# apple/ml-unigen

Hardware: AMD Instinct MI355X
Metric: train-step samples/s (1.5B, 256^2 img) (higher is better)
Workload: dtype bf16

## Files before the change

include/unigen_hip.h:

```cpp
#ifndef UNIGEN_HIP_H
#define UNIGEN_HIP_H

#include <stdint.h>
#include <hip/hip_runtime_api.h>

#ifdef __cplusplus
extern "C" {
#endif

#define UG_ABI_VERSION 7

const char* ug_last_error(void);
int ug_abi_version(void);

typedef struct ug_handle ug_handle;
int ug_create(ug_handle** out);
int ug_destroy(ug_handle* h);

#define UG_EPI_BF16 0
#define UG_EPI_F32 1
#define UG_EPI_RESID 2
int ug_gemm_bf16(const ug_handle* h, const void* A, int64_t lda, int a_kmajor, const void* B, int64_t ldb, int b_kmajor,
                 void* C, int64_t ldc, int64_t M, int64_t N, int64_t K, int epilogue, const void* bias,
                 const float* resid, int64_t ldr, int beta, const float* alpha_dev, int policy, hipStream_t stream);
#define UG_GEMM_NARROW_EPILOGUE 0x100
#define UG_GEMM_ONE_BARRIER 0x200
#define UG_GEMM_TWO_BARRIERS 0x400
#define UG_GEMM_POLICY_AUTO_BITS 0xff

int ug_cast_f32_bf16(const float* in, void* out, int64_t n, hipStream_t stream);

int ug_gemm_bf16_swiglu_bwd(const ug_handle* h, const void* dy, int64_t ld_dy, const void* w_down, int64_t ldw, const void* gu,
                            int64_t ld_gu, void* dgu, int64_t ld_dgu, int64_t M, int64_t I, int64_t K, hipStream_t stream);
int ug_gemm_set_fused_tile_height(int rows);
int ug_gemm_bf16_qkv_rope(const ug_handle* h, const void* x, int64_t ldx, const void* w, int64_t ldw, const void* bias, void* qkv,
                          int64_t ldq, int64_t M, int64_t N, int64_t K, const float* cos_tab, const float* sin_tab, int64_t L,
                          int64_t rope_cols, int head_dim, hipStream_t stream);
int ug_gemm_bf16_swiglu(const ug_handle* h, const void* x, int64_t ldx, const void* w_gate_up, int64_t ldw, void* gu,
                        int64_t ld_gu, void* act, int64_t ld_act, int64_t M, int64_t I, int64_t K, hipStream_t stream);

int ug_gemm_bf16_wgrad_group(int n, const void* const* dy, const int64_t* ld_dy, const void* const* x, const int64_t* ld_x,
                             float* const* dw, const int64_t* ld_dw, const int64_t* rows, const int64_t* cols,
                             const int* beta, const int64_t* K, hipStream_t stream);

int ug_rmsnorm_fwd(const float* x, const float* w, void* y, float* rstd, int64_t rows, int64_t cols,
                   float eps, int out_f32, hipStream_t stream);
int ug_rmsnorm_bwd(const void* dy, const float* x, const float* rstd, const float* w, float* dres,
                   float* dw, void* dres_bf16, int64_t rows, int64_t cols, hipStream_t stream);
int ug_rope(void* qkv, const float* cos_tab, const float* sin_tab, int64_t tokens, int64_t L, int64_t ldq,
            int nheads, int head_dim, int backward, hipStream_t stream);
int ug_swiglu_fwd(const void* gate_up, void* act, int64_t tokens, int64_t I, hipStream_t stream);
int ug_swiglu_bwd(const void* gate_up, const void* dact, void* dgate_up, int64_t tokens, int64_t I,
                  hipStream_t stream);
int ug_gelu(const void* x, const void* dy_or_null, void* out, int64_t n, hipStream_t stream);
int ug_embed_fwd(const int64_t* ids, const float* W, float* out, int64_t tokens, int64_t H, int64_t V,
                 int* err_flag, hipStream_t stream);
int ug_embed_bwd(const int64_t* ids, const float* dout, float* dW, int64_t tokens, int64_t H, int64_t V,
                 hipStream_t stream);
int ug_embed_bwd_sorted(const int64_t* ids_sorted, const int64_t* order, const float* rows, float* dW, int64_t n,
                        int64_t H, int64_t V, float scale, hipStream_t stream);
int ug_gather_rows_bf16(const void* in, int64_t ld_in, const int64_t* idx, void* out, int64_t ld_out,
                        int64_t n, int64_t C, int scatter, hipStream_t stream);
int ug_colsum_bf16(const void* in, int64_t ld, float* out, int64_t R, int64_t C, hipStream_t stream);

#define UG_MASK_F32 0
#define UG_MASK_BF16 1
#define UG_MASK_I64 2
#define UG_MASK_BOOL 3
int ug_attn_mask_compress(const void* mask, int mask_dtype, int64_t stride_b, int64_t stride_row,
                          uint64_t* bits, uint8_t* tileany, int64_t B, int64_t L, int* err_flag,
                          hipStream_t stream);
int ug_attn_mask_causal(const uint8_t* key_valid , uint64_t* bits, uint8_t* tileany,
                        int64_t B, int64_t L, hipStream_t stream);
int ug_attn_fwd(const void* q, const void* k, const void* v, int64_t ldq, void* o,
                int64_t ldo, float* lse, const uint64_t* bits, const uint8_t* tileany, int64_t B, int64_t L,
                int64_t Lp, int H, int HKV, int head_dim, float scale, hipStream_t stream);
int ug_attn_bwd(const void* q, const void* k, const void* v, int64_t ldq,
                const void* o, const void* dout, int64_t ldo, const float* lse,
                float* delta, void* dq, void* dk, void* dv, int64_t ldg, const uint64_t* bits,
                const uint8_t* tileany, int64_t B, int64_t L, int64_t Lp, int H, int HKV, int head_dim,
                float scale, float* dkv_ws, const float* rope_cos, const float* rope_sin, float* dbias_qkv, hipStream_t stream);

int ug_kv_store(const void* qkv, int64_t ldq, int64_t k_col, int64_t v_col, void* cache_k, void* cache_v,
                int64_t rows, int64_t L, int HKV, int head_dim, int64_t Tmax, const int* pos_dev, int pos_host,
                hipStream_t stream);
int ug_rope_at(void* qkv, const float* cos_tab, const float* sin_tab, int64_t rows, int64_t ldq, int nheads,
               int head_dim, const int* pos_dev, int64_t max_pos, hipStream_t stream);
int ug_attn_decode(const void* q, int64_t ldq, const void* cache_k, const void* cache_v, const uint8_t* key_valid,
                   void* o, int64_t ldo, int64_t rows, int H, int HKV, int head_dim, int64_t Tmax,
                   const int* len_dev, float scale, hipStream_t stream);
int ug_gemv_bf16(const void* x, int64_t ldx, int64_t R, const void* W, int64_t ldw, float* acc, int64_t acc_stride_r,
                 int64_t acc_stride_n, int64_t N, int64_t K, hipStream_t stream);
int ug_decode_finish_resid_norm(float* acc, int64_t ldacc, float* x, const float* w, void* xn, int64_t rows, int64_t cols,
                                float eps, int* pos_inc, int* len_inc, hipStream_t stream);
int ug_decode_gemv(const void* x, int64_t ldx, int64_t R, const void* W, int64_t ldw, float* acc, int64_t ldacc, int64_t N,
                   int64_t K, float* zero0, int64_t n0, float* zero1, int64_t n1, float* ss_zero, hipStream_t stream);
int ug_decode_gemv_resid_norm(const float* x_in, const float* pending, int64_t ld_pending, const float* norm_w, float* x_out,
                              float* ss_out, int64_t R, const void* W, int64_t ldw, float* acc, int64_t ldacc, int64_t N,
                              int64_t K, float* zero0, int64_t n0, float* zero1, int64_t n1, float* ss_zero,
                              hipStream_t stream);
int ug_decode_gemv_swiglu(const float* gate_up_acc, int64_t ld_gu, const float* ss_in, float eps, int64_t norm_cols, int64_t R,
                          const void* W, int64_t ldw, float* acc, int64_t ldacc, int64_t N, int64_t K, float* zero0, int64_t n0,
                          float* zero1, int64_t n1, float* ss_zero, hipStream_t stream);
int ug_attn_decode_fused(const float* acc_qkv, int64_t ldacc, const float* ss_in, float eps, int64_t norm_cols, const void* bias,
                         const float* cos_tab, const float* sin_tab, const int* pos_dev, void* cache_k, void* cache_v,
                         const uint8_t* key_valid, void* o, int64_t ldo, int64_t rows, int H, int HKV, int head_dim,
                         int64_t Tmax, int64_t max_pos, float scale, hipStream_t stream);
int ug_decode_sw_supported(int64_t hidden, int64_t inter, int64_t q_dim, int head_dim);
int ug_decode_sw_kblock(const void* x, int64_t ldx, int64_t R, const void* W, int64_t ldw, float* acc, int64_t ldacc, int64_t N, int64_t K,
                        float* zero0, int64_t n0, float* zero1, int64_t n1, float* ss_zero, hipStream_t stream);
int ug_decode_sw_resid(const void* x, int64_t ldx, int64_t R, const void* W, int64_t ldw, int64_t N, int64_t K, float* h,
                       hipStream_t stream);
int ug_decode_sw_gate_up(const float* h, const float* pend, int64_t ld_pend, float* x_out, const float* norm_w, float eps, int64_t R,
                         int64_t H, const void* W, int64_t ldw, int64_t I, void* act, int64_t ld_act, hipStream_t stream);
int ug_decode_sw_head(const float* h, const float* pend, int64_t ld_pend, float* x_out, const float* norm_w, float eps, int64_t R,
                      int64_t H, const void* W, int64_t ldw, int64_t N, float* logits, int64_t ld_logits, int* pos_inc, int* len_inc,
                      hipStream_t stream);
int ug_skinny_finish(const float* acc, const void* bias, void* out_bf16, float* resid, int64_t M, int64_t N,
                     int mode, hipStream_t stream);
int ug_gemv_bf16_ord(const void* x, int64_t ldx, int64_t R, const void* W, int64_t ldw, float* part, int64_t ldpart, int64_t part_stride,
                     int64_t N, int64_t K, hipStream_t stream);
int ug_skinny_finish_ord(const float* parts, int64_t nparts, int64_t part_stride, const void* bias, void* out_bf16, float* out_f32,
                         float* resid, int64_t M, int64_t N, hipStream_t stream);
int ug_decode_gemv_resid_norm_ord(const float* x_in, const float* pend_parts, int64_t ld_pending, int64_t npend, const float* norm_w,
                                  float* x_out, float* ss_part, int64_t R, const void* W, int64_t ldw, float* part, int64_t ldpart,
                                  int64_t N, int64_t K, hipStream_t stream);
int ug_attn_decode_fused_ord(const float* qkv_part, int64_t ldpart, int64_t nparts, const float* ss_part, float eps, int64_t norm_cols,
                             const void* bias, const float* cos_tab, const float* sin_tab, const int* pos_dev, void* cache_k,
                             void* cache_v, const uint8_t* key_valid, void* o, int64_t ldo, int64_t rows, int H, int HKV, int head_dim,
                             int64_t Tmax, int64_t max_pos, float scale, hipStream_t stream);
int ug_decode_sw_kblock_ord(const void* x, int64_t ldx, int64_t R, const void* W, int64_t ldw, float* part, int64_t ldpart, int64_t N,
                            int64_t K, hipStream_t stream);
int ug_decode_finish_resid_norm_ord(const float* parts, int64_t ldp, int64_t nparts, float* x, const float* w, void* xn, int64_t rows,
                                    int64_t cols, float eps, int* pos_inc, int* len_inc, hipStream_t stream);

int ug_t2i_assemble(const int64_t* text_ids, const int64_t* text_offsets, const int64_t* conv_start, int64_t n_start,
                    const int64_t* conv_end, int64_t n_end, const int64_t* image_in, const int64_t* image_labels, int64_t B,
                    int64_t n_image, int64_t max_seq_len, int64_t pad_id, int64_t soi_id, int64_t eoi_id, int64_t ignore_id,
                    int64_t* input_ids, int64_t* labels, uint8_t* attn01, hipStream_t stream);
int ug_attn_mask_from_ids(const int64_t* ids, int64_t B, int64_t L, int64_t pad_id, int64_t soi_id, int64_t eoi_id, int mode,
                          int* meta_ws, uint8_t* flags_ws, uint64_t* bits, uint8_t* tileany, hipStream_t stream);

int ug_maskgit_train_mask(const int64_t* tokens, const float* scores, const float* num_masked, int64_t B, int64_t n,
                          int64_t mask_id, int64_t ignore_id, int64_t* input_ids, int64_t* labels, hipStream_t stream);

int ug_maskgit_step(const void* logits, int64_t ld, int64_t V, int64_t N, int64_t n, int cfg, float guidance_scale,
                    const float* u_sample, const float* u_conf, const int64_t* cur_ids, int64_t mask_id, int64_t id_offset,
                    int64_t mask_len_sched, float temperature, int64_t* sampled, float* sel_ws, int64_t* next_cur,
                    int64_t* next_ids, uint8_t* masking_out, hipStream_t stream);

int ug_ar_sample(float* acc, int64_t ldacc, int64_t bsz, int64_t V, float guidance_scale, float temperature, int greedy,
                 const float* uniforms, const int* pos_dev, int64_t pos0, int64_t nsteps, const float* embed, int64_t ld_embed,
                 int64_t H, int64_t id_offset, int64_t* tok, int* out_tokens, float* x, hipStream_t stream);

int ug_ar_sample_filtered(float* acc, int64_t ldacc, int64_t bsz, int64_t V, float guidance_scale, float temperature, int greedy,
                          const float* uniforms, const int* pos_dev, int64_t pos0, int64_t nsteps, const float* embed,
                          int64_t ld_embed, int64_t H, int64_t id_offset, int64_t* tok, int* out_tokens, float* x, int64_t top_k,
                          float top_p, float min_p, float* stats, hipStream_t stream);

int ug_text_pick(float* logits, int64_t ld, int64_t R, int64_t V, int clear, const int64_t* stop_ids, int64_t n_stop, int64_t pad_id,
                 const float* embed, int64_t ld_embed, int64_t embed_rows, int64_t H, int* state, int64_t nsteps, int64_t* tok,
                 int* out_tokens, int* lengths, float* x, hipStream_t stream);

int ug_text_sample_workspace_ints(int64_t R);

int ug_text_sample(float* logits, int64_t ld, int64_t R, int64_t V, int clear, float temperature, int64_t top_k, float top_p,
                   const float* uniforms, int* workspace, float* stats, const int64_t* stop_ids, int64_t n_stop, int64_t pad_id,
                   const float* embed, int64_t ld_embed, int64_t embed_rows, int64_t H, int* state, int64_t nsteps, int64_t* tok,
                   int* out_tokens, int* lengths, float* x, hipStream_t stream);


int ug_text_seen_mark(int* seen, int64_t ld_words, const int64_t* ids, int64_t ld_ids, int64_t R, int64_t L, const uint8_t* valid,
                      int64_t V, hipStream_t stream);

int ug_text_penalize(float* logits, int64_t ld, int64_t R, int64_t V, float penalty, int* seen, int64_t ld_words, const int64_t* tok,
                     hipStream_t stream);

int ug_ce_fwd(const void* logits, int64_t ld, int64_t R, int64_t V, const int64_t* labels,
              int64_t ignore_index, float* lse, float* loss_row, float* logp_label, float* loss_and_count,
              hipStream_t stream);
int ug_ce_bwd(void* logits_inout, int64_t ld, int64_t R, int64_t V, const int64_t* labels,
              int64_t ignore_index, const float* lse, const float* loss_and_count, const float* gscale,
              const float* row_scale, hipStream_t stream);

int ug_adamw_flat(float* p, const float* g, float* m, float* v, void* p_bf16, int64_t n, float lr,
                  float beta1, float beta2, float eps, float weight_decay, int64_t step, float grad_scale,
                  int max_blocks ,
                  hipStream_t stream);

int ug_grad_pack_bf16(const float* in, void* out_bf16, int64_t n, float scale, hipStream_t stream);
int ug_zero_ranges_f32(float* buf, const int64_t* ranges, int64_t n_ranges, int64_t max_len, hipStream_t stream);
int ug_grad_unpack_bf16(const void* in_bf16, float* out, int64_t n, hipStream_t stream);
int ug_grad_sum_shards_bf16(const void* shards_bf16, int world, int64_t stride, void* out_bf16, int64_t n, float scale,
                            hipStream_t stream);

typedef struct ug_comm ug_comm;
#define UG_COMM_ID_BYTES 128
#define UG_COMM_FP32 0
#define UG_COMM_BF16_FP32ACC 1
#define UG_COMM_BF16 2
#define UG_COMM_FP32_RSAG 3
int ug_comm_unique_id(void* id128);
int ug_comm_init(ug_comm** out, int world, int rank, const void* id128, int64_t max_bucket_elems);
int ug_comm_allreduce_bucket(ug_comm* comm, float* grad, int64_t n, int mode, hipStream_t producer);
int ug_comm_allgather(ug_comm* comm, const void* send, void* recv, int64_t bytes_per_rank, hipStream_t producer);
int ug_comm_wait(ug_comm* comm, hipStream_t consumer);
int ug_comm_destroy(ug_comm* comm);
int64_t ug_comm_bytes_on_wire(const ug_comm* comm);

int ug_conv2d_f32(const float* x, const float* w_packed, const float* bias, const float* residual, float* y,
                  int64_t B, int Hin, int Win, int Cin, int Cout, int cout_pad, int ksize, int stride,
                  int pad_top, int pad_left, int Hout, int Wout, int upsample2x, hipStream_t stream);
int ug_conv_split_weights(const float* w_packed, uint16_t* w_split, int taps, int Cin, int cout_pad, hipStream_t stream);
int ug_amax_f32(const float* x, int64_t rows, int64_t cols, int64_t ld, float* out_amax, hipStream_t stream);
int ug_amax_f32_into_zeroed(const float* x, int64_t rows, int64_t cols, int64_t ld, float* out_amax, hipStream_t stream);
int ug_conv2d_split(const float* x, const float* x_amax, const uint16_t* w_split, const float* bias, const float* residual,
                    float* y, int64_t B, int Hin, int Win, int Cin, int Cout, int cout_pad, int ksize, int stride,
                    int pad_top, int pad_left, int Hout, int Wout, int upsample2x, double* out_stats, int out_groups,
                    hipStream_t stream);
int ug_conv3x3_split(const float* x, const float* x_amax, const uint16_t* w_split, const float* bias, const float* residual,
                     float* y, int64_t B, int H, int W, int Cin, int Cout, int cout_pad, const float* gn_mu_rstd,
                     const float* gn_gamma, const float* gn_beta, int gn_groups, int gn_swish, double* out_stats, int out_groups,
                     hipStream_t stream);
int ug_groupnorm_finalize(const double* stats, float* mu_rstd, int64_t B, int64_t HW, int C, int groups, float eps,
                          hipStream_t stream);
int ug_groupnorm_stats(const float* x, double* stats_ws, float* mu_rstd, int64_t B, int64_t HW, int C, int groups,
                       float eps, hipStream_t stream);
int ug_siglip_attn_f32(const float* qkv, int64_t ld, const float* qkv_amax, float* out, int64_t ldo, int64_t B, int64_t T,
                       int H, int head_dim, float scale, hipStream_t stream);
int ug_linear_split(const float* x, int64_t ldx, const float* x_amax, const uint16_t* w_split, const float* bias,
                    const float* residual, int64_t ldres, float* y, int64_t ldy, int64_t M, int64_t N, int64_t K, int n_pad,
                    int act, hipStream_t stream);
int ug_gemm_f32(const float* A, int64_t lda, int64_t stride_a, const float* B, int64_t ldb, int64_t stride_b,
                int b_is_nk, float* C, int64_t ldc, int64_t stride_c, int64_t M, int64_t N, int64_t K,
                int64_t batch, float alpha, hipStream_t stream);
int ug_gemm_f32_nested(const float* A, int64_t lda, int64_t sa_in, int64_t sa_out, const float* B, int64_t ldb,
                       int64_t sb_in, int64_t sb_out, int b_is_nk, float* C, int64_t ldc, int64_t sc_in, int64_t sc_out,
                       int64_t M, int64_t N, int64_t K, int64_t batch_in, int64_t batch_out, float alpha,
                       hipStream_t stream);
int ug_groupnorm_swish(const float* x, const float* gamma, const float* beta, float* y, double* stats_ws,
                       int64_t B, int64_t HW, int C, int groups, float eps, int apply_swish, hipStream_t stream);
int ug_softmax_rows_f32(float* x, int64_t rows, int64_t cols, int64_t ld, float scale, hipStream_t stream);
int ug_linear_f32(const float* x, int64_t ldx, const float* W, int64_t ldw, const float* bias,
                  const float* residual, int64_t ldres, float* y, int64_t ldy, int64_t M, int64_t N, int64_t K,
                  int act, hipStream_t stream);
int ug_layernorm_f32(const float* x, const float* gamma, const float* beta, float* y, int64_t rows, int64_t cols,
                     float eps, hipStream_t stream);
int ug_layernorm_bwd_f32(const float* dy, const float* x, const float* gamma, const float* dres_in, float* dx, float* dgamma,
                         float* dbeta, int64_t rows, int64_t cols, float eps, hipStream_t stream);
int ug_gelu_tanh_f32(const float* pre, const float* dy_or_null, float* out, int64_t n, hipStream_t stream);
int ug_softmax_bwd_rows_f32(const float* P, float* dP, int64_t rows, int64_t cols, int64_t ld, float scale, hipStream_t stream);
int ug_colsum_f32(const float* x, int64_t ld, float* out, int64_t rows, int64_t cols, hipStream_t stream);
int ug_transpose_f32(const float* in, int64_t ld_in, int64_t stride_in, float* out, int64_t ld_out, int64_t stride_out,
                     int64_t rows, int64_t cols, int64_t batch, hipStream_t stream);
int ug_nchw_to_nhwc(const float* in, float* out, int64_t B, int C, int64_t HW, int c_pad, hipStream_t stream);
int ug_nhwc_to_nchw(const float* in, float* out, int64_t B, int C, int64_t HW, int c_pad, hipStream_t stream);
int ug_lfq_pack(const float* z, int64_t ldz, int64_t* idx, int64_t n, int nbits, hipStream_t stream);
int ug_lfq_unpack(const int64_t* idx, float* z, int64_t n, int nbits, int* err_flag, hipStream_t stream);

int ug_probe_layouts(float* out, int64_t n_floats, hipStream_t stream);

#ifdef __cplusplus
}
#endif
#endif
```

ml-unigen_amd/csrc/gemm_bf16.hip:

```cpp
#include "common.h"
#include <type_traits>
#include <atomic>
#include "unigen_hip.h"
#include "vmem_asm.h"

namespace {

constexpr int BM = 128, BN = 128, BK = 64;
constexpr int TILE_BYTES = BM * BK * 2;
constexpr int GROUP_M = 8;
constexpr int P8_GROUP_M = 4;

enum Epi { EPI_BF16 = 0, EPI_F32 = 1, EPI_RESID = 2, EPI_ROPE = 3, EPI_SWIGLU = 4, EPI_SWIGLU_BWD = 5 };

typedef const __attribute__((address_space(1))) void* gptr_t;
typedef __attribute__((address_space(3))) void* lptr_t;
typedef __attribute__((ext_vector_type(4))) short s16x4_t;

__device__ __attribute__((aligned(16))) uint32_t g_zero_page[64];

struct GemmArgs {
  const bf16_t* A; const bf16_t* B; void* C;
  const bf16_t* bias;
  const float* resid;
  const float* alpha_dev;
  int M, N, K;
  int64_t lda, ldb, ldc, ldr;
  int beta;
  const bf16_t* sw_gu; int64_t ld_gu;
  const float* rope_cos; const float* rope_sin; int rope_L, rope_cols;
  int tiles_m, tiles_n;
  int full_tiles, tail_split;
  float* tail_ws;
  int tail_private;
  int one_barrier;
  int wide_epilogue;
  int swiglu_I;
  bf16_t* act; int64_t ld_act;
};

__device__ __forceinline__ int swz_rowk(int row, int chunk) { return chunk ^ ((row >> 1) & 7); }
__device__ __forceinline__ int swz_krow(int k, int chunk) { return chunk ^ ((((k & 3) | (((k >> 3) & 1) << 2))) << 1); }

template <bool KMAJOR, int ROWS, int NW>
struct Stager {
  static constexpr int NI = ROWS / (8 * NW);
  const bf16_t* src[NI];
  int64_t step[NI];
  int kofs[NI];
  __device__ __forceinline__ void init(const bf16_t* X, int64_t ld, int row0, int rows_total, int wave, int lane) {
    const bf16_t* zero = reinterpret_cast<const bf16_t*>(g_zero_page);
    constexpr int CPR = ROWS / 8;
    constexpr int KPI = 64 / CPR;
#pragma unroll
    for (int i = 0; i < NI; ++i) {
      const int inst = i * NW + wave;
      if constexpr (!KMAJOR) {
        const int row = inst * 8 + (lane >> 3);
        const int chunk = swz_rowk(row, lane & 7);
        const int r = min(row0 + row, rows_total - 1);
        src[i] = X + (int64_t)r * ld + chunk * 8;
        step[i] = BK;
        kofs[i] = chunk * 8;
      } else {
        const int k = inst * KPI + lane / CPR;
        const int chunk = swz_krow(k, lane % CPR);
        const int col = row0 + chunk * 8;
        const bool ok = (col + 8 <= ld);
        src[i] = ok ? X + (int64_t)k * ld + col : zero;
        step[i] = ok ? (int64_t)BK * ld : 0;
        kofs[i] = k;
      }
    }
  }
  template <bool CHECK>
  __device__ __forceinline__ void issue(int kt, int K, char* lds_tile, int wave) const {
    const bf16_t* zero = reinterpret_cast<const bf16_t*>(g_zero_page);
#pragma unroll
    for (int i = 0; i < NI; ++i) {
      const bf16_t* s = src[i] + kt * step[i];
      if constexpr (CHECK) {
        const bool past = kt * BK + kofs[i] >= (KMAJOR ? K : ((K + 7) & ~7));
        s = reinterpret_cast<const bf16_t*>(past ? reinterpret_cast<uintptr_t>(zero) : reinterpret_cast<uintptr_t>(s));
      }
      char* dst = lds_tile + (i * NW + wave) * 1024;
      __builtin_amdgcn_global_load_lds((gptr_t)s, (lptr_t)dst, 16, 0, 0);
    }
  }
};

template <bool KMAJOR, int ROWS>
__device__ __forceinline__ bf16x8_t load_frag(const char* tile, int r0, int ks, int lane) {
  if constexpr (!KMAJOR) {
    const int row = r0 + (lane & 15);
    const int chunk = swz_rowk(row, ks * 4 + (lane >> 4));
    return *reinterpret_cast<const bf16x8_t*>(tile + row * 128 + chunk * 16);
  } else {
    const int i16 = lane & 15, g = lane >> 4;
    const int k = ks * 32 + g * 8 + (i16 >> 2);
    const int chunk = (r0 >> 3) + ((i16 & 3) >> 1);
    const int sub = (i16 & 1) * 8;
    const char* p0 = tile + k * (ROWS * 2) + swz_krow(k, chunk) * 16 + sub;
    const char* p1 = tile + (k + 4) * (ROWS * 2) + swz_krow(k + 4, chunk) * 16 + sub;
    const s16x4_t lo = __builtin_amdgcn_ds_read_tr16_b64_v4i16((__attribute__((address_space(3))) s16x4_t*)p0);
    const s16x4_t hi = __builtin_amdgcn_ds_read_tr16_b64_v4i16((__attribute__((address_space(3))) s16x4_t*)p1);
    return __builtin_shufflevector(lo, hi, 0, 1, 2, 3, 4, 5, 6, 7);
  }
}

template <int EPI>
__device__ __forceinline__ void store_tile(const GemmArgs& p, f32x4_t (&acc)[4][4], int mbase, int nbase, int lane,
                                           bool split) {
  float alpha = 1.f;
  if constexpr (EPI == EPI_F32) { if (p.alpha_dev) alpha = *p.alpha_dev; }
#pragma unroll
  for (int i = 0; i < 4; ++i) {
    const int m = mbase + i * 16 + (lane & 15);
    if (m >= p.M) continue;
#pragma unroll
    for (int j = 0; j < 4; ++j) {
      const int n = nbase + j * 16 + (lane >> 4) * 4;
      if (n >= p.N) continue;
      f32x4_t v = acc[i][j];
      const bool full = (n + 3 < p.N);
      if constexpr (EPI == EPI_BF16) {
        bf16_t* c = reinterpret_cast<bf16_t*>(p.C) + (int64_t)m * p.ldc + n;
        if (p.bias) {
#pragma unroll
          for (int r = 0; r < 4; ++r) if (n + r < p.N) v[r] += bf2f(p.bias[n + r]);
        }
        if (full) {
          uint2 o; o.x = pack_bf2(v[0], v[1]); o.y = pack_bf2(v[2], v[3]);
          *reinterpret_cast<uint2*>(c) = o;
        } else {
          for (int r = 0; r < 4; ++r) if (n + r < p.N) c[r] = f2bf(v[r]);
        }
      } else if constexpr (EPI == EPI_F32) {
        float* c = reinterpret_cast<float*>(p.C) + (int64_t)m * p.ldc + n;
        if (split) {
          for (int r = 0; r < 4; ++r) if (n + r < p.N) atomicAdd(c + r, v[r] * alpha);
        } else if (full) {
          float4 o = make_float4(v[0] * alpha, v[1] * alpha, v[2] * alpha, v[3] * alpha);
          if (p.beta) { const float4 old = *reinterpret_cast<const float4*>(c);
                        o.x += old.x; o.y += old.y; o.z += old.z; o.w += old.w; }
          *reinterpret_cast<float4*>(c) = o;
        } else {
          for (int r = 0; r < 4; ++r) if (n + r < p.N) c[r] = (p.beta ? c[r] : 0.f) + v[r] * alpha;
        }
      } else {
        float* c = reinterpret_cast<float*>(p.C) + (int64_t)m * p.ldc + n;
        const float* rs = p.resid + (int64_t)m * p.ldr + n;
        if (full) {
          const float4 old = *reinterpret_cast<const float4*>(rs);
          float4 o;
          o.x = old.x + bf2f(f2bf(v[0])); o.y = old.y + bf2f(f2bf(v[1]));
          o.z = old.z + bf2f(f2bf(v[2])); o.w = old.w + bf2f(f2bf(v[3]));
          *reinterpret_cast<float4*>(c) = o;
        } else {
          for (int r = 0; r < 4; ++r) if (n + r < p.N) c[r] = rs[r] + bf2f(f2bf(v[r]));
        }
      }
    }
  }
}

#define UG_ST16(ptr, val) (*reinterpret_cast<uint4*>(ptr) = (val))
typedef unsigned int gnt4_t __attribute__((ext_vector_type(4)));
constexpr int EP_ROWS = 32;
constexpr int EP_PITCH_BF16 = 144, EP_PITCH_F32 = 272;
constexpr int EP_STRIP = EP_ROWS * EP_PITCH_F32;

__device__ __forceinline__ void rope_pair(float x1, float x2, float c, float s, float& o1, float& o2) {
#pragma clang fp contract(off)
  const float a1 = x1 * c, a2 = x2 * c;
  const float b1 = x2 * s, b2 = x1 * s;
  o1 = a1 - b1; o2 = a2 + b2;
}

template <int EPI, int MF = 8>
__device__ __forceinline__ void store_tile_lds(const GemmArgs& p, f32x4_t (&acc)[MF][4], char* strip, int mbase, int nbase, int lane,
                                               int rope_p0 = 0, bool roped = false) {
  constexpr bool BF = EPI == EPI_BF16 || EPI == EPI_ROPE;
  float alpha = 1.f;
  if constexpr (EPI == EPI_F32) { if (p.alpha_dev) alpha = *p.alpha_dev; }
  float bias4[4][4];
  if constexpr (BF) {
#pragma unroll
    for (int j = 0; j < 4; ++j) {
      uint2 b = make_uint2(0u, 0u);
      const int cj = EPI == EPI_ROPE ? (j & 1) * 16 + (j >> 1) * 64 : j * 16;
      if (p.bias) b = *reinterpret_cast<const uint2*>(p.bias + nbase + cj + (lane >> 4) * 4);
      bias4[j][0] = __uint_as_float(b.x << 16); bias4[j][1] = __uint_as_float(b.x & 0xffff0000u);
      bias4[j][2] = __uint_as_float(b.y << 16); bias4[j][3] = __uint_as_float(b.y & 0xffff0000u);
    }
  }
#pragma unroll
  for (int c = 0; c < (MF + 1) / 2; ++c) {
    const int rows_here = (2 * c + 1 < MF) ? 32 : 16;
#pragma unroll
    for (int ii = 0; ii < 2; ++ii) {
      if (2 * c + ii >= MF) break;
      const int row = ii * 16 + (lane & 15);
      if constexpr (EPI == EPI_ROPE) {
        if (roped) {
          const int pos = min(mbase + c * EP_ROWS + row, p.M - 1) % p.rope_L;
#pragma unroll
          for (int j = 0; j < 2; ++j) {
            const int pc = rope_p0 + j * 16 + (lane >> 4) * 4;
            const float4 cs = *reinterpret_cast<const float4*>(p.rope_cos + (int64_t)pos * 64 + pc);
            const float4 sn = *reinterpret_cast<const float4*>(p.rope_sin + (int64_t)pos * 64 + pc);
            const float cc[4] = {cs.x, cs.y, cs.z, cs.w}, ss[4] = {sn.x, sn.y, sn.z, sn.w};
            f32x4_t& lo = acc[2 * c + ii][j];
            f32x4_t& hi = acc[2 * c + ii][j + 2];
#pragma unroll
            for (int k = 0; k < 4; ++k) {
              const float x1 = bf2f(f2bf(lo[k] + bias4[j][k])), x2 = bf2f(f2bf(hi[k] + bias4[j + 2][k]));
              float o1, o2;
              rope_pair(x1, x2, cc[k], ss[k], o1, o2);
              lo[k] = o1; hi[k] = o2;
            }
          }
        }
      }
#pragma unroll
      for (int j = 0; j < 4; ++j) {
        const int col = j * 16 + (lane >> 4) * 4;
        const f32x4_t v = acc[2 * c + ii][j];
        if constexpr (EPI == EPI_ROPE) {
          uint2 o;
          if (roped) { o.x = pack_bf2(v[0], v[1]); o.y = pack_bf2(v[2], v[3]); }
          else { o.x = pack_bf2(v[0] + bias4[j][0], v[1] + bias4[j][1]); o.y = pack_bf2(v[2] + bias4[j][2], v[3] + bias4[j][3]); }
          *reinterpret_cast<uint2*>(strip + row * EP_PITCH_BF16 + col * 2) = o;
        } else if constexpr (EPI == EPI_BF16) {
          uint2 o;
          o.x = pack_bf2(v[0] + bias4[j][0], v[1] + bias4[j][1]);
          o.y = pack_bf2(v[2] + bias4[j][2], v[3] + bias4[j][3]);
          *reinterpret_cast<uint2*>(strip + row * EP_PITCH_BF16 + col * 2) = o;
        } else {
          *reinterpret_cast<float4*>(strip + row * EP_PITCH_F32 + col * 4) = make_float4(v[0], v[1], v[2], v[3]);
        }
      }
    }
    asm volatile("s_waitcnt lgkmcnt(0)" ::: "memory");
    if constexpr (BF) {
#pragma unroll
      for (int q = 0; q < 4; ++q) {
        const int row = q * 8 + (lane >> 3), ch = lane & 7;
        const int m = mbase + c * EP_ROWS + row;
        const uint4 v = *reinterpret_cast<const uint4*>(strip + row * EP_PITCH_BF16 + ch * 16);
        const int gc = EPI == EPI_ROPE ? (ch & 3) * 8 + (ch >> 2) * 64 : ch * 8;
        if (m < p.M && row < rows_here) UG_ST16(reinterpret_cast<bf16_t*>(p.C) + (int64_t)m * p.ldc + nbase + gc, v);
      }
    } else {
#pragma unroll
      for (int q = 0; q < 8; ++q) {
        const int row = q * 4 + (lane >> 4), ch = lane & 15;
        const int m = mbase + c * EP_ROWS + row;
        float4 v = *reinterpret_cast<const float4*>(strip + row * EP_PITCH_F32 + ch * 16);
        if (m < p.M && row < rows_here) {
          float* cptr = reinterpret_cast<float*>(p.C) + (int64_t)m * p.ldc + nbase + ch * 4;
          if constexpr (EPI == EPI_F32) {
            v.x *= alpha; v.y *= alpha; v.z *= alpha; v.w *= alpha;
            if (p.beta) { const float4 old = *reinterpret_cast<const float4*>(cptr); v.x += old.x; v.y += old.y; v.z += old.z; v.w += old.w; }
          } else {
            const float4 old = *reinterpret_cast<const float4*>(p.resid + (int64_t)m * p.ldr + nbase + ch * 4);
            v.x = old.x + bf2f(f2bf(v.x)); v.y = old.y + bf2f(f2bf(v.y)); v.z = old.z + bf2f(f2bf(v.z)); v.w = old.w + bf2f(f2bf(v.w));
          }
          *reinterpret_cast<float4*>(cptr) = v;
        }
      }
    }
    asm volatile("s_waitcnt lgkmcnt(0)" ::: "memory");
  }
}

__device__ __forceinline__ float silu_gemm(float g) { return silu_train(g); }

template <int MF>
__device__ __forceinline__ void store_tile_swiglu_perm(const GemmArgs& p, f32x4_t (&acc)[MF][4], char* strip, int mbase, int hbase, int lane) {
  constexpr int ACT_PITCH = 80;
  char* astrip = strip + EP_ROWS * EP_PITCH_BF16;
  bf16_t* C = reinterpret_cast<bf16_t*>(p.C);
#pragma unroll
  for (int c = 0; c < (MF + 1) / 2; ++c) {
    const int rows_here = (2 * c + 1 < MF) ? 32 : 16;
#pragma unroll
    for (int ii = 0; ii < 2; ++ii) {
      if (2 * c + ii >= MF) break;
      const int row = ii * 16 + (lane & 15);
#pragma unroll
      for (int j = 0; j < 2; ++j) {
        const f32x4_t gv = acc[2 * c + ii][j], uv = acc[2 * c + ii][j + 2];
        float a[4];
        uint32_t gb[4], ub[4];
#pragma unroll
        for (int k = 0; k < 4; ++k) {
          gb[k] = f2bf(gv[k]); ub[k] = f2bf(uv[k]);
          const float s = bf2f(f2bf(silu_gemm(bf2f((bf16_t)gb[k]))));
          a[k] = s * bf2f((bf16_t)ub[k]);
        }
        const int col = j * 16 + (lane >> 4) * 4;
        *reinterpret_cast<uint2*>(strip + row * EP_PITCH_BF16 + col * 2) = make_uint2(gb[0] | (gb[1] << 16), gb[2] | (gb[3] << 16));
        *reinterpret_cast<uint2*>(strip + row * EP_PITCH_BF16 + (32 + col) * 2) = make_uint2(ub[0] | (ub[1] << 16), ub[2] | (ub[3] << 16));
        *reinterpret_cast<uint2*>(astrip + row * ACT_PITCH + col * 2) = make_uint2(pack_bf2(a[0], a[1]), pack_bf2(a[2], a[3]));
      }
    }
    asm volatile("s_waitcnt lgkmcnt(0)" ::: "memory");
#pragma unroll
    for (int q = 0; q < 4; ++q) {
      const int row = q * 8 + (lane >> 3), ch = lane & 7;
      const int m = mbase + c * EP_ROWS + row;
      const uint4 v = *reinterpret_cast<const uint4*>(strip + row * EP_PITCH_BF16 + ch * 16);
      const int gc = (ch >> 2) * p.swiglu_I + hbase + (ch & 3) * 8;
      if (m < p.M && row < rows_here) UG_ST16(C + (int64_t)m * p.ldc + gc, v);
    }
#pragma unroll
    for (int q = 0; q < 2; ++q) {
      const int row = q * 16 + (lane >> 2), ch = lane & 3;
      const int m = mbase + c * EP_ROWS + row;
      const uint4 v = *reinterpret_cast<const uint4*>(astrip + row * ACT_PITCH + ch * 16);
      if (m < p.M && row < rows_here)
        UG_ST16(p.act + (int64_t)m * p.ld_act + hbase + ch * 8, v);
    }
    asm volatile("s_waitcnt lgkmcnt(0)" ::: "memory");
  }
}

typedef unsigned int gu4_t __attribute__((ext_vector_type(4)));
template <int MF>
__device__ __forceinline__ void store_tile_swiglu_bwd(const GemmArgs& p, f32x4_t (&acc)[MF][4], char* strip, int mbase, int nbase, int lane) {
  constexpr int NCH = (MF + 1) / 2;
  bf16_t* C = reinterpret_cast<bf16_t*>(p.C);
  const int I = p.swiglu_I;
  gu4_t gq[2][4], uq[2][4];
  auto fetch = [&](int c, gu4_t (&g)[4], gu4_t (&u)[4]) {
#pragma unroll
    for (int q = 0; q < 4; ++q) {
      const int row = q * 8 + (lane >> 3), ch = lane & 7;
      const int m = min(mbase + c * EP_ROWS + row, p.M - 1);
      const bf16_t* gp = p.sw_gu + (int64_t)m * p.ld_gu + nbase + ch * 8;
      asm volatile("global_load_dwordx4 %0, %1, off" : "=&v"(g[q]) : "v"(gp) : "memory");
      asm volatile("global_load_dwordx4 %0, %1, off" : "=&v"(u[q]) : "v"(gp + I) : "memory");
    }
  };
  fetch(0, gq[0], uq[0]);
#pragma unroll
  for (int c = 0; c < NCH; ++c) {
    const int rows_here = (2 * c + 1 < MF) ? 32 : 16;
    gu4_t (&g)[4] = gq[c & 1];
    gu4_t (&u)[4] = uq[c & 1];
    if (c + 1 < NCH) fetch(c + 1, gq[(c + 1) & 1], uq[(c + 1) & 1]);
#pragma unroll
    for (int ii = 0; ii < 2; ++ii) {
      if (2 * c + ii >= MF) break;
      const int row = ii * 16 + (lane & 15);
#pragma unroll
      for (int j = 0; j < 4; ++j) {
        const f32x4_t v = acc[2 * c + ii][j];
        *reinterpret_cast<uint2*>(strip + row * EP_PITCH_BF16 + (j * 16 + (lane >> 4) * 4) * 2) = make_uint2(pack_bf2(v[0], v[1]), pack_bf2(v[2], v[3]));
      }
    }
    if (c + 1 < NCH)
      asm volatile("s_waitcnt vmcnt(8)" : "+v"(g[0]), "+v"(g[1]), "+v"(g[2]), "+v"(g[3]), "+v"(u[0]), "+v"(u[1]), "+v"(u[2]), "+v"(u[3]) : : "memory");
    else
      asm volatile("s_waitcnt vmcnt(0)" : "+v"(g[0]), "+v"(g[1]), "+v"(g[2]), "+v"(g[3]), "+v"(u[0]), "+v"(u[1]), "+v"(u[2]), "+v"(u[3]) : : "memory");
    asm volatile("s_waitcnt lgkmcnt(0)" ::: "memory");
#pragma unroll
    for (int q = 0; q < 4; ++q) {
      const int row = q * 8 + (lane >> 3), ch = lane & 7;
      const int m = mbase + c * EP_ROWS + row;
      const uint4 dv = *reinterpret_cast<const uint4*>(strip + row * EP_PITCH_BF16 + ch * 16);
      const uint32_t dw[4] = {dv.x, dv.y, dv.z, dv.w};
      uint32_t og[4], ou[4];
#pragma unroll
      for (int e = 0; e < 4; ++e) {
        float g0, g1, u0, u1;
        swiglu_bwd_elem(__uint_as_float(g[q][e] << 16), __uint_as_float(u[q][e] << 16), __uint_as_float(dw[e] << 16), g0, u0);
        swiglu_bwd_elem(__uint_as_float(g[q][e] & 0xffff0000u), __uint_as_float(u[q][e] & 0xffff0000u), __uint_as_float(dw[e] & 0xffff0000u), g1, u1);
        og[e] = pack_bf2(g0, g1); ou[e] = pack_bf2(u0, u1);
      }
      if (m < p.M && row < rows_here) {
        bf16_t* cp = C + (int64_t)m * p.ldc + nbase + ch * 8;
        UG_ST16(cp, make_uint4(og[0], og[1], og[2], og[3]));
        UG_ST16(cp + I, make_uint4(ou[0], ou[1], ou[2], ou[3]));
      }
    }
    asm volatile("s_waitcnt lgkmcnt(0)" ::: "memory");
  }
}

template <int EPI, bool AK, bool BKM, bool DBUF>
__global__ __launch_bounds__(256, DBUF ? 2 : 4) void gemm_kernel(GemmArgs p) {
  __shared__ __attribute__((aligned(16))) char lds[(DBUF ? 4 : 2) * TILE_BYTES];
  const int tid = threadIdx.x, lane = tid & 63, wave = tid >> 6;
  const int wm = wave >> 1, wn = wave & 1;

  const int nwg = p.tiles_m * p.tiles_n;
  const int pid = xcd_remap(blockIdx.x, nwg);
  const int per_group = GROUP_M * p.tiles_n;
  const int gid = pid / per_group, first_m = gid * GROUP_M;
  const int gsz = min(p.tiles_m - first_m, GROUP_M);
  const int tm = first_m + (pid % per_group) % gsz;
  const int tn = (pid % per_group) / gsz;
  const int m0 = tm * BM, n0 = tn * BN;

  Stager<AK, BM, 4> sa; Stager<BKM, BN, 4> sb;
  sa.init(p.A, p.lda, m0, p.M, wave, lane);
  sb.init(p.B, p.ldb, n0, p.N, wave, lane);

  f32x4_t acc[4][4];
#pragma unroll
  for (int i = 0; i < 4; ++i)
#pragma unroll
    for (int j = 0; j < 4; ++j) acc[i][j] = f32x4_t{0.f, 0.f, 0.f, 0.f};

  const int nk_all = (p.K + BK - 1) / BK;
  const int per_split = (nk_all + gridDim.y - 1) / gridDim.y;
  const int kt0 = blockIdx.y * per_split;
  const int nk = min(nk_all, kt0 + per_split);
  if (kt0 >= nk) return;
  const bool ragged = (p.K % BK) != 0;
  if (kt0 + 1 == nk_all && ragged) { sa.template issue<true>(kt0, p.K, lds, wave); sb.template issue<true>(kt0, p.K, lds + TILE_BYTES, wave); }
  else { sa.template issue<false>(kt0, p.K, lds, wave); sb.template issue<false>(kt0, p.K, lds + TILE_BYTES, wave); }
  __syncthreads();

  for (int kt = kt0; kt < nk; ++kt) {
    const int cur = DBUF ? ((kt - kt0) & 1) : 0;
    if (DBUF && kt + 1 < nk) {
      char* nxt = lds + (cur ^ 1) * 2 * TILE_BYTES;
      if (ragged && kt + 2 == nk_all) { sa.template issue<true>(kt + 1, p.K, nxt, wave); sb.template issue<true>(kt + 1, p.K, nxt + TILE_BYTES, wave); }
      else { sa.template issue<false>(kt + 1, p.K, nxt, wave); sb.template issue<false>(kt + 1, p.K, nxt + TILE_BYTES, wave); }
    }
    const char* tA = lds + cur * 2 * TILE_BYTES;
    const char* tB = tA + TILE_BYTES;
#pragma unroll
    for (int ks = 0; ks < 2; ++ks) {
      bf16x8_t fa[4], fb[4];
#pragma unroll
      for (int i = 0; i < 4; ++i) {
        fa[i] = load_frag<AK, BM>(tA, wm * 64 + i * 16, ks, lane);
        fb[i] = load_frag<BKM, BN>(tB, wn * 64 + i * 16, ks, lane);
      }
#pragma unroll
      for (int i = 0; i < 4; ++i)
#pragma unroll
        for (int j = 0; j < 4; ++j)
          acc[i][j] = __builtin_amdgcn_mfma_f32_16x16x32_bf16(fb[j], fa[i], acc[i][j], 0, 0, 0);
    }
    __syncthreads();
    if constexpr (!DBUF) {
      if (kt + 1 < nk) {
        if (ragged && kt + 2 == nk_all) { sa.template issue<true>(kt + 1, p.K, lds, wave); sb.template issue<true>(kt + 1, p.K, lds + TILE_BYTES, wave); }
        else { sa.template issue<false>(kt + 1, p.K, lds, wave); sb.template issue<false>(kt + 1, p.K, lds + TILE_BYTES, wave); }
        __syncthreads();
      }
    }
  }

  store_tile<EPI>(p, acc, m0 + wm * 64, n0 + wn * 64, lane, gridDim.y > 1);
}

constexpr int PBM = 256, PBN = 256, PBK = 32;
constexpr int P_TILE = PBM * PBK * 2;
constexpr int P_STAGE = 2 * P_TILE;
constexpr int P_NST = 4;
constexpr int CPOL_STAGER = 0, CPOL_P10A = 0;
static_assert(CPOL_P10A == 0, "dma16 issues the default cache policy");

__device__ __forceinline__ int swz_rowk32(int row, int chunk) { return chunk ^ ((0 - (row >> 2)) & 3); }

template <bool KMAJOR>
struct Stager32 {
  const bf16_t* src[2];
  int64_t step[2];
  int kofs[2];
  __device__ __forceinline__ void init(const bf16_t* X, int64_t ld, int row0, int rows_total, int wave, int lane, int split_rows = 0) {
    const bf16_t* zero = reinterpret_cast<const bf16_t*>(g_zero_page);
#pragma unroll
    for (int i = 0; i < 2; ++i) {
      const int inst = i * 8 + wave;
      if constexpr (!KMAJOR) {
        const int row = inst * 16 + (lane >> 2);
        const int chunk = swz_rowk32(row, lane & 3);
        const int grow = (split_rows > 0 && row >= 128) ? split_rows + row0 + row - 128 : row0 + row;
        const int r = min(grow, rows_total - 1);
        src[i] = X + (int64_t)r * ld + chunk * 8;
        step[i] = PBK;
        kofs[i] = chunk * 8;
      } else {
        const int k = inst * 2 + (lane >> 5);
        const int chunk = swz_krow(k, lane & 31);
        const int col = row0 + chunk * 8;
        const bool ok = (col + 8 <= ld);
        src[i] = ok ? X + (int64_t)k * ld + col : zero;
        step[i] = ok ? (int64_t)PBK * ld : 0;
        kofs[i] = k;
      }
    }
  }
  template <bool CHECK>
  __device__ __forceinline__ void issue(int kt, int K, char* lds_tile, int wave) const {
    const bf16_t* zero = reinterpret_cast<const bf16_t*>(g_zero_page);
#pragma unroll
    for (int i = 0; i < 2; ++i) {
      const bf16_t* s = src[i] + kt * step[i];
      if constexpr (CHECK) {
        const bool past = kt * PBK + kofs[i] >= (KMAJOR ? K : ((K + 7) & ~7));
        s = reinterpret_cast<const bf16_t*>(past ? reinterpret_cast<uintptr_t>(zero) : reinterpret_cast<uintptr_t>(s));
      }
      char* dst = lds_tile + (i * 8 + wave) * 1024;
      static_assert(CPOL_STAGER == 0, "dma16 issues the default cache policy");
      dma16(s, __builtin_amdgcn_readfirstlane(lds_addr_of(dst)));
    }
  }
};

template <bool KMAJOR>
__device__ __forceinline__ bf16x8_t load_frag32(const char* tile, int r0, int lane) {
  if constexpr (!KMAJOR) {
    const int row = r0 + (lane & 15);
    return *reinterpret_cast<const bf16x8_t*>(tile + row * 64 + swz_rowk32(row, lane >> 4) * 16);
  } else {
    const int i16 = lane & 15, g = lane >> 4;
    const int k = g * 8 + (i16 >> 2);
    const int chunk = (r0 >> 3) + ((i16 & 3) >> 1);
    const int sub = (i16 & 1) * 8;
    const char* p0 = tile + k * (PBM * 2) + swz_krow(k, chunk) * 16 + sub;
    const char* p1 = tile + (k + 4) * (PBM * 2) + swz_krow(k + 4, chunk) * 16 + sub;
    const s16x4_t lo = __builtin_amdgcn_ds_read_tr16_b64_v4i16((__attribute__((address_space(3))) s16x4_t*)p0);
    const s16x4_t hi = __builtin_amdgcn_ds_read_tr16_b64_v4i16((__attribute__((address_space(3))) s16x4_t*)p1);
    return __builtin_shufflevector(lo, hi, 0, 1, 2, 3, 4, 5, 6, 7);
  }
}

#define P_BARRIER() asm volatile("s_barrier" ::: "memory")

#define UG_MFMA_BLOCK(NI)                                                                                                  \
  _Pragma("unroll") for (int i = 0; i < (NI); ++i) _Pragma("unroll") for (int jj = 0; jj < 4; ++jj) {                       \
    const int j = (i & 1) ? 3 - jj : jj;                                                                                   \
    acc[i][j] = __builtin_amdgcn_mfma_f32_16x16x32_bf16(fb[j], fa[i], acc[i][j], 0, 0, 0);                                  \
    __builtin_amdgcn_sched_barrier(0); }

template <int EPI, bool AK, bool BKM, bool ONEBAR>
__device__ __forceinline__ void p8_body(const GemmArgs& p, const int bid, char* lds) {
  const int tid = threadIdx.x, lane = tid & 63;
  const int wave = __builtin_amdgcn_readfirstlane(tid >> 6);
  const int grp = wave >> 2, wn = wave & 3;

  const int nwg = p.tiles_m * p.tiles_n;
  const bool tail = p.tail_split > 1 && bid >= p.full_tiles;
  const int tail_j = tail ? bid - p.full_tiles : 0;
  const int tile_lin = tail ? p.full_tiles + tail_j / p.tail_split : bid;
  const int pid = xcd_remap(tile_lin, nwg);
  const int per_group = P8_GROUP_M * p.tiles_n;
  const int gid = pid / per_group, first_m = gid * P8_GROUP_M;
  const int gsz = min(p.tiles_m - first_m, P8_GROUP_M);
  const int tm = first_m + (pid % per_group) % gsz;
  const int tn = (pid % per_group) / gsz;
  const int m0 = tm * PBM, n0 = tn * PBN;

  Stager32<AK> sa; Stager32<BKM> sb;
  sa.init(p.A, p.lda, m0, p.M, wave, lane);
  sb.init(p.B, p.ldb, n0, p.N, wave, lane);

  f32x4_t acc[8][4];
#pragma unroll
  for (int i = 0; i < 8; ++i)
#pragma unroll
    for (int j = 0; j < 4; ++j) acc[i][j] = f32x4_t{0.f, 0.f, 0.f, 0.f};

  const int nk_all = (p.K + PBK - 1) / PBK;
  const int per_split = tail ? (nk_all + p.tail_split - 1) / p.tail_split : nk_all;
  const int kt0 = tail ? (tail_j % p.tail_split) * per_split : 0;
  const int nk = min(nk_all, kt0 + per_split) - kt0;
  if (nk <= 0) return;
  const bool ragged = (p.K % PBK) != 0;
  auto stage_in = [&](int lt) {
    const int kt = kt0 + lt;
    char* st = lds + (lt & (P_NST - 1)) * P_STAGE;
    if (ragged && kt + 1 == nk_all) { sa.template issue<true>(kt, p.K, st, wave); sb.template issue<true>(kt, p.K, st + P_TILE, wave); }
    else { sa.template issue<false>(kt, p.K, st, wave); sb.template issue<false>(kt, p.K, st + P_TILE, wave); }
  };
  auto stage_whole = [&](int lt) {
    char* st = lds + (lt & (P_NST - 1)) * P_STAGE;
    sa.template issue<false>(kt0 + lt, p.K, st, wave);
    sb.template issue<false>(kt0 + lt, p.K, st + P_TILE, wave);
  };
  const int nk_steady = max(nk - 4, 0);
  bf16x8_t fa[8], fb[4];
  auto read_frags = [&](int t) {
    const char* tA = lds + (t & (P_NST - 1)) * P_STAGE;
    const char* tB = tA + P_TILE;
#pragma unroll
    for (int i = 0; i < 8; ++i) fa[i] = load_frag32<AK>(tA, grp * 128 + i * 16, lane);
#pragma unroll
    for (int j = 0; j < 4; ++j) fb[j] = load_frag32<BKM>(tB, wn * 64 + j * 16, lane);
  };
  auto request = [&](int t, auto steady) {
    if constexpr (decltype(steady)::value) stage_whole(t + 3);
    else if (t + 3 < nk) stage_in(t + 3);
  };
  auto landed = [&](int t, auto steady) {
    if constexpr (decltype(steady)::value) asm volatile("s_waitcnt vmcnt(8)" ::: "memory");
    else if (t + 3 < nk) asm volatile("s_waitcnt vmcnt(8)" ::: "memory");
    else if (t + 2 < nk) asm volatile("s_waitcnt vmcnt(4)" ::: "memory");
    else asm volatile("s_waitcnt vmcnt(0)" ::: "memory");
  };
  auto mfmas = [&](int prio) {
    __builtin_amdgcn_sched_barrier(0);
    if (prio == 2) __builtin_amdgcn_s_setprio(2); else __builtin_amdgcn_s_setprio(1);
    UG_MFMA_BLOCK(8)
    __builtin_amdgcn_s_setprio(0);
    __builtin_amdgcn_sched_barrier(0);
  };
  const std::true_type STEADY{};
  const std::false_type CHECKED{};
  stage_in(0);
  if (nk > 1) stage_in(1);
  if (nk > 2) stage_in(2);
  if (nk > 2) asm volatile("s_waitcnt vmcnt(8)" ::: "memory");
  else if (nk > 1) asm volatile("s_waitcnt vmcnt(4)" ::: "memory");
  else asm volatile("s_waitcnt vmcnt(0)" ::: "memory");
  if constexpr (ONEBAR) {
    if (grp == 0) {
      auto interval = [&](int t, auto steady) {
        P_BARRIER();
        read_frags(t);
        request(t, steady);
        asm volatile("s_waitcnt lgkmcnt(0)" ::: "memory");
        mfmas(1);
        landed(t, steady);
      };
      int t = 0;
      for (; t < nk_steady; ++t) interval(t, STEADY);
      for (; t < nk; ++t) interval(t, CHECKED);
      P_BARRIER();
    } else {
      P_BARRIER();
      read_frags(0);
      request(0, CHECKED);
      landed(0, CHECKED);
      asm volatile("s_waitcnt lgkmcnt(0)" ::: "memory");
      auto interval = [&](int t, auto steady) {
        P_BARRIER();
        mfmas(2);
        read_frags(t);
        request(t, steady);
        asm volatile("s_waitcnt lgkmcnt(0)" ::: "memory");
        landed(t, steady);
      };
      int t = 1;
      for (; t < nk_steady; ++t) interval(t, STEADY);
      for (; t < nk; ++t) interval(t, CHECKED);
      P_BARRIER();
      mfmas(2);
    }
  } else {
    P_BARRIER();
    if (grp == 1) P_BARRIER();
    auto iteration = [&](int t, auto steady) {
      read_frags(t);
      request(t, steady);
      landed(t, steady);
      asm volatile("s_waitcnt lgkmcnt(0)" ::: "memory");
      P_BARRIER();
      mfmas(1);
      P_BARRIER();
    };
    int t = 0;
    for (; t < nk_steady; ++t) iteration(t, STEADY);
    for (; t < nk; ++t) iteration(t, CHECKED);
    if (grp == 0) P_BARRIER();
  }

  if (tail) {
    const int64_t slot = p.tail_private ? (int64_t)(tile_lin - p.full_tiles) * p.tail_split + tail_j % p.tail_split
                                        : (int64_t)(tile_lin - p.full_tiles);
    float* ws = p.tail_ws + slot * (PBM * PBN);
#pragma unroll
    for (int i = 0; i < 8; ++i) {
      const int ml = grp * 128 + i * 16 + (lane & 15);
#pragma unroll
      for (int j = 0; j < 4; ++j) {
        float* dst = ws + ml * PBN + wn * 64 + j * 16 + (lane >> 4) * 4;
        if (p.tail_private) {
          *reinterpret_cast<float4*>(dst) = make_float4(acc[i][j][0], acc[i][j][1], acc[i][j][2], acc[i][j][3]);
        } else {
#pragma unroll
          for (int r = 0; r < 4; ++r) atomicAdd(dst + r, acc[i][j][r]);
        }
      }
    }
    return;
  }
  const bool wide = (n0 + PBN <= p.N) && p.wide_epilogue &&
                    (EPI == EPI_BF16 ? (p.ldc % 8 == 0 && (!p.bias || (reinterpret_cast<uintptr_t>(p.bias) & 7) == 0))
                                     : (p.ldc % 4 == 0 && (EPI != EPI_RESID || p.ldr % 4 == 0)));
  if (wide) {
    store_tile_lds<EPI>(p, acc, lds + wave * EP_STRIP, m0 + grp * 128, n0 + wn * 64, lane);
    return;
  }
  store_tile<EPI>(p, reinterpret_cast<f32x4_t (&)[4][4]>(acc[0]), m0 + grp * 128, n0 + wn * 64, lane, false);
  store_tile<EPI>(p, reinterpret_cast<f32x4_t (&)[4][4]>(acc[4]), m0 + grp * 128 + 64, n0 + wn * 64, lane, false);
}

template <int EPI, bool AK, bool BKM, bool ONEBAR = false>
__global__ __launch_bounds__(512, 2) void gemm_kernel_p8(GemmArgs p) {
  __shared__ __attribute__((aligned(16))) char lds[P_NST * P_STAGE];
  p8_body<EPI, AK, BKM, ONEBAR>(p, (int)blockIdx.x, lds);
}

constexpr int GROUP_MAX = 8;
struct GroupProblem {
  const bf16_t* A; const bf16_t* B; float* C;
  int64_t lda, ldb, ldc;
  int M, N, K, beta, tiles_m, tiles_n, start;
};
struct GroupArgs { GroupProblem pr[GROUP_MAX]; int n; };

__global__ __launch_bounds__(512, 2) void gemm_kernel_p8_wgrad_group(GroupArgs g) {
  __shared__ __attribute__((aligned(16))) char lds[P_NST * P_STAGE];
  const int b = (int)blockIdx.x;
  int q = 0;
#pragma unroll
  for (int i = 1; i < GROUP_MAX; ++i) if (i < g.n && b >= g.pr[i].start) q = i;
  const GroupProblem& pr = g.pr[q];
  const int local = b - pr.start;
  if (local >= pr.tiles_m * pr.tiles_n) return;
  GemmArgs p;
  p.A = pr.A; p.B = pr.B; p.C = pr.C; p.bias = nullptr; p.resid = nullptr; p.alpha_dev = nullptr;
  p.M = pr.M; p.N = pr.N; p.K = pr.K; p.lda = pr.lda; p.ldb = pr.ldb; p.ldc = pr.ldc; p.ldr = 0; p.beta = pr.beta;
  p.tiles_m = pr.tiles_m; p.tiles_n = pr.tiles_n; p.full_tiles = pr.tiles_m * pr.tiles_n; p.tail_split = 1;
  p.tail_ws = nullptr; p.tail_private = 1; p.one_barrier = 1; p.wide_epilogue = 1; p.swiglu_I = 0; p.act = nullptr; p.ld_act = 0;
  p8_body<EPI_F32, true, true, true>(p, local, lds);
}

constexpr int P10_GROUP_M = 4;
constexpr int QBM = 320;
constexpr int Q_TILE_A = QBM * PBK * 2;
constexpr int Q_STAGE = Q_TILE_A + P_TILE;

template <int EPI, bool BKM, int F0, int F1>
__global__ __launch_bounds__(512, 2) void gemm_kernel_p10(GemmArgs p) {
  constexpr int BMV = 16 * (F0 + F1), NINST = BMV / 16, LO = NINST / 8, REM = NINST % 8;
  constexpr int TILE_A = BMV * PBK * 2, STAGE = TILE_A + P_TILE;
  static_assert(F0 >= F1 && F0 <= 10 && F1 >= 1 && LO >= 1 && LO + (REM ? 1 : 0) <= 3, "gemm_kernel_p10: unsupported tile height");
  __shared__ __attribute__((aligned(16))) char lds[P_NST * STAGE];
  const int tid = threadIdx.x, lane = tid & 63;
  const int wave = __builtin_amdgcn_readfirstlane(tid >> 6);
  const int grp = wave >> 2, wn = wave & 3;
  const int nwg = p.tiles_m * p.tiles_n;
  const int pid = xcd_remap((int)blockIdx.x, nwg);
  const int per_group = P10_GROUP_M * p.tiles_n;
  const int gid = pid / per_group, first_m = gid * P10_GROUP_M;
  const int gsz = min(p.tiles_m - first_m, P10_GROUP_M);
  const int tm = first_m + (pid % per_group) % gsz;
  const int tn = (pid % per_group) / gsz;
  const int m0 = tm * BMV, n0 = tn * PBN;

  const bf16_t* asrc[3];
#pragma unroll
  for (int i = 0; i < 3; ++i) {
    const int inst = min(i * 8 + wave, NINST - 1);
    const int row = inst * 16 + (lane >> 2);
    const int r = min(m0 + row, p.M - 1);
    asrc[i] = p.A + (int64_t)r * p.lda + swz_rowk32(row, lane & 3) * 8;
  }
  Stager32<BKM> sb;
  if constexpr (EPI == EPI_SWIGLU) sb.init(p.B, p.ldb, tn * 128, p.N, wave, lane, p.swiglu_I);
  else sb.init(p.B, p.ldb, n0, p.N, wave, lane);

  f32x4_t acc[F0][4];
#pragma unroll
  for (int i = 0; i < F0; ++i)
#pragma unroll
    for (int j = 0; j < 4; ++j) acc[i][j] = f32x4_t{0.f, 0.f, 0.f, 0.f};
  const int nk = p.K / PBK;

  auto run = [&](auto group0, auto na_tag) {
    constexpr bool G0 = decltype(group0)::value;
    constexpr int NA = decltype(na_tag)::value;
    constexpr int FG = G0 ? F0 : F1;
    constexpr int PER = NA + 2;
    auto stage_in = [&](int lt) {
      char* st = lds + (lt & (P_NST - 1)) * STAGE;
#pragma unroll
      for (int i = 0; i < NA; ++i)
        dma16(asrc[i] + (int64_t)lt * PBK, __builtin_amdgcn_readfirstlane(lds_addr_of(st + (i * 8 + wave) * 1024)));
      sb.template issue<false>(lt, p.K, st + TILE_A, wave);
    };
    auto landed = [&](int in_flight) {
      if (in_flight >= 2) asm volatile("s_waitcnt vmcnt(%0)" ::"n"(2 * PER) : "memory");
      else if (in_flight == 1) asm volatile("s_waitcnt vmcnt(%0)" ::"n"(PER) : "memory");
      else asm volatile("s_waitcnt vmcnt(0)" ::: "memory");
    };
    stage_in(0);
    if (nk > 1) stage_in(1);
    if (nk > 2) stage_in(2);
    landed(min(nk, 3) - 1);
    P_BARRIER();
    if (!G0) P_BARRIER();
    auto iteration = [&](int t, auto steady) {
      const char* tA = lds + (t & (P_NST - 1)) * STAGE;
      const char* tB = tA + TILE_A;
      bf16x8_t fa[FG], fb[4];
#pragma unroll
      for (int i = 0; i < FG; ++i) fa[i] = load_frag32<false>(tA, (G0 ? 0 : 16 * F0) + i * 16, lane);
#pragma unroll
      for (int j = 0; j < 4; ++j)
        fb[j] = load_frag32<BKM>(tB, EPI == EPI_ROPE ? (wn >> 1) * 128 + (wn & 1) * 32 + (j & 1) * 16 + (j >> 1) * 64
                                     : EPI == EPI_SWIGLU ? (j >> 1) * 128 + wn * 32 + (j & 1) * 16 : wn * 64 + j * 16, lane);
      if constexpr (decltype(steady)::value) {
        stage_in(t + 3);
        landed(2);
      } else {
        if (t + 3 < nk) stage_in(t + 3);
        landed(min(nk - 1, t + 3) - (t + 1));
      }
      asm volatile("s_waitcnt lgkmcnt(0)" ::: "memory");
      P_BARRIER();
      __builtin_amdgcn_s_setprio(1);
      UG_MFMA_BLOCK(FG)
      __builtin_amdgcn_s_setprio(0);
      P_BARRIER();
    };
    int t = 0;
    for (; t + 4 < nk; ++t) iteration(t, std::true_type{});
    for (; t < nk; ++t) iteration(t, std::false_type{});
    if (G0) P_BARRIER();
    if constexpr (EPI == EPI_SWIGLU_BWD)
      store_tile_swiglu_bwd<FG>(p, reinterpret_cast<f32x4_t (&)[FG][4]>(acc[0]), lds + wave * EP_STRIP, m0 + (G0 ? 0 : 16 * F0), n0 + wn * 64, lane);
    else if constexpr (EPI == EPI_SWIGLU)
      store_tile_swiglu_perm<FG>(p, reinterpret_cast<f32x4_t (&)[FG][4]>(acc[0]), lds + wave * EP_STRIP, m0 + (G0 ? 0 : 16 * F0), tn * 128 + wn * 32, lane);
    else if constexpr (EPI == EPI_ROPE)
      store_tile_lds<EPI, FG>(p, reinterpret_cast<f32x4_t (&)[FG][4]>(acc[0]), lds + wave * EP_STRIP, m0 + (G0 ? 0 : 16 * F0),
                              n0 + (wn >> 1) * 128 + (wn & 1) * 32, lane, (wn & 1) * 32, n0 < p.rope_cols);
    else
      store_tile_lds<EPI, FG>(p, reinterpret_cast<f32x4_t (&)[FG][4]>(acc[0]), lds + wave * EP_STRIP, m0 + (G0 ? 0 : 16 * F0), n0 + wn * 64, lane);
  };
  const bool more = REM != 0 && wave < REM;
  if (grp == 0) { if (more) run(std::true_type{}, std::integral_constant<int, LO + (REM ? 1 : 0)>{}); else run(std::true_type{}, std::integral_constant<int, LO>{}); }
  else { if (more) run(std::false_type{}, std::integral_constant<int, LO + (REM ? 1 : 0)>{}); else run(std::false_type{}, std::integral_constant<int, LO>{}); }
}


template <int EPI>
__global__ __launch_bounds__(256) void tail_finish_kernel(GemmArgs p, int ntail) {
  const int nwg = p.tiles_m * p.tiles_n;
  const int per_tile = PBM * PBN / 4;
  const int64_t total = (int64_t)ntail * per_tile;
  float alpha = 1.f;
  if constexpr (EPI == EPI_F32) { if (p.alpha_dev) alpha = *p.alpha_dev; }
  for (int64_t idx = blockIdx.x * (int64_t)blockDim.x + threadIdx.x; idx < total; idx += (int64_t)gridDim.x * blockDim.x) {
    const int tl = (int)(idx / per_tile), q = (int)(idx % per_tile);
    const int pid = xcd_remap(p.full_tiles + tl, nwg);
    const int per_group = P8_GROUP_M * p.tiles_n;
    const int gid = pid / per_group, first_m = gid * P8_GROUP_M;
    const int gsz = min(p.tiles_m - first_m, P8_GROUP_M);
    const int tm = first_m + (pid % per_group) % gsz;
    const int tn = (pid % per_group) / gsz;
    const int ml = q / (PBN / 4), nl = (q % (PBN / 4)) * 4;
    float4 v4;
    if (p.tail_private) {
      const int nk_all = (p.K + PBK - 1) / PBK, per_split = (nk_all + p.tail_split - 1) / p.tail_split;
      v4 = make_float4(0.f, 0.f, 0.f, 0.f);
      for (int sp = 0; sp < p.tail_split && sp * per_split < nk_all; ++sp) {
        const float4 t = *reinterpret_cast<const float4*>(p.tail_ws + ((int64_t)tl * p.tail_split + sp) * (PBM * PBN) + ml * PBN + nl);
        v4.x += t.x; v4.y += t.y; v4.z += t.z; v4.w += t.w;
      }
    } else {
      float4* src = reinterpret_cast<float4*>(p.tail_ws + (int64_t)tl * (PBM * PBN) + ml * PBN + nl);
      v4 = *src;
      *src = make_float4(0.f, 0.f, 0.f, 0.f);
    }
    const int m = tm * PBM + ml, n = tn * PBN + nl;
    if (m >= p.M || n >= p.N) continue;
    float v[4] = {v4.x, v4.y, v4.z, v4.w};
    for (int r = 0; r < 4 && n + r < p.N; ++r) {
      if constexpr (EPI == EPI_BF16) {
        float o = v[r];
        if (p.bias) o += bf2f(p.bias[n + r]);
        reinterpret_cast<bf16_t*>(p.C)[(int64_t)m * p.ldc + n + r] = f2bf(o);
      } else if constexpr (EPI == EPI_F32) {
        float* c = reinterpret_cast<float*>(p.C) + (int64_t)m * p.ldc + n + r;
        *c = (p.beta ? *c : 0.f) + v[r] * alpha;
      } else {
        reinterpret_cast<float*>(p.C)[(int64_t)m * p.ldc + n + r] = p.resid[(int64_t)m * p.ldr + n + r] + bf2f(f2bf(v[r]));
      }
    }
  }
}

constexpr int WS_PRIVATE_SLOTS = UG_HANDLE_WS_SLOTS;

template <int EPI, bool AK, bool BKM>
int launch(GemmArgs a, const ug_handle* h, int policy, hipStream_t st) {
  float* const ws = (h && h->tail_ws) ? h->tail_ws : nullptr;
  const int g_tile_policy = policy;
  const int tiles = a.tiles_m * a.tiles_n;
  int splits = 1;
  if (EPI == EPI_F32 && a.beta == 1 && tiles < 384) {
    const int nk = (a.K + BK - 1) / BK;
    splits = min(32, max(1, 768 / tiles));
    splits = max(1, min(splits, nk / 2));
  }
  const int tiles_p8 = ((a.M + PBM - 1) / PBM) * ((a.N + PBN - 1) / PBN);
  const int rounds = (tiles_p8 + 255) / 256;
  const bool p8_fits = (tiles_p8 <= 256) ? (tiles_p8 >= 200) : (4 * tiles_p8 >= 3 * rounds * 256);
  if constexpr (!AK && EPI != EPI_F32) {
    const int tiles_q = ((a.M + QBM - 1) / QBM) * (a.N / PBN);
    const bool aligned = a.N % PBN == 0 && a.K % PBK == 0 &&
                         (EPI == EPI_BF16 ? (a.ldc % 8 == 0 && (!a.bias || (reinterpret_cast<uintptr_t>(a.bias) & 7) == 0))
                                          : (a.ldc % 4 == 0 && a.ldr % 4 == 0));
    const bool fewer_rounds = tiles_p8 >= 1024 && 1.1625f * (float)((tiles_q + 255) / 256) < 0.97f * (float)((tiles_p8 + 255) / 256);
    int hb_multi = 0;
    int hb = 0;
    static const bool heights_on = !(getenv("UNIGEN_GEMM_HEIGHTS") && atoi(getenv("UNIGEN_GEMM_HEIGHTS")) == 0);
    if (aligned && g_tile_policy < 0 && a.N / PBN >= 1 && a.N / PBN <= 64) {
      static const int heights[] = {128, 144, 160, 176, 192, 208, 224, 240, 256, 272, 288, 304, 320};
      for (int h_ : heights) {
        if (!heights_on && h_ != QBM) continue;
        const int64_t wgs = (int64_t)((a.M + h_ - 1) / h_) * (a.N / PBN);
        if (wgs <= 256) { if (wgs >= 64 && !(a.K / PBK >= 2048 && wgs < 200)) hb = h_; break; }
      }
      if (hb == 256 && p8_fits) hb = 0;
    }
    if (aligned && g_tile_policy < 0 && heights_on && hb == 0 && tiles_p8 >= 768) {
      static const int mheights[] = {176, 192, 208, 224, 240, 272, 288, 304, 320};
      float best = 0.97f * (float)((tiles_p8 + 255) / 256);
      for (int h_ : mheights) {
        const int64_t wgs = (int64_t)((a.M + h_ - 1) / h_) * (a.N / PBN);
        const float cost = (float)((wgs + 255) / 256) * (0.35f + 0.00254f * (float)h_);
        if (cost < best) { best = cost; hb_multi = h_; }
      }
    }
    if (aligned && g_tile_policy >= 40 && g_tile_policy <= 52 && g_tile_policy != 48) hb = 16 * (g_tile_policy - 32);
    if (hb == 0 && hb_multi != 0) hb = hb_multi;
    if (hb == 0 && aligned && (g_tile_policy == 10 || (g_tile_policy < 0 && !heights_on && fewer_rounds))) hb = QBM;
    if (hb != 0) {
      a.tiles_m = (a.M + hb - 1) / hb; a.tiles_n = a.N / PBN;
      const dim3 grid(a.tiles_m * a.tiles_n), block(512);
      switch (hb) {
        case 320: hipLaunchKernelGGL((gemm_kernel_p10<EPI, BKM, 10, 10>), grid, block, 0, st, a); break;
        case 304: hipLaunchKernelGGL((gemm_kernel_p10<EPI, BKM, 10, 9>), grid, block, 0, st, a); break;
        case 288: hipLaunchKernelGGL((gemm_kernel_p10<EPI, BKM, 9, 9>), grid, block, 0, st, a); break;
        case 272: hipLaunchKernelGGL((gemm_kernel_p10<EPI, BKM, 9, 8>), grid, block, 0, st, a); break;
        case 256: hipLaunchKernelGGL((gemm_kernel_p10<EPI, BKM, 8, 8>), grid, block, 0, st, a); break;
        case 240: hipLaunchKernelGGL((gemm_kernel_p10<EPI, BKM, 8, 7>), grid, block, 0, st, a); break;
        case 224: hipLaunchKernelGGL((gemm_kernel_p10<EPI, BKM, 7, 7>), grid, block, 0, st, a); break;
        case 208: hipLaunchKernelGGL((gemm_kernel_p10<EPI, BKM, 7, 6>), grid, block, 0, st, a); break;
        case 192: hipLaunchKernelGGL((gemm_kernel_p10<EPI, BKM, 6, 6>), grid, block, 0, st, a); break;
        case 176: hipLaunchKernelGGL((gemm_kernel_p10<EPI, BKM, 6, 5>), grid, block, 0, st, a); break;
        case 160: hipLaunchKernelGGL((gemm_kernel_p10<EPI, BKM, 5, 5>), grid, block, 0, st, a); break;
        case 144: hipLaunchKernelGGL((gemm_kernel_p10<EPI, BKM, 5, 4>), grid, block, 0, st, a); break;
        default: hipLaunchKernelGGL((gemm_kernel_p10<EPI, BKM, 4, 4>), grid, block, 0, st, a); break;
      }
      UG_CHECK_LAUNCH("ug_gemm_bf16(p10)");
      return UG_OK;
    }
  }
  int tail_r = 0, tail_s = 1;
  if (!p8_fits && tiles_p8 > 256 && (tiles_p8 % 256) <= 128 && g_tile_policy != 5) {
    const int r = tiles_p8 % 256, nk32 = (a.K + PBK - 1) / PBK;
    int sp = 256 / r;
    while (sp > 1 && nk32 / sp < 40) --sp;
    if ((sp >= 3 || g_tile_policy == 6) && sp >= 2 && r * sp <= WS_PRIVATE_SLOTS && ws) { tail_r = r; tail_s = sp; }
  }
  {
    const int nk32 = (a.K + PBK - 1) / PBK;
    int sp = 0;
    if (EPI == EPI_F32 && tiles_p8 >= 24 && tiles_p8 <= 128 && a.M >= 512 && a.N >= 512) {
      sp = 256 / tiles_p8;
      while (sp > 1 && nk32 / sp < 32) --sp;
    } else if (tiles_p8 >= 24 && tiles_p8 < 200 && nk32 >= 2048) {
      float best = (tiles_p8 > 128) ? (float)tiles_p8 / 256.f : 0.f;
      for (int c = 2; c <= 8 && tiles_p8 * c <= WS_PRIVATE_SLOTS; ++c) {
        const int items = tiles_p8 * c, r = (items + 255) / 256;
        const float eff = (float)items / (float)(r * 256);
        if (eff > best + 0.01f) { best = eff; sp = c; }
      }
    }
    if (sp >= 2 && tiles_p8 * sp <= WS_PRIVATE_SLOTS && (g_tile_policy < 0 || g_tile_policy == 8) && ws) {
      a.tiles_m = (a.M + PBM - 1) / PBM; a.tiles_n = (a.N + PBN - 1) / PBN;
      a.full_tiles = 0; a.tail_split = sp; a.tail_private = 1;
      a.tail_ws = ws;
      if (a.one_barrier) hipLaunchKernelGGL((gemm_kernel_p8<EPI, AK, BKM, true>), dim3(tiles_p8 * sp), dim3(512), 0, st, a);
      else hipLaunchKernelGGL((gemm_kernel_p8<EPI, AK, BKM>), dim3(tiles_p8 * sp), dim3(512), 0, st, a);
      UG_CHECK_LAUNCH("ug_gemm_bf16(p8 k-sliced)");
      hipLaunchKernelGGL((tail_finish_kernel<EPI>), dim3(tiles_p8 * 16), dim3(256), 0, st, a, tiles_p8);
      UG_CHECK_LAUNCH("ug_gemm_bf16(partial sum)");
      return UG_OK;
    }
  }
  if (g_tile_policy == 3 || g_tile_policy == 6 || (g_tile_policy < 0 && (p8_fits || tail_s > 1))) {
    a.tiles_m = (a.M + PBM - 1) / PBM; a.tiles_n = (a.N + PBN - 1) / PBN;
    a.full_tiles = tiles_p8 - tail_r; a.tail_split = tail_s;
    a.tail_private = 1;
    a.tail_ws = ws;
    if (a.one_barrier) hipLaunchKernelGGL((gemm_kernel_p8<EPI, AK, BKM, true>), dim3(a.full_tiles + tail_r * tail_s), dim3(512), 0, st, a);
    else hipLaunchKernelGGL((gemm_kernel_p8<EPI, AK, BKM>), dim3(a.full_tiles + tail_r * tail_s), dim3(512), 0, st, a);
    UG_CHECK_LAUNCH("ug_gemm_bf16(p8)");
    if (tail_s > 1) {
      hipLaunchKernelGGL((tail_finish_kernel<EPI>), dim3(tail_r * 16), dim3(256), 0, st, a, tail_r);
      UG_CHECK_LAUNCH("ug_gemm_bf16(tail finish)");
    }
    return UG_OK;
  }
  bool dbuf = (!AK && !BKM && a.K >= 4096);
  if (g_tile_policy == 0) dbuf = true;
  if (g_tile_policy == 2) dbuf = false;
  dim3 grid(tiles, splits);
  if (dbuf) hipLaunchKernelGGL((gemm_kernel<EPI, AK, BKM, true>), grid, dim3(256), 0, st, a);
  else hipLaunchKernelGGL((gemm_kernel<EPI, AK, BKM, false>), grid, dim3(256), 0, st, a);
  UG_CHECK_LAUNCH("ug_gemm_bf16");
  return UG_OK;
}

}

extern "C" int ug_gemm_bf16(const ug_handle* h, const void* A, int64_t lda, int a_kmajor, const void* B, int64_t ldb, int b_kmajor,
                            void* C, int64_t ldc, int64_t M, int64_t N, int64_t K, int epilogue, const void* bias,
                            const float* resid, int64_t ldr, int beta, const float* alpha_dev, int policy, hipStream_t stream) {
  UG_REQUIRE(M > 0 && N > 0 && K > 0, "ug_gemm_bf16: empty problem M=%ld N=%ld K=%ld", (long)M, (long)N, (long)K);
  UG_REQUIRE(lda % 8 == 0 && ldb % 8 == 0, "ug_gemm_bf16: lda/ldb must be multiples of 8 elements (16-byte rows)");
  UG_REQUIRE(ug_aligned16(A) && ug_aligned16(B) && ug_aligned16(C), "ug_gemm_bf16: A/B/C must be 16-byte aligned");
  UG_REQUIRE(ldc % 4 == 0, "ug_gemm_bf16: ldc must be a multiple of 4 elements");
  UG_REQUIRE(M < (1 << 30) && N < (1 << 30) && K < (1 << 30), "ug_gemm_bf16: dims too large");
  UG_REQUIRE(a_kmajor || b_kmajor || K % 8 == 0,
             "ug_gemm_bf16: K=%ld must be a multiple of 8 when both operands are row-major", (long)K);
  UG_REQUIRE(a_kmajor || lda >= ((K + 7) & ~7LL), "ug_gemm_bf16: row-major A needs lda >= round_up(K,8)");
  UG_REQUIRE(b_kmajor || ldb >= ((K + 7) & ~7LL), "ug_gemm_bf16: row-major B needs ldb >= round_up(K,8)");
  UG_REQUIRE(!a_kmajor || lda >= M, "ug_gemm_bf16: k-major A needs lda >= M");
  UG_REQUIRE(!b_kmajor || ldb >= N, "ug_gemm_bf16: k-major B needs ldb >= N");
  GemmArgs a;
  a.A = (const bf16_t*)A; a.B = (const bf16_t*)B; a.C = C;
  a.bias = (const bf16_t*)bias; a.resid = resid; a.alpha_dev = alpha_dev;
  a.M = (int)M; a.N = (int)N; a.K = (int)K;
  a.lda = lda; a.ldb = ldb; a.ldc = ldc; a.ldr = ldr; a.beta = beta;
  a.swiglu_I = 0; a.act = nullptr; a.ld_act = 0;
  a.wide_epilogue = (policy >= 0 && (policy & UG_GEMM_NARROW_EPILOGUE)) ? 0 : 1;
  a.one_barrier = (a_kmajor && b_kmajor) ? 1 : 0;
  if (policy >= 0 && (policy & UG_GEMM_ONE_BARRIER)) a.one_barrier = 1;
  if (policy >= 0 && (policy & UG_GEMM_TWO_BARRIERS)) a.one_barrier = 0;
  if (policy >= 0) policy &= ~(UG_GEMM_NARROW_EPILOGUE | UG_GEMM_ONE_BARRIER | UG_GEMM_TWO_BARRIERS);
  if (policy == UG_GEMM_POLICY_AUTO_BITS) policy = -1;
  a.tiles_m = (int)((M + BM - 1) / BM); a.tiles_n = (int)((N + BN - 1) / BN);
  const int mode = (a_kmajor ? 2 : 0) | (b_kmajor ? 1 : 0);
  if (epilogue == EPI_RESID) UG_REQUIRE(resid != nullptr && ldr % 4 == 0, "ug_gemm_bf16: EPI_RESID needs a 16B-aligned residual");
  switch (mode * 4 + epilogue) {
    case 0 * 4 + EPI_BF16: return launch<EPI_BF16, false, false>(a, h, policy, stream);
    case 0 * 4 + EPI_F32: return launch<EPI_F32, false, false>(a, h, policy, stream);
    case 0 * 4 + EPI_RESID: return launch<EPI_RESID, false, false>(a, h, policy, stream);
    case 1 * 4 + EPI_BF16: return launch<EPI_BF16, false, true>(a, h, policy, stream);
    case 1 * 4 + EPI_F32: return launch<EPI_F32, false, true>(a, h, policy, stream);
    case 3 * 4 + EPI_F32: return launch<EPI_F32, true, true>(a, h, policy, stream);
    case 3 * 4 + EPI_BF16: return launch<EPI_BF16, true, true>(a, h, policy, stream);
    default:
      ug_set_error("ug_gemm_bf16: layout/epilogue combination (a_kmajor=%d b_kmajor=%d epilogue=%d) is not instantiated",
                   a_kmajor, b_kmajor, epilogue);
      return UG_ERR_ARG;
  }
}

extern "C" int ug_gemm_bf16_wgrad_group(int n, const void* const* dy, const int64_t* ld_dy, const void* const* x, const int64_t* ld_x,
                                        float* const* dw, const int64_t* ld_dw, const int64_t* rows, const int64_t* cols,
                                        const int* beta, const int64_t* K, hipStream_t stream) {
  UG_REQUIRE(n >= 1 && n <= GROUP_MAX && K, "ug_gemm_bf16_wgrad_group: 1..%d problems and their contraction lengths required", GROUP_MAX);
  GroupArgs g;
  g.n = n;
  int start = 0;
  for (int i = 0; i < n; ++i) {
    UG_REQUIRE(rows[i] > 0 && cols[i] > 0 && rows[i] < (1 << 30) && cols[i] < (1 << 30) && K[i] > 0 && K[i] < (1 << 30),
               "ug_gemm_bf16_wgrad_group: empty problem %d", i);
    UG_REQUIRE(ld_dy[i] % 8 == 0 && ld_x[i] % 8 == 0 && ld_dy[i] >= rows[i] && ld_x[i] >= cols[i] && ld_dw[i] % 4 == 0 && ld_dw[i] >= cols[i],
               "ug_gemm_bf16_wgrad_group: problem %d: token-major operands need leading dimensions that are multiples of 8 and cover "
               "their rows; ld_dw a multiple of 4", i);
    UG_REQUIRE(ug_aligned16(dy[i]) && ug_aligned16(x[i]) && ug_aligned16(dw[i]), "ug_gemm_bf16_wgrad_group: problem %d: 16-byte alignment", i);
    GroupProblem& pr = g.pr[i];
    pr.A = (const bf16_t*)dy[i]; pr.B = (const bf16_t*)x[i]; pr.C = dw[i];
    pr.lda = ld_dy[i]; pr.ldb = ld_x[i]; pr.ldc = ld_dw[i];
    pr.M = (int)rows[i]; pr.N = (int)cols[i]; pr.K = (int)K[i]; pr.beta = beta[i];
    pr.tiles_m = (pr.M + PBM - 1) / PBM; pr.tiles_n = (pr.N + PBN - 1) / PBN;
    pr.start = start;
    start += (pr.tiles_m * pr.tiles_n + 7) & ~7;
  }
  for (int i = n; i < GROUP_MAX; ++i) { g.pr[i] = g.pr[0]; g.pr[i].start = 1 << 30; }
  hipLaunchKernelGGL(gemm_kernel_p8_wgrad_group, dim3(start), dim3(512), 0, stream, g);
  UG_CHECK_LAUNCH("ug_gemm_bf16_wgrad_group");
  return UG_OK;
}


static std::atomic<int> g_fused_height{0};
extern "C" int ug_gemm_set_fused_tile_height(int rows) {
  UG_REQUIRE(rows == 0 || (rows >= 128 && rows <= 320 && rows % 16 == 0), "ug_gemm_set_fused_tile_height: 0 (automatic) or 128 ... 320 in steps of 16 (%d)", rows);
  g_fused_height.store(rows);
  return UG_OK;
}
template <size_t NH>
static int pick_fused_height(const int (&heights)[NH], int64_t M, int64_t col_tiles, const char* who, int* out) {
  const int forced = g_fused_height.load();
  if (forced) {
    for (int h_ : heights)
      if (h_ == forced) { *out = forced; return UG_OK; }
    ug_set_error("%s: tile height %d forced by ug_gemm_set_fused_tile_height is not instantiated for this epilogue", who, forced);
    return UG_ERR_ARG;
  }
  int hb = heights[NH - 1]; float best = 1e30f;
  for (int h_ : heights) {
    const int64_t wgs = ((M + h_ - 1) / h_) * col_tiles;
    const float cost = (float)((wgs + 255) / 256) * (0.35f + 0.00254f * (float)h_);
    if (cost < best) { best = cost; hb = h_; }
  }
  *out = hb;
  return UG_OK;
}

extern "C" int ug_swiglu_fwd(const void* gate_up, void* act, int64_t tokens, int64_t I, hipStream_t st);

extern "C" int ug_gemm_bf16_swiglu(const ug_handle* h, const void* x, int64_t ldx, const void* w_gate_up, int64_t ldw, void* gu,
                                   int64_t ld_gu, void* act, int64_t ld_act, int64_t M, int64_t I, int64_t K, hipStream_t stream) {
  UG_REQUIRE(M > 0 && I > 0 && K > 0 && K % 8 == 0 && I % 8 == 0, "ug_gemm_bf16_swiglu: bad problem M=%ld I=%ld K=%ld", (long)M, (long)I, (long)K);
  UG_REQUIRE(ldx % 8 == 0 && ldw % 8 == 0 && ld_gu % 8 == 0 && ld_act % 8 == 0 && ldx >= K && ldw >= K && ld_gu >= 2 * I && ld_act >= I,
             "ug_gemm_bf16_swiglu: row strides must be multiples of 8 elements and cover the rows");
  UG_REQUIRE(ug_aligned16(x) && ug_aligned16(w_gate_up) && ug_aligned16(gu) && ug_aligned16(act), "ug_gemm_bf16_swiglu: alignment");
  UG_REQUIRE(M < (1 << 30) && I < (1 << 29) && K < (1 << 30), "ug_gemm_bf16_swiglu: dims too large");
  const int64_t tiles = ((M + PBM - 1) / PBM) * (2 * I / PBN);
  if (I % 128 != 0 || tiles < 64 || K % PBK != 0 || 2 * I / PBN > (1 << 20)) {
    if (int rc = ug_gemm_bf16(h, x, ldx, 0, w_gate_up, ldw, 0, gu, ld_gu, M, 2 * I, K, EPI_BF16, nullptr, nullptr, 0, 0, nullptr, -1, stream))
      return rc;
    UG_REQUIRE(ld_gu == 2 * I && ld_act == I, "ug_gemm_bf16_swiglu: the two-launch form needs packed gu / act rows");
    return ug_swiglu_fwd(gu, act, M, I, stream);
  }
  GemmArgs a{};
  a.A = (const bf16_t*)x; a.B = (const bf16_t*)w_gate_up; a.C = gu;
  a.M = (int)M; a.N = (int)(2 * I); a.K = (int)K;
  a.lda = ldx; a.ldb = ldw; a.ldc = ld_gu;
  a.tail_split = 1; a.tail_private = 1; a.wide_epilogue = 1;
  a.swiglu_I = (int)I; a.act = (bf16_t*)act; a.ld_act = ld_act;
  static const int heights[] = {128, 160, 192, 208, 224, 256, 288, 320};
  int hb = 320;
  if (int rc = pick_fused_height(heights, M, 2 * I / PBN, "ug_gemm_bf16_swiglu", &hb)) return rc;
  a.tiles_m = (int)((M + hb - 1) / hb); a.tiles_n = (int)(2 * I / PBN);
  const dim3 grid(a.tiles_m * a.tiles_n), block(512);
  switch (hb) {
    case 320: hipLaunchKernelGGL((gemm_kernel_p10<EPI_SWIGLU, false, 10, 10>), grid, block, 0, stream, a); break;
    case 288: hipLaunchKernelGGL((gemm_kernel_p10<EPI_SWIGLU, false, 9, 9>), grid, block, 0, stream, a); break;
    case 256: hipLaunchKernelGGL((gemm_kernel_p10<EPI_SWIGLU, false, 8, 8>), grid, block, 0, stream, a); break;
    case 224: hipLaunchKernelGGL((gemm_kernel_p10<EPI_SWIGLU, false, 7, 7>), grid, block, 0, stream, a); break;
    case 208: hipLaunchKernelGGL((gemm_kernel_p10<EPI_SWIGLU, false, 7, 6>), grid, block, 0, stream, a); break;
    case 192: hipLaunchKernelGGL((gemm_kernel_p10<EPI_SWIGLU, false, 6, 6>), grid, block, 0, stream, a); break;
    case 160: hipLaunchKernelGGL((gemm_kernel_p10<EPI_SWIGLU, false, 5, 5>), grid, block, 0, stream, a); break;
    default: hipLaunchKernelGGL((gemm_kernel_p10<EPI_SWIGLU, false, 4, 4>), grid, block, 0, stream, a); break;
  }
  UG_CHECK_LAUNCH("ug_gemm_bf16_swiglu(p10)");
  return UG_OK;
}

extern "C" int ug_rope(void* qkv, const float* cos_tab, const float* sin_tab, int64_t tokens, int64_t L, int64_t ldq,
                       int nheads, int head_dim, int backward, hipStream_t st);

extern "C" int ug_gemm_bf16_qkv_rope(const ug_handle* h, const void* x, int64_t ldx, const void* w, int64_t ldw, const void* bias, void* qkv,
                                     int64_t ldq, int64_t M, int64_t N, int64_t K, const float* cos_tab, const float* sin_tab, int64_t L,
                                     int64_t rope_cols, int head_dim, hipStream_t stream) {
  UG_REQUIRE(M > 0 && N > 0 && K > 0 && L > 0 && M % L == 0 && head_dim > 0 && rope_cols >= 0 && rope_cols <= N && rope_cols % head_dim == 0,
             "ug_gemm_bf16_qkv_rope: bad problem M=%ld N=%ld K=%ld L=%ld rope_cols=%ld head_dim=%d", (long)M, (long)N, (long)K, (long)L,
             (long)rope_cols, head_dim);
  UG_REQUIRE(cos_tab && sin_tab && ug_aligned16(cos_tab) && ug_aligned16(sin_tab), "ug_gemm_bf16_qkv_rope: cos / sin tables [L, head_dim / 2] fp32, 16-byte aligned");
  UG_REQUIRE(M < (1 << 30) && N < (1 << 30) && K < (1 << 30), "ug_gemm_bf16_qkv_rope: dims too large");
  const bool fused = head_dim == 128 && N % PBN == 0 && rope_cols % PBN == 0 && K % PBK == 0 && ldq % 8 == 0 && ldx % 8 == 0 && ldw % 8 == 0 &&
                     ldx >= K && ldw >= K && ldq >= N && ug_aligned16(x) && ug_aligned16(w) && ug_aligned16(qkv) &&
                     (!bias || (reinterpret_cast<uintptr_t>(bias) & 7) == 0) && N / PBN <= 64;
  static const bool fused_on = !(getenv("UNIGEN_FUSED_ROPE") && atoi(getenv("UNIGEN_FUSED_ROPE")) == 0);
  if (!fused || !fused_on) {
    if (int rc = ug_gemm_bf16(h, x, ldx, 0, w, ldw, 0, qkv, ldq, M, N, K, EPI_BF16, bias, nullptr, 0, 0, nullptr, -1, stream)) return rc;
    if (rope_cols == 0) return UG_OK;
    return ug_rope(qkv, cos_tab, sin_tab, M, L, ldq, (int)(rope_cols / head_dim), head_dim, 0, stream);
  }
  GemmArgs a{};
  a.A = (const bf16_t*)x; a.B = (const bf16_t*)w; a.C = qkv; a.bias = (const bf16_t*)bias;
  a.M = (int)M; a.N = (int)N; a.K = (int)K; a.lda = ldx; a.ldb = ldw; a.ldc = ldq;
  a.rope_cos = cos_tab; a.rope_sin = sin_tab; a.rope_L = (int)L; a.rope_cols = (int)rope_cols;
  a.tail_split = 1; a.tail_private = 1; a.wide_epilogue = 1;
  static const int heights[] = {128, 160, 192, 208, 224, 256, 288, 320};
  int hb = 320;
  if (int rc = pick_fused_height(heights, M, N / PBN, "ug_gemm_bf16_qkv_rope", &hb)) return rc;
  a.tiles_m = (int)((M + hb - 1) / hb); a.tiles_n = (int)(N / PBN);
  const dim3 grid(a.tiles_m * a.tiles_n), block(512);
  switch (hb) {
    case 320: hipLaunchKernelGGL((gemm_kernel_p10<EPI_ROPE, false, 10, 10>), grid, block, 0, stream, a); break;
    case 288: hipLaunchKernelGGL((gemm_kernel_p10<EPI_ROPE, false, 9, 9>), grid, block, 0, stream, a); break;
    case 256: hipLaunchKernelGGL((gemm_kernel_p10<EPI_ROPE, false, 8, 8>), grid, block, 0, stream, a); break;
    case 224: hipLaunchKernelGGL((gemm_kernel_p10<EPI_ROPE, false, 7, 7>), grid, block, 0, stream, a); break;
    case 208: hipLaunchKernelGGL((gemm_kernel_p10<EPI_ROPE, false, 7, 6>), grid, block, 0, stream, a); break;
    case 192: hipLaunchKernelGGL((gemm_kernel_p10<EPI_ROPE, false, 6, 6>), grid, block, 0, stream, a); break;
    case 160: hipLaunchKernelGGL((gemm_kernel_p10<EPI_ROPE, false, 5, 5>), grid, block, 0, stream, a); break;
    default: hipLaunchKernelGGL((gemm_kernel_p10<EPI_ROPE, false, 4, 4>), grid, block, 0, stream, a); break;
  }
  UG_CHECK_LAUNCH("ug_gemm_bf16_qkv_rope");
  return UG_OK;
}


extern "C" int ug_gemm_bf16_swiglu_bwd(const ug_handle* h, const void* dy, int64_t ld_dy, const void* w_down, int64_t ldw, const void* gu,
                                       int64_t ld_gu, void* dgu, int64_t ld_dgu, int64_t M, int64_t I, int64_t K, hipStream_t stream) {
  (void)h;
  UG_REQUIRE(M > 0 && I > 0 && K > 0 && M < (1 << 30) && I < (1 << 29) && K < (1 << 30), "ug_gemm_bf16_swiglu_bwd: bad problem M=%ld I=%ld K=%ld", (long)M, (long)I, (long)K);
  UG_REQUIRE(I % PBN == 0 && K % PBK == 0 && I / PBN <= (1 << 20), "ug_gemm_bf16_swiglu_bwd: fused form needs I %% 256 == 0 and K %% 32 == 0 (I=%ld K=%ld): run ug_gemm_bf16 + ug_swiglu_bwd", (long)I, (long)K);
  UG_REQUIRE(ld_dy % 8 == 0 && ldw % 8 == 0 && ld_gu % 8 == 0 && ld_dgu % 8 == 0 && ld_dy >= K && ldw >= I && ld_gu >= 2 * I && ld_dgu >= 2 * I,
             "ug_gemm_bf16_swiglu_bwd: row strides must be multiples of 8 elements and cover the rows");
  UG_REQUIRE(ug_aligned16(dy) && ug_aligned16(w_down) && ug_aligned16(gu) && ug_aligned16(dgu), "ug_gemm_bf16_swiglu_bwd: alignment");
  GemmArgs a{};
  a.A = (const bf16_t*)dy; a.B = (const bf16_t*)w_down; a.C = dgu;
  a.M = (int)M; a.N = (int)I; a.K = (int)K; a.lda = ld_dy; a.ldb = ldw; a.ldc = ld_dgu;
  a.sw_gu = (const bf16_t*)gu; a.ld_gu = ld_gu; a.swiglu_I = (int)I;
  a.tail_split = 1; a.tail_private = 1; a.wide_epilogue = 1;
  static const int heights[] = {128, 160, 192, 208, 224, 256, 272, 288, 320};
  int hb = 320;
  if (int rc = pick_fused_height(heights, M, I / PBN, "ug_gemm_bf16_swiglu_bwd", &hb)) return rc;
  a.tiles_m = (int)((M + hb - 1) / hb); a.tiles_n = (int)(I / PBN);
  const dim3 grid(a.tiles_m * a.tiles_n), block(512);
  switch (hb) {
    case 320: hipLaunchKernelGGL((gemm_kernel_p10<EPI_SWIGLU_BWD, true, 10, 10>), grid, block, 0, stream, a); break;
    case 288: hipLaunchKernelGGL((gemm_kernel_p10<EPI_SWIGLU_BWD, true, 9, 9>), grid, block, 0, stream, a); break;
    case 272: hipLaunchKernelGGL((gemm_kernel_p10<EPI_SWIGLU_BWD, true, 9, 8>), grid, block, 0, stream, a); break;
    case 256: hipLaunchKernelGGL((gemm_kernel_p10<EPI_SWIGLU_BWD, true, 8, 8>), grid, block, 0, stream, a); break;
    case 224: hipLaunchKernelGGL((gemm_kernel_p10<EPI_SWIGLU_BWD, true, 7, 7>), grid, block, 0, stream, a); break;
    case 208: hipLaunchKernelGGL((gemm_kernel_p10<EPI_SWIGLU_BWD, true, 7, 6>), grid, block, 0, stream, a); break;
    case 192: hipLaunchKernelGGL((gemm_kernel_p10<EPI_SWIGLU_BWD, true, 6, 6>), grid, block, 0, stream, a); break;
    case 160: hipLaunchKernelGGL((gemm_kernel_p10<EPI_SWIGLU_BWD, true, 5, 5>), grid, block, 0, stream, a); break;
    default: hipLaunchKernelGGL((gemm_kernel_p10<EPI_SWIGLU_BWD, true, 4, 4>), grid, block, 0, stream, a); break;
  }
  UG_CHECK_LAUNCH("ug_gemm_bf16_swiglu_bwd");
  return UG_OK;
}
```

ml-unigen_amd/csrc/vmem_asm.h:

```cpp
#pragma once
#include <stdint.h>

template <int N>
__device__ __forceinline__ void wait_vm() { asm volatile("s_waitcnt vmcnt(%0)" ::"n"(N) : "memory"); }
__device__ __forceinline__ void wait_vm_n(int n) {
#define UG_W(v) case v: asm volatile("s_waitcnt vmcnt(" #v ")" ::: "memory"); break;
  switch (n) {
    UG_W(0) UG_W(1) UG_W(2) UG_W(3) UG_W(4) UG_W(6) UG_W(8) UG_W(9) UG_W(12) UG_W(16) UG_W(24) UG_W(32) UG_W(40) UG_W(48)
    default: asm volatile("s_waitcnt vmcnt(0)" ::: "memory"); break;
  }
#undef UG_W
}
__device__ __forceinline__ void dma16_nt(uint64_t base, uint32_t voff, uint32_t lds_addr) {
  asm volatile("s_mov_b32 m0, %2\n\ts_nop 0\n\tglobal_load_lds_dwordx4 %0, %1 nt" ::"v"(voff), "s"(base), "s"(lds_addr) : "memory");
}
__device__ __forceinline__ void dma16(uint64_t base, uint32_t voff, uint32_t lds_addr) {
  asm volatile("s_mov_b32 m0, %2\n\ts_nop 0\n\tglobal_load_lds_dwordx4 %0, %1" ::"v"(voff), "s"(base), "s"(lds_addr) : "memory");
}
__device__ __forceinline__ void dma16_nt(const void* src, uint32_t lds_addr) {
  asm volatile("s_mov_b32 m0, %1\n\ts_nop 0\n\tglobal_load_lds_dwordx4 %0, off nt" ::"v"(src), "s"(lds_addr) : "memory");
}
__device__ __forceinline__ void dma16(const void* src, uint32_t lds_addr) {
  asm volatile("s_mov_b32 m0, %1\n\ts_nop 0\n\tglobal_load_lds_dwordx4 %0, off" ::"v"(src), "s"(lds_addr) : "memory");
}
template <int OFF, typename T>
__device__ __forceinline__ void ld16(T& v, uint64_t base, uint32_t voff) {
  asm volatile("global_load_dwordx4 %0, %1, %2 offset:%3" : "=&v"(v) : "v"(voff), "s"(base), "n"(OFF) : "memory");
}
template <typename T>
__device__ __forceinline__ void ld16(T& v, const void* p) { asm volatile("global_load_dwordx4 %0, %1, off" : "=&v"(v) : "v"(p) : "memory"); }
template <typename T>
__device__ __forceinline__ void ld8(T& v, const void* p) { asm volatile("global_load_dwordx2 %0, %1, off" : "=&v"(v) : "v"(p) : "memory"); }
template <typename T>
__device__ __forceinline__ void ld4(T& v, const void* p) { asm volatile("global_load_dword %0, %1, off" : "=&v"(v) : "v"(p) : "memory"); }
template <typename T>
__device__ __forceinline__ void ld2u(T& v, const void* p) { asm volatile("global_load_ushort %0, %1, off" : "=&v"(v) : "v"(p) : "memory"); }
template <typename T>
__device__ __forceinline__ void tie(T& v) { asm volatile("" : "+v"(v)); }
__device__ __forceinline__ uint32_t lds_addr_of(const void* p) { return (uint32_t)(uintptr_t)p; }
__device__ __forceinline__ void sld4(int& v, const void* p) { asm volatile("s_load_dword %0, %1, 0x0" : "=&s"(v) : "s"(p) : "memory"); }
__device__ __forceinline__ void wait_lgkm0() { asm volatile("s_waitcnt lgkmcnt(0)" ::: "memory"); }
template <typename T>
__device__ __forceinline__ void tie_s(T& v) { asm volatile("" : "+s"(v)); }
```

ml-unigen_amd/unigen_hip/lib.py:

```python
import ctypes
import os
import subprocess

_HERE = os.path.dirname(os.path.abspath(__file__))
CSRC_DIR = os.path.normpath(os.path.join(_HERE, "..", "csrc"))
LIB_PATH = os.environ.get("UNIGEN_HIP_LIB") or os.path.join(CSRC_DIR, "libunigen_hip.so")

ABI_VERSION = 7
P = ctypes.c_void_p
I64 = ctypes.c_int64
I32 = ctypes.c_int
F32 = ctypes.c_float

SIGNATURES = {
    "ug_abi_version": [],
    "ug_create": [P],
    "ug_destroy": [P],
    "ug_gemm_bf16": [P, P, I64, I32, P, I64, I32, P, I64, I64, I64, I64, I32, P, P, I64, I32, P, I32, P],
    "ug_gemm_bf16_qkv_rope": [P, P, I64, P, I64, P, P, I64, I64, I64, I64, P, P, I64, I64, I32, P],
    "ug_gemm_bf16_swiglu_bwd": [P, P, I64, P, I64, P, I64, P, I64, I64, I64, I64, P],
    "ug_gemm_bf16_swiglu": [P, P, I64, P, I64, P, I64, P, I64, I64, I64, I64, P],
    "ug_cast_f32_bf16": [P, P, I64, P],
    "ug_rmsnorm_fwd": [P, P, P, P, I64, I64, F32, I32, P],
    "ug_rmsnorm_bwd": [P, P, P, P, P, P, P, I64, I64, P],
    "ug_rope": [P, P, P, I64, I64, I64, I32, I32, I32, P],
    "ug_swiglu_fwd": [P, P, I64, I64, P],
    "ug_swiglu_bwd": [P, P, P, I64, I64, P],
    "ug_gelu": [P, P, P, I64, P],
    "ug_embed_fwd": [P, P, P, I64, I64, I64, P, P],
    "ug_embed_bwd": [P, P, P, I64, I64, I64, P],
    "ug_embed_bwd_sorted": [P, P, P, P, I64, I64, I64, F32, P],
    "ug_gather_rows_bf16": [P, I64, P, P, I64, I64, I64, I32, P],
    "ug_colsum_bf16": [P, I64, P, I64, I64, P],
    "ug_attn_mask_compress": [P, I32, I64, I64, P, P, I64, I64, P, P],
    "ug_attn_mask_causal": [P, P, P, I64, I64, P],
    "ug_attn_fwd": [P, P, P, I64, P, I64, P, P, P, I64, I64, I64, I32, I32, I32, F32, P],
    "ug_attn_bwd": [P, P, P, I64, P, P, I64, P, P, P, P, P, I64, P, P, I64, I64, I64, I32, I32, I32, F32, P, P, P, P, P],
    "ug_kv_store": [P, I64, I64, I64, P, P, I64, I64, I32, I32, I64, P, I32, P],
    "ug_rope_at": [P, P, P, I64, I64, I32, I32, P, I64, P],
    "ug_attn_decode": [P, I64, P, P, P, P, I64, I64, I32, I32, I32, I64, P, F32, P],
    "ug_gemv_bf16": [P, I64, I64, P, I64, P, I64, I64, I64, I64, P],
    "ug_decode_gemv": [P, I64, I64, P, I64, P, I64, I64, I64, P, I64, P, I64, P, P],
    "ug_decode_gemv_resid_norm": [P, P, I64, P, P, P, I64, P, I64, P, I64, I64, I64, P, I64, P, I64, P, P],
    "ug_decode_gemv_swiglu": [P, I64, P, F32, I64, I64, P, I64, P, I64, I64, I64, P, I64, P, I64, P, P],
    "ug_gemm_set_fused_tile_height": [I32],
    "ug_attn_decode_fused": [P, I64, P, F32, I64, P, P, P, P, P, P, P, P, I64, I64, I32, I32, I32, I64, I64, F32, P],
    "ug_decode_finish_resid_norm": [P, I64, P, P, P, I64, I64, F32, P, P, P],
    "ug_decode_sw_supported": [I64, I64, I64, I32],
    "ug_decode_sw_kblock": [P, I64, I64, P, I64, P, I64, I64, I64, P, I64, P, I64, P, P],
    "ug_decode_sw_resid": [P, I64, I64, P, I64, I64, I64, P, P],
    "ug_decode_sw_gate_up": [P, P, I64, P, P, F32, I64, I64, P, I64, I64, P, I64, P],
    "ug_decode_sw_head": [P, P, I64, P, P, F32, I64, I64, P, I64, I64, P, I64, P, P, P],
    "ug_t2i_assemble": [P, P, P, I64, P, I64, P, P, I64, I64, I64, I64, I64, I64, I64, P, P, P, P],
    "ug_attn_mask_from_ids": [P, I64, I64, I64, I64, I64, I32, P, P, P, P, P],
    "ug_maskgit_train_mask": [P, P, P, I64, I64, I64, I64, P, P, P],
    "ug_ar_sample": [P, I64, I64, I64, F32, F32, I32, P, P, I64, I64, P, I64, I64, I64, P, P, P, P],
    "ug_ar_sample_filtered": [P, I64, I64, I64, F32, F32, I32, P, P, I64, I64, P, I64, I64, I64, P, P, P, I64, F32, F32, P, P],
    "ug_text_pick": [P, I64, I64, I64, I32, P, I64, I64, P, I64, I64, I64, P, I64, P, P, P, P, P],
    "ug_text_sample_workspace_ints": [I64],
    "ug_text_sample": [P, I64, I64, I64, I32, F32, I64, F32, P, P, P, P, I64, I64, P, I64, I64, I64, P, I64, P, P, P, P, P],
    "ug_text_seen_mark": [P, I64, P, I64, I64, I64, P, I64, P],
    "ug_text_penalize": [P, I64, I64, I64, F32, P, I64, P, P],
    "ug_maskgit_step": [P, I64, I64, I64, I64, I32, F32, P, P, P, I64, I64, I64, F32, P, P, P, P, P, P],
    "ug_skinny_finish": [P, P, P, P, I64, I64, I32, P],
    "ug_gemv_bf16_ord": [P, I64, I64, P, I64, P, I64, I64, I64, I64, P],
    "ug_skinny_finish_ord": [P, I64, I64, P, P, P, P, I64, I64, P],
    "ug_decode_gemv_resid_norm_ord": [P, P, I64, I64, P, P, P, I64, P, I64, P, I64, I64, I64, P],
    "ug_attn_decode_fused_ord": [P, I64, I64, P, F32, I64, P, P, P, P, P, P, P, P, I64, I64, I32, I32, I32, I64, I64, F32, P],
    "ug_decode_sw_kblock_ord": [P, I64, I64, P, I64, P, I64, I64, I64, P],
    "ug_decode_finish_resid_norm_ord": [P, I64, I64, P, P, P, I64, I64, F32, P, P, P],
    "ug_ce_fwd": [P, I64, I64, I64, P, I64, P, P, P, P, P],
    "ug_ce_bwd": [P, I64, I64, I64, P, I64, P, P, P, P, P],
    "ug_adamw_flat": [P, P, P, P, P, I64, F32, F32, F32, F32, F32, I64, F32, I32, P],
    "ug_gemm_bf16_wgrad_group": [I32, P, P, P, P, P, P, P, P, P, P, P],
    "ug_grad_pack_bf16": [P, P, I64, F32, P],
    "ug_comm_unique_id": [P],
    "ug_comm_init": [P, I32, I32, P, I64],
    "ug_comm_allreduce_bucket": [P, P, I64, I32, P],
    "ug_comm_allgather": [P, P, P, I64, P],
    "ug_comm_wait": [P, P],
    "ug_comm_destroy": [P],
    "ug_comm_bytes_on_wire": [P],
    "ug_zero_ranges_f32": [P, P, I64, I64, P],
    "ug_grad_unpack_bf16": [P, P, I64, P],
    "ug_grad_sum_shards_bf16": [P, I32, I64, P, I64, F32, P],
    "ug_conv2d_f32": [P, P, P, P, P, I64, I32, I32, I32, I32, I32, I32, I32, I32, I32, I32, I32, I32, P],
    "ug_conv_split_weights": [P, P, I32, I32, I32, P],
    "ug_amax_f32": [P, I64, I64, I64, P, P],
    "ug_amax_f32_into_zeroed": [P, I64, I64, I64, P, P],
    "ug_conv2d_split": [P, P, P, P, P, P, I64, I32, I32, I32, I32, I32, I32, I32, I32, I32, I32, I32, I32, P, I32, P],
    "ug_conv3x3_split": [P, P, P, P, P, P, I64, I32, I32, I32, I32, I32, P, P, P, I32, I32, P, I32, P],
    "ug_groupnorm_finalize": [P, P, I64, I64, I32, I32, F32, P],
    "ug_groupnorm_stats": [P, P, P, I64, I64, I32, I32, F32, P],
    "ug_siglip_attn_f32": [P, I64, P, P, I64, I64, I64, I32, I32, F32, P],
    "ug_linear_split": [P, I64, P, P, P, P, I64, P, I64, I64, I64, I64, I32, I32, P],
    "ug_gemm_f32_nested": [P, I64, I64, I64, P, I64, I64, I64, I32, P, I64, I64, I64, I64, I64, I64, I64, I64, F32, P],
    "ug_gemm_f32": [P, I64, I64, P, I64, I64, I32, P, I64, I64, I64, I64, I64, I64, F32, P],
    "ug_groupnorm_swish": [P, P, P, P, P, I64, I64, I32, I32, F32, I32, P],
    "ug_softmax_rows_f32": [P, I64, I64, I64, F32, P],
    "ug_linear_f32": [P, I64, P, I64, P, P, I64, P, I64, I64, I64, I64, I32, P],
    "ug_layernorm_f32": [P, P, P, P, I64, I64, F32, P],
    "ug_layernorm_bwd_f32": [P, P, P, P, P, P, P, I64, I64, F32, P],
    "ug_gelu_tanh_f32": [P, P, P, I64, P],
    "ug_softmax_bwd_rows_f32": [P, P, I64, I64, I64, F32, P],
    "ug_colsum_f32": [P, I64, P, I64, I64, P],
    "ug_transpose_f32": [P, I64, I64, P, I64, I64, I64, I64, I64, P],
    "ug_nchw_to_nhwc": [P, P, I64, I32, I64, I32, P],
    "ug_nhwc_to_nchw": [P, P, I64, I32, I64, I32, P],
    "ug_lfq_pack": [P, I64, P, I64, I32, P],
    "ug_lfq_unpack": [P, P, I64, I32, P, P],
    "ug_probe_layouts": [P, I64, P],
}

_lib = None

PROFILE = None


def family_of(name):
    if name.startswith("ug_gemm_bf16"):
        return "gemm"
    if name in ("ug_attn_fwd", "ug_attn_bwd"):
        return "attention"
    if name.startswith(("ug_conv", "ug_groupnorm", "ug_amax", "ug_lfq", "ug_nchw", "ug_nhwc", "ug_gemm_f32", "ug_softmax_rows", "ug_linear_",
                        "ug_layernorm", "ug_siglip")):
        return "tokenizer_and_towers"
    if name == "ug_adamw_flat":
        return "adamw"
    return "elementwise"


def _profiled(name, fn):
    fam = family_of(name)

    def call(*args):
        prof = PROFILE
        if prof is None:
            return fn(*args)
        import torch
        e0, e1 = torch.cuda.Event(enable_timing=True), torch.cuda.Event(enable_timing=True)
        sp = args[-1]
        sp = getattr(sp, "value", sp) or 0
        st = torch.cuda.current_stream() if sp == torch.cuda.current_stream().cuda_stream else torch.cuda.ExternalStream(sp)
        e0.record(st)
        rc = fn(*args)
        e1.record(st)
        tag = name
        if name == "ug_gemm_bf16":
            tag = "ug_gemm_bf16[M=%d N=%d K=%d ak=%d bk=%d epi=%d]" % (args[9], args[10], args[11], args[3], args[6], args[12])
        elif name == "ug_conv3x3_split":
            tag = "ug_conv3x3_split[B=%d %dx%d %d->%d gn=%d]" % (args[6], args[7], args[8], args[9], args[10], 1 if args[12] else 0)
        elif name == "ug_gemm_bf16_wgrad_group":
            tag = "ug_gemm_bf16_wgrad_group[%s]" % " ".join("%dx%dx%d" % (args[7][i], args[8][i], args[10][i]) for i in range(args[0]))
        prof.setdefault(fam, []).append((e0, e1, tag))
        return rc
    call.__name__ = name
    return call


class UniGenHipError(RuntimeError):
    pass


def build(verbose=False):
    cmd = ["make", "-C", CSRC_DIR, "-j8"]
    res = subprocess.run(cmd, capture_output=True, text=True)
    if verbose or res.returncode != 0:
        print(res.stdout[-4000:])
        print(res.stderr[-4000:])
    if res.returncode != 0:
        raise UniGenHipError("building libunigen_hip.so failed (see output above)")
    return LIB_PATH


def load():
    global _lib
    if _lib is not None:
        return _lib
    if not os.path.exists(LIB_PATH):
        raise UniGenHipError(
            f"{LIB_PATH} is missing: the HIP extension is the only implementation of this path "
            f"(no CPU fallback). Build it with `make -C {CSRC_DIR}` or `python -c 'import __graft_entry__ as g; g.build()'`.")
    import torch
    lib = ctypes.CDLL(LIB_PATH)
    lib.ug_last_error.restype = ctypes.c_char_p
    lib.ug_last_error.argtypes = []
    for name, argtypes in SIGNATURES.items():
        fn = getattr(lib, name)
        fn.argtypes = argtypes
        fn.restype = ctypes.c_int64 if name == "ug_comm_bytes_on_wire" else ctypes.c_int
        if name.startswith("ug_comm_") or name in ("ug_abi_version", "ug_create", "ug_destroy"):
            continue
        setattr(lib, name, _profiled(name, fn))
    if lib.ug_abi_version() != ABI_VERSION:
        raise UniGenHipError(f"ABI version mismatch: library reports {lib.ug_abi_version()}, binding expects {ABI_VERSION}")
    _lib = lib
    return lib


def check(rc, name="ug call"):
    if rc != 0:
        msg = load().ug_last_error().decode("utf-8", "replace")
        raise UniGenHipError(f"{name} failed (rc={rc}): {msg}")
```

ml-unigen_amd/unigen_hip/ops.py:

```python
import ctypes
import math
import torch

from . import lib as _l

UG_EPI_BF16, UG_EPI_F32, UG_EPI_RESID = 0, 1, 2
_MASK_DTYPES = {torch.float32: 0, torch.bfloat16: 1, torch.int64: 2, torch.bool: 3}


GEMM_PROFILE = None
GEMM_PROFILE_FUSED = None


def _stream():
    return torch.cuda.current_stream().cuda_stream


def _p(t):
    return 0 if t is None else t.data_ptr()


_HANDLES = {}
GEMM_POLICY = -1
UG_GEMM_NARROW_EPILOGUE, UG_GEMM_POLICY_AUTO_BITS = 0x100, 0xff


def _handle():
    s = torch.cuda.current_stream()
    key = (s.device_index, s.cuda_stream)
    h = _HANDLES.get(key)
    if h is None:
        if torch.cuda.is_current_stream_capturing():
            return 0
        out = ctypes.c_void_p()
        _l.check(_l.load().ug_create(ctypes.byref(out)), "ug_create")
        h = _HANDLES[key] = out.value
    return h


def release_handles():
    lib = _l.load()
    for h in _HANDLES.values():
        lib.ug_destroy(h)
    _HANDLES.clear()


def _need_cuda(*ts):
    for t in ts:
        if t is not None and not t.is_cuda:
            raise _l.UniGenHipError("unigen_hip ops need tensors in GPU memory (no CPU fallback exists)")


def round_up(x, m):
    return (x + m - 1) // m * m


def gemm(a, b, out=None, *, M=None, N=None, K=None, a_kmajor=False, b_kmajor=False, epilogue=UG_EPI_BF16,
         bias=None, resid=None, beta=0, alpha_dev=None, out_dtype=None):
    _need_cuda(a, b)
    if M is None:
        M = a.shape[1] if a_kmajor else a.shape[0]
    if N is None:
        N = b.shape[1] if b_kmajor else b.shape[0]
    if K is None:
        K = a.shape[0] if a_kmajor else a.shape[1]
    if out is None:
        dt = out_dtype or (torch.bfloat16 if epilogue == UG_EPI_BF16 else torch.float32)
        out = torch.empty((M, N), dtype=dt, device=a.device)
    lib = _l.load()
    prof = GEMM_PROFILE
    if prof is not None:
        e0, e1 = torch.cuda.Event(enable_timing=True), torch.cuda.Event(enable_timing=True)
        e0.record()
    rc = lib.ug_gemm_bf16(_handle(), _p(a), a.stride(0), int(a_kmajor), _p(b), b.stride(0), int(b_kmajor), _p(out), out.stride(0),
                          M, N, K, epilogue, _p(bias), _p(resid), resid.stride(0) if resid is not None else 0, beta,
                          _p(alpha_dev), GEMM_POLICY, _stream())
    _l.check(rc, "ug_gemm_bf16")
    if prof is not None:
        e1.record()
        prof.append((e0, e1, 2.0 * M * N * K))
    return out


FUSED_SWIGLU = __import__("os").environ.get("UNIGEN_FUSED_SWIGLU", "1") == "1"


def gemm_swiglu(x, w_gate_up):
    _need_cuda(x, w_gate_up)
    if not FUSED_SWIGLU or GEMM_POLICY != -1:
        gu = gemm(x, w_gate_up)
        return gu, swiglu_fwd(gu)
    M, K = x.shape
    I = w_gate_up.shape[0] // 2
    gu = torch.empty((M, 2 * I), dtype=torch.bfloat16, device=x.device)
    act = torch.empty((M, I), dtype=torch.bfloat16, device=x.device)
    prof = GEMM_PROFILE
    if prof is not None:
        e0, e1 = torch.cuda.Event(enable_timing=True), torch.cuda.Event(enable_timing=True)
        e0.record()
    _l.check(_l.load().ug_gemm_bf16_swiglu(_handle(), _p(x), x.stride(0), _p(w_gate_up), w_gate_up.stride(0), _p(gu), gu.stride(0),
                                           _p(act), act.stride(0), M, I, K, _stream()), "ug_gemm_bf16_swiglu")
    if prof is not None:
        e1.record()
        prof.append((e0, e1, 2.0 * M * 2 * I * K))
        if GEMM_PROFILE_FUSED is not None:
            GEMM_PROFILE_FUSED.append(len(prof) - 1)
    return gu, act


WGRAD_GROUP_MIN_TILES = 256


def gemm_wgrad_group(problems):
    tiles = sum(((dy.shape[1] + 255) // 256) * ((x.shape[1] + 255) // 256) for dy, x, _, _ in problems)
    if tiles < WGRAD_GROUP_MIN_TILES or len(problems) > 8 or GEMM_POLICY != -1:
        for dy, x, dw, beta in problems:
            gemm(dy, x, out=dw, a_kmajor=True, b_kmajor=True, epilogue=UG_EPI_F32, beta=beta)
        return
    n = len(problems)
    PA, LA, IA = ctypes.c_void_p * n, ctypes.c_int64 * n, ctypes.c_int * n
    for dy, x, dw, _ in problems:
        _need_cuda(dy, x, dw)
        assert dy.shape[0] == x.shape[0] and dw.shape == (dy.shape[1], x.shape[1])
    prof = GEMM_PROFILE
    if prof is not None:
        e0, e1 = torch.cuda.Event(enable_timing=True), torch.cuda.Event(enable_timing=True)
        e0.record()
    rc = _l.load().ug_gemm_bf16_wgrad_group(
        n, PA(*[_p(dy) for dy, _, _, _ in problems]), LA(*[dy.stride(0) for dy, _, _, _ in problems]),
        PA(*[_p(x) for _, x, _, _ in problems]), LA(*[x.stride(0) for _, x, _, _ in problems]),
        PA(*[_p(dw) for _, _, dw, _ in problems]), LA(*[dw.stride(0) for _, _, dw, _ in problems]),
        LA(*[dy.shape[1] for dy, _, _, _ in problems]), LA(*[x.shape[1] for _, x, _, _ in problems]),
        IA(*[int(b) for _, _, _, b in problems]), LA(*[dy.shape[0] for dy, _, _, _ in problems]), _stream())
    _l.check(rc, "ug_gemm_bf16_wgrad_group")
    if prof is not None:
        e1.record()
        prof.append((e0, e1, sum(2.0 * dy.shape[1] * x.shape[1] * dy.shape[0] for dy, x, _, _ in problems)))


def set_gemm_tile_policy(policy):
    global GEMM_POLICY
    policy = int(policy)
    if policy == 100:
        GEMM_POLICY = UG_GEMM_POLICY_AUTO_BITS | UG_GEMM_NARROW_EPILOGUE
    elif policy == 101:
        GEMM_POLICY = -1
    elif policy in (102, 104):
        GEMM_POLICY = UG_GEMM_POLICY_AUTO_BITS | (0x200 if policy == 102 else 0x400)
    elif policy in (103, 105):
        GEMM_POLICY = 3 | (0x200 if policy == 103 else 0x400)
    else:
        GEMM_POLICY = policy


def set_fused_tile_height(rows):
    _l.check(_l.load().ug_gemm_set_fused_tile_height(int(rows)), "ug_gemm_set_fused_tile_height")


def gemm_nt(a, b, out=None, **kw):
    return gemm(a, b, out, **kw)


def cast_bf16(x, out=None):
    _need_cuda(x)
    if out is None:
        out = torch.empty(x.shape, dtype=torch.bfloat16, device=x.device)
    _l.check(_l.load().ug_cast_f32_bf16(_p(x), _p(out), x.numel(), _stream()), "ug_cast_f32_bf16")
    return out


def zero_ranges_(buf, ranges, max_len):
    _l.check(_l.load().ug_zero_ranges_f32(_p(buf), _p(ranges), ranges.shape[0], int(max_len), _stream()), "ug_zero_ranges_f32")
    return buf


def grad_pack_bf16(g, out, scale):
    _need_cuda(g, out)
    _l.check(_l.load().ug_grad_pack_bf16(_p(g), _p(out), g.numel(), float(scale), _stream()), "ug_grad_pack_bf16")


def grad_unpack_bf16(src, g):
    _need_cuda(src, g)
    _l.check(_l.load().ug_grad_unpack_bf16(_p(src), _p(g), g.numel(), _stream()), "ug_grad_unpack_bf16")


def grad_sum_shards_bf16(shards, world, stride, out, scale):
    _need_cuda(shards, out)
    _l.check(_l.load().ug_grad_sum_shards_bf16(_p(shards), int(world), int(stride), _p(out), out.numel(), float(scale), _stream()),
             "ug_grad_sum_shards_bf16")


def rmsnorm_fwd(x, w, eps, out_f32=False, want_rstd=True, out=None):
    _need_cuda(x, w)
    rows, cols = x.shape
    y = out if out is not None else torch.empty((rows, cols), dtype=torch.float32 if out_f32 else torch.bfloat16, device=x.device)
    rstd = torch.empty((rows,), dtype=torch.float32, device=x.device) if want_rstd else None
    _l.check(_l.load().ug_rmsnorm_fwd(_p(x), _p(w), _p(y), _p(rstd), rows, cols, eps, int(out_f32), _stream()),
             "ug_rmsnorm_fwd")
    return y, rstd


def rmsnorm_bwd(dy, x, rstd, w, dres, dw, want_bf16=False):
    rows, cols = x.shape
    out = torch.empty((rows, cols), dtype=torch.bfloat16, device=x.device) if want_bf16 else None
    _l.check(_l.load().ug_rmsnorm_bwd(_p(dy), _p(x), _p(rstd), _p(w), _p(dres), _p(dw), _p(out), rows, cols, _stream()),
             "ug_rmsnorm_bwd")
    return out


def rope_inv_freq(head_dim, theta, scaling=None, seq_len=None):
    base = float(theta)
    kind = (scaling or {}).get("rope_type", (scaling or {}).get("type", "default"))
    factor = float((scaling or {}).get("factor", 1.0))
    if kind == "dynamic":
        max_pos = int((scaling or {}).get("max_position_embeddings", 32768))
        sl = torch.tensor(max(int(seq_len or 0), max_pos))
        base = base * ((factor * sl / max_pos) - (factor - 1)) ** (head_dim / (head_dim - 2))
    elif kind not in ("default", "linear"):
        raise _l.UniGenHipError(f"rope_type {kind!r} is not implemented (default, linear and dynamic are)")
    inv_freq = 1.0 / (base ** (torch.arange(0, head_dim, 2, dtype=torch.float) / head_dim))
    if kind == "linear":
        inv_freq = inv_freq / factor
    return inv_freq


def rope_tables(L, head_dim, theta, device, scaling=None):
    inv_freq = rope_inv_freq(head_dim, theta, scaling, L)
    pos = torch.arange(L, dtype=torch.float)
    freqs = (inv_freq[None, :, None] @ pos[None, None, :]).transpose(1, 2)[0]
    return freqs.cos().contiguous().to(device), freqs.sin().contiguous().to(device)


def rope_(qkv, cos, sin, L, nheads, head_dim, backward=False):
    tokens = qkv.shape[0]
    _l.check(_l.load().ug_rope(_p(qkv), _p(cos), _p(sin), tokens, L, qkv.stride(0), nheads, head_dim,
                               int(backward), _stream()), "ug_rope")
    return qkv


def gemm_qkv_rope(x, w, bias, cos, sin, L, nheads, head_dim):
    _need_cuda(x, w)
    M, K = x.shape
    N = w.shape[0]
    if GEMM_POLICY != -1:
        qkv = gemm(x, w, bias=bias)
        return rope_(qkv, cos, sin, L, nheads, head_dim)
    qkv = torch.empty((M, N), dtype=torch.bfloat16, device=x.device)
    prof = GEMM_PROFILE
    if prof is not None:
        e0, e1 = torch.cuda.Event(enable_timing=True), torch.cuda.Event(enable_timing=True)
        e0.record()
    _l.check(_l.load().ug_gemm_bf16_qkv_rope(_handle(), _p(x), x.stride(0), _p(w), w.stride(0), _p(bias), _p(qkv), qkv.stride(0), M, N, K,
                                              _p(cos), _p(sin), L, nheads * head_dim, head_dim, _stream()), "ug_gemm_bf16_qkv_rope")
    if prof is not None:
        e1.record()
        prof.append((e0, e1, 2.0 * M * N * K))
        if GEMM_PROFILE_FUSED is not None:
            GEMM_PROFILE_FUSED.append(len(prof) - 1)
    return qkv


def swiglu_fwd(gu):
    tokens, two_i = gu.shape
    act = torch.empty((tokens, two_i // 2), dtype=torch.bfloat16, device=gu.device)
    _l.check(_l.load().ug_swiglu_fwd(_p(gu), _p(act), tokens, two_i // 2, _stream()), "ug_swiglu_fwd")
    return act


FUSED_SWIGLU_BWD = __import__("os").environ.get("UNIGEN_FUSED_SWIGLU_BWD", "1") == "1"


def gemm_swiglu_bwd(dy, w_down, gu):
    _need_cuda(dy, w_down, gu)
    M, K = dy.shape
    I = gu.shape[1] // 2
    ok = (FUSED_SWIGLU_BWD and GEMM_POLICY == -1 and I % 256 == 0 and K % 32 == 0 and w_down.shape == (K, I)
          and dy.stride(0) % 8 == 0 and w_down.stride(0) % 8 == 0 and gu.stride(0) % 8 == 0)
    if not ok:
        return swiglu_bwd(gu, gemm(dy, w_down, b_kmajor=True))
    dgu = torch.empty_like(gu)
    prof = GEMM_PROFILE
    if prof is not None:
        e0, e1 = torch.cuda.Event(enable_timing=True), torch.cuda.Event(enable_timing=True)
        e0.record()
    _l.check(_l.load().ug_gemm_bf16_swiglu_bwd(_handle(), _p(dy), dy.stride(0), _p(w_down), w_down.stride(0), _p(gu), gu.stride(0),
                                                _p(dgu), dgu.stride(0), M, I, K, _stream()), "ug_gemm_bf16_swiglu_bwd")
    if prof is not None:
        e1.record()
        prof.append((e0, e1, 2.0 * M * I * K))
        if GEMM_PROFILE_FUSED is not None:
            GEMM_PROFILE_FUSED.append(len(prof) - 1)
    return dgu


def swiglu_bwd(gu, dact):
    dgu = torch.empty_like(gu)
    _l.check(_l.load().ug_swiglu_bwd(_p(gu), _p(dact), _p(dgu), gu.shape[0], gu.shape[1] // 2, _stream()),
             "ug_swiglu_bwd")
    return dgu


def embed_fwd(ids, W, err_flag=None):
    tokens = ids.numel()
    V, H = W.shape
    out = torch.empty((tokens, H), dtype=torch.float32, device=W.device)
    _l.check(_l.load().ug_embed_fwd(_p(ids), _p(W), _p(out), tokens, H, V, _p(err_flag), _stream()), "ug_embed_fwd")
    return out


def embed_bwd(ids, dout, dW):
    V, H = dW.shape
    _l.check(_l.load().ug_embed_bwd(_p(ids), _p(dout), _p(dW), ids.numel(), H, V, _stream()), "ug_embed_bwd")


def embed_bwd_sorted(ids_sorted, order, rows, dW, scale):
    V, H = dW.shape
    _l.check(_l.load().ug_embed_bwd_sorted(_p(ids_sorted), _p(order), _p(rows), _p(dW), ids_sorted.numel(), H, V, float(scale), _stream()),
             "ug_embed_bwd_sorted")


def gather_rows(x, idx):
    n, C = idx.numel(), x.shape[1]
    out = torch.empty((n, C), dtype=torch.bfloat16, device=x.device)
    _l.check(_l.load().ug_gather_rows_bf16(_p(x), x.stride(0), _p(idx), _p(out), C, n, C, 0, _stream()), "ug_gather_rows_bf16")
    return out


def scatter_rows_(src, idx, out):
    n, C = idx.numel(), src.shape[1]
    _l.check(_l.load().ug_gather_rows_bf16(_p(src), src.stride(0), _p(idx), _p(out), out.stride(0), n, C, 1, _stream()),
             "ug_gather_rows_bf16")
    return out


def colsum_(x, out, R=None, C=None):
    R = x.shape[0] if R is None else R
    C = x.shape[1] if C is None else C
    _l.check(_l.load().ug_colsum_bf16(_p(x), x.stride(0), _p(out), R, C, _stream()), "ug_colsum_bf16")


class MaskBits:

    def __init__(self, bits, tileany, B, L):
        self.bits, self.tileany, self.B, self.L = bits, tileany, B, L
        self.nW = (L + 63) // 64
        self.Lp = self.nW * 64


def _alloc_mask(B, L, device):
    nW = (L + 63) // 64
    bits = torch.empty((B, L, nW), dtype=torch.int64, device=device)
    tileany = torch.empty((B, nW, nW), dtype=torch.uint8, device=device)
    return bits, tileany


def mask_compress(mask4d, err_flag=None):
    _need_cuda(mask4d)
    if mask4d.dim() == 4:
        if mask4d.shape[1] != 1:
            raise _l.UniGenHipError("per-head attention masks are not part of the reference path")
        m = mask4d[:, 0]
    else:
        m = mask4d
    B, L, L2 = m.shape
    if L != L2 or m.stride(2) != 1:
        raise _l.UniGenHipError(f"attention mask must be [B,1,L,L] with contiguous rows, got {tuple(mask4d.shape)}")
    if m.dtype not in _MASK_DTYPES:
        raise _l.UniGenHipError(f"unsupported attention-mask dtype {m.dtype}")
    bits, tileany = _alloc_mask(B, L, m.device)
    _l.check(_l.load().ug_attn_mask_compress(_p(m), _MASK_DTYPES[m.dtype], m.stride(0), m.stride(1), _p(bits),
                                             _p(tileany), B, L, _p(err_flag), _stream()), "ug_attn_mask_compress")
    return MaskBits(bits, tileany, B, L)


def mask_causal(B, L, device, key_valid=None):
    bits, tileany = _alloc_mask(B, L, device)
    kv = None if key_valid is None else key_valid.to(torch.uint8).contiguous()
    _l.check(_l.load().ug_attn_mask_causal(_p(kv), _p(bits), _p(tileany), B, L, _stream()), "ug_attn_mask_causal")
    return MaskBits(bits, tileany, B, L)


MASK_T2I, MASK_LM, MASK_MMU = 0, 1, 2


def mask_from_ids(ids, pad_id, soi_id, eoi_id, mode=MASK_T2I):
    _need_cuda(ids)
    B, L = ids.shape
    ids = ids.to(torch.int64).contiguous()
    bits, tileany = _alloc_mask(B, L, ids.device)
    meta = torch.empty((B, 4), dtype=torch.int32, device=ids.device)
    flags = torch.empty((B, L), dtype=torch.uint8, device=ids.device)
    _l.check(_l.load().ug_attn_mask_from_ids(_p(ids), B, L, int(pad_id), int(soi_id), int(eoi_id), int(mode), _p(meta), _p(flags),
                                             _p(bits), _p(tileany), _stream()), "ug_attn_mask_from_ids")
    return MaskBits(bits, tileany, B, L)


def t2i_assemble(text_ids, image_in, image_labels, max_seq_len, pad_id, soi_id, eoi_id, conv_start, conv_end, ignore_id=-100):
    dev = image_in.device
    if isinstance(text_ids, tuple):
        flat, offs = text_ids
    else:
        offs = [0]
        for t in text_ids:
            offs.append(offs[-1] + len(t))
        flat = torch.tensor([v for t in text_ids for v in t] or [0], dtype=torch.int64)
        offs = torch.tensor(offs, dtype=torch.int64)
    flat, offs = flat.to(dev), offs.to(dev)
    as_dev = lambda v: v.to(device=dev, dtype=torch.int64) if torch.is_tensor(v) else torch.as_tensor(list(v), dtype=torch.int64).to(dev)
    cs, ce = as_dev(conv_start), as_dev(conv_end)
    B, n = image_in.shape
    ids = torch.empty((B, max_seq_len), dtype=torch.int64, device=dev)
    labels = torch.empty_like(ids)
    attn = torch.empty((B, max_seq_len), dtype=torch.uint8, device=dev)
    _l.check(_l.load().ug_t2i_assemble(_p(flat), _p(offs), _p(cs), cs.numel(), _p(ce), ce.numel(), _p(image_in.to(torch.int64).contiguous()),
                                       _p(image_labels.to(torch.int64).contiguous()), B, n, max_seq_len, int(pad_id), int(soi_id),
                                       int(eoi_id), int(ignore_id), _p(ids), _p(labels), _p(attn), _stream()), "ug_t2i_assemble")
    return ids, attn, labels


def attn_fwd(qkv, mb, H, HKV, hd, scale=None, out=None):
    B, L, Lp = mb.B, mb.L, mb.Lp
    scale = 1.0 / math.sqrt(hd) if scale is None else scale
    q = qkv[:, : H * hd]
    k = qkv[:, H * hd: (H + HKV) * hd]
    v = qkv[:, (H + HKV) * hd:]
    if out is not None:
        o, lse = out
    else:
        o = torch.empty((B * L, H * hd), dtype=torch.bfloat16, device=qkv.device)
        lse = torch.empty((B, H, L), dtype=torch.float32, device=qkv.device)
    _l.check(_l.load().ug_attn_fwd(_p(q), _p(k), _p(v), qkv.stride(0), _p(o), o.stride(0), _p(lse), _p(mb.bits),
                                   _p(mb.tileany), B, L, Lp, H, HKV, hd, scale, _stream()), "ug_attn_fwd")
    return o, lse


_DKV_WS = {}


def _dkv_workspace(tokens, width, device):
    key = (device, tokens, width)
    if key not in _DKV_WS:
        _DKV_WS.clear()
        _DKV_WS[key] = torch.zeros((tokens, width), dtype=torch.float32, device=device)
    return _DKV_WS[key]


def attn_bwd(qkv, o, lse, dout, mb, H, HKV, hd, scale=None, split_heads=True, rope=None, dbias=None, out=None):
    B, L, Lp = mb.B, mb.L, mb.Lp
    scale = 1.0 / math.sqrt(hd) if scale is None else scale
    q = qkv[:, : H * hd]
    k = qkv[:, H * hd: (H + HKV) * hd]
    v = qkv[:, (H + HKV) * hd:]
    dqkv = torch.empty_like(qkv) if out is None else out
    dq = dqkv[:, : H * hd]
    dk = dqkv[:, H * hd: (H + HKV) * hd]
    dv = dqkv[:, (H + HKV) * hd:]
    delta = torch.empty((B, H, L), dtype=torch.float32, device=qkv.device)
    ws = _dkv_workspace(B * L, 2 * HKV * hd, qkv.device) if split_heads and H > HKV else None
    _l.check(_l.load().ug_attn_bwd(_p(q), _p(k), _p(v), qkv.stride(0), _p(o), _p(dout), o.stride(0),
                                   _p(lse), _p(delta), _p(dq), _p(dk), _p(dv), dqkv.stride(0), _p(mb.bits),
                                   _p(mb.tileany), B, L, Lp, H, HKV, hd, scale, _p(ws), _p(rope[0] if rope else None),
                                   _p(rope[1] if rope else None), _p(dbias), _stream()), "ug_attn_bwd")
    return dqkv


def kv_store(qkv, cache_k, cache_v, rows, L, H, HKV, hd, Tmax, pos_dev=None, pos_host=0):
    _l.check(_l.load().ug_kv_store(_p(qkv), qkv.stride(0), H * hd, (H + HKV) * hd, _p(cache_k), _p(cache_v), rows, L, HKV, hd,
                                   Tmax, _p(pos_dev), pos_host, _stream()), "ug_kv_store")


def rope_at_(qkv, cos, sin, nheads, hd, pos_dev):
    _l.check(_l.load().ug_rope_at(_p(qkv), _p(cos), _p(sin), qkv.shape[0], qkv.stride(0), nheads, hd, _p(pos_dev),
                                  cos.shape[0], _stream()), "ug_rope_at")
    return qkv


def attn_decode(qkv, cache_k, cache_v, key_valid, H, HKV, hd, Tmax, len_dev, scale=None, out=None):
    rows = qkv.shape[0]
    scale = 1.0 / math.sqrt(hd) if scale is None else scale
    o = out if out is not None else torch.empty((rows, H * hd), dtype=torch.bfloat16, device=qkv.device)
    _l.check(_l.load().ug_attn_decode(_p(qkv), qkv.stride(0), _p(cache_k), _p(cache_v), _p(key_valid), _p(o), o.stride(0),
                                      rows, H, HKV, hd, Tmax, _p(len_dev), scale, _stream()), "ug_attn_decode")
    return o


def skinny_linear(x, w, bias=None, resid=None):
    M, N = x.shape[0], w.shape[0]
    acc = torch.zeros((M, N), dtype=torch.float32, device=x.device)
    K = w.shape[1]
    if M <= 32 and K % 32 == 0:
        _l.check(_l.load().ug_gemv_bf16(_p(x), x.stride(0), M, _p(w), w.stride(0), _p(acc), N, 1, N, K, _stream()), "ug_gemv_bf16")
    else:
        gemm(x, w, out=acc, epilogue=UG_EPI_F32, beta=1)
    out = None if resid is not None else torch.empty((M, N), dtype=torch.bfloat16, device=x.device)
    _l.check(_l.load().ug_skinny_finish(_p(acc), _p(bias), _p(out), _p(resid), M, N, 0 if resid is None else 1, _stream()),
             "ug_skinny_finish")
    return resid if resid is not None else out


def gemv_acc_(x, w, acc):
    M, N, K = x.shape[0], w.shape[0], w.shape[1]
    _l.check(_l.load().ug_gemv_bf16(_p(x), x.stride(0), M, _p(w), w.stride(0), _p(acc), acc.stride(0), 1, N, K, _stream()),
             "ug_gemv_bf16")
    return acc


def decode_finish_resid_norm_(acc, x, w, xn, eps, advance=None):
    pos, ln = advance if advance is not None else (None, None)
    _l.check(_l.load().ug_decode_finish_resid_norm(_p(acc), acc.stride(0), _p(x), _p(w), _p(xn), x.shape[0], x.shape[1], eps,
                                                   _p(pos), _p(ln), _stream()), "ug_decode_finish_resid_norm")
    return xn


def _clr(t):
    return (_p(t), t.numel()) if t is not None else (None, 0)


def decode_gemv_(x, w, acc, zero0=None, zero1=None, ss_zero=None):
    _l.check(_l.load().ug_decode_gemv(_p(x), x.stride(0), x.shape[0], _p(w), w.stride(0), _p(acc), acc.stride(0), w.shape[0],
                                      w.shape[1], *_clr(zero0), *_clr(zero1), _p(ss_zero), _stream()), "ug_decode_gemv")
    return acc


def decode_gemv_resid_norm_(x_in, pending, norm_w, x_out, ss_out, w, acc, zero0=None, zero1=None, ss_zero=None):
    _l.check(_l.load().ug_decode_gemv_resid_norm(_p(x_in), _p(pending), pending.stride(0), _p(norm_w), _p(x_out), _p(ss_out),
                                                 x_in.shape[0], _p(w), w.stride(0), _p(acc), acc.stride(0), w.shape[0],
                                                 w.shape[1], *_clr(zero0), *_clr(zero1), _p(ss_zero), _stream()),
             "ug_decode_gemv_resid_norm")
    return acc


def decode_gemv_swiglu_(gu_acc, ss_in, eps, norm_cols, w, acc, zero0=None, zero1=None, ss_zero=None):
    _l.check(_l.load().ug_decode_gemv_swiglu(_p(gu_acc), gu_acc.stride(0), _p(ss_in), eps, norm_cols, gu_acc.shape[0], _p(w),
                                             w.stride(0), _p(acc), acc.stride(0), w.shape[0], w.shape[1], *_clr(zero0),
                                             *_clr(zero1), _p(ss_zero), _stream()), "ug_decode_gemv_swiglu")
    return acc


def decode_sw_supported(hidden, inter, q_dim, head_dim):
    return bool(_l.load().ug_decode_sw_supported(int(hidden), int(inter), int(q_dim), int(head_dim)))


def decode_sw_resid_(x, w, h):
    _l.check(_l.load().ug_decode_sw_resid(_p(x), x.stride(0), x.shape[0], _p(w), w.stride(0), w.shape[0], w.shape[1], _p(h), _stream()),
             "ug_decode_sw_resid")
    return h


def decode_sw_kblock_(x, w, acc, zero0=None, zero1=None, ss_zero=None):
    _l.check(_l.load().ug_decode_sw_kblock(_p(x), x.stride(0), x.shape[0], _p(w), w.stride(0), _p(acc), acc.stride(0), w.shape[0],
                                           w.shape[1], *_clr(zero0), *_clr(zero1), _p(ss_zero), _stream()), "ug_decode_sw_kblock")
    return acc


def decode_sw_gate_up_(h, norm_w, eps, w, act, pend=None, x_out=None):
    _l.check(_l.load().ug_decode_sw_gate_up(_p(h), _p(pend), pend.stride(0) if pend is not None else 0, _p(x_out), _p(norm_w), eps,
                                            h.shape[0], h.shape[1], _p(w), w.stride(0), w.shape[0] // 2, _p(act), act.stride(0), _stream()),
             "ug_decode_sw_gate_up")
    return act


def decode_sw_head_(h, norm_w, eps, w, logits, pend=None, x_out=None, advance=None):
    pos, ln = advance if advance is not None else (None, None)
    _l.check(_l.load().ug_decode_sw_head(_p(h), _p(pend), pend.stride(0) if pend is not None else 0, _p(x_out), _p(norm_w), eps,
                                         h.shape[0], h.shape[1], _p(w), w.stride(0), w.shape[0], _p(logits), logits.stride(0),
                                         _p(pos), _p(ln), _stream()), "ug_decode_sw_head")
    return logits


def attn_decode_fused(acc_qkv, ss_in, eps, norm_cols, bias, cos, sin, pos_dev, cache_k, cache_v, key_valid, out, H, HKV, hd, Tmax,
                      scale=None):
    scale = 1.0 / math.sqrt(hd) if scale is None else scale
    _l.check(_l.load().ug_attn_decode_fused(_p(acc_qkv), acc_qkv.stride(0), _p(ss_in), eps, norm_cols, _p(bias), _p(cos), _p(sin),
                                            _p(pos_dev), _p(cache_k), _p(cache_v), _p(key_valid), _p(out), out.stride(0),
                                            acc_qkv.shape[0], H, HKV, hd, Tmax, cos.shape[0], scale, _stream()),
             "ug_attn_decode_fused")
    return out


ORD_QKV_SLABS = 6
ORD_DOWN_KBLOCKS = 5
ORD_ROW_BLOCK = 32


def ord_slices(K):
    return (K + 255) // 256


def skinny_linear_ord(x, w, bias=None, resid=None, out_f32=None):
    M, N, K = x.shape[0], w.shape[0], w.shape[1]
    if K % 32:
        raise _l.UniGenHipError(f"skinny_linear_ord: K={K} must be a multiple of 32")
    S = ord_slices(K)
    parts = torch.empty((S, M, N), dtype=torch.float32, device=x.device)
    L = _l.load()
    for r0 in range(0, M, ORD_ROW_BLOCK):
        r1 = min(M, r0 + ORD_ROW_BLOCK)
        _l.check(L.ug_gemv_bf16_ord(_p(x[r0:r1]), x.stride(0), r1 - r0, _p(w), w.stride(0), _p(parts[:, r0:r1]), N, M * N, N, K, _stream()),
                 "ug_gemv_bf16_ord")
    out = None
    if resid is None and out_f32 is None:
        out = torch.empty((M, N), dtype=torch.bfloat16, device=x.device)
    _l.check(L.ug_skinny_finish_ord(_p(parts), S, M * N, _p(bias), _p(out), _p(out_f32), _p(resid), M, N, _stream()), "ug_skinny_finish_ord")
    return out if out is not None else (resid if resid is not None else out_f32)


def decode_gemv_resid_norm_ord_(x_in, pend_parts, norm_w, x_out, ss_part, w, part):
    npend = 0 if pend_parts is None else pend_parts.shape[0]
    _l.check(_l.load().ug_decode_gemv_resid_norm_ord(_p(x_in), _p(pend_parts), pend_parts.stride(1) if npend else 0, npend, _p(norm_w), _p(x_out),
                                                     _p(ss_part), x_in.shape[0], _p(w), w.stride(0), _p(part), part.stride(1), w.shape[0],
                                                     w.shape[1], _stream()), "ug_decode_gemv_resid_norm_ord")
    return part


def attn_decode_fused_ord(qkv_part, ss_part, eps, norm_cols, bias, cos, sin, pos_dev, cache_k, cache_v, key_valid, out, H, HKV, hd, Tmax,
                          scale=None):
    scale = 1.0 / math.sqrt(hd) if scale is None else scale
    _l.check(_l.load().ug_attn_decode_fused_ord(_p(qkv_part), qkv_part.stride(1), qkv_part.shape[0], _p(ss_part), eps, norm_cols, _p(bias),
                                                _p(cos), _p(sin), _p(pos_dev), _p(cache_k), _p(cache_v), _p(key_valid), _p(out),
                                                out.stride(0), qkv_part.shape[1], H, HKV, hd, Tmax, cos.shape[0], scale, _stream()),
             "ug_attn_decode_fused_ord")
    return out


def decode_sw_kblock_ord_(x, w, part):
    _l.check(_l.load().ug_decode_sw_kblock_ord(_p(x), x.stride(0), x.shape[0], _p(w), w.stride(0), _p(part), part.stride(1), w.shape[0],
                                               w.shape[1], _stream()), "ug_decode_sw_kblock_ord")
    return part


def decode_finish_resid_norm_ord_(parts, x, w, xn, eps, advance=None):
    pos, ln = advance if advance is not None else (None, None)
    _l.check(_l.load().ug_decode_finish_resid_norm_ord(_p(parts), parts.stride(1), parts.shape[0], _p(x), _p(w), _p(xn), x.shape[0], x.shape[1],
                                                       eps, _p(pos), _p(ln), _stream()), "ug_decode_finish_resid_norm_ord")
    return xn


def maskgit_step(logits, N, n, cfg, guidance_scale, u_sample, u_conf, cur_ids, mask_id, id_offset, mask_len_sched, temperature,
                 want_masking=False):
    V = logits.shape[-1]
    logits = logits.reshape(-1, V)
    if logits.dtype != torch.bfloat16 or logits.stride(1) != 1:
        raise _l.UniGenHipError("maskgit_step: logits must be bf16 with contiguous rows")
    dev = logits.device
    sampled = torch.empty((N, n), dtype=torch.int64, device=dev)
    next_cur, next_ids = torch.empty_like(sampled), torch.empty_like(sampled)
    sel = torch.empty((N, n), dtype=torch.float32, device=dev)
    masking = torch.empty((N, n), dtype=torch.uint8, device=dev) if want_masking else None
    cur_ids = cur_ids.to(torch.int64).contiguous()
    _l.check(_l.load().ug_maskgit_step(_p(logits), logits.stride(0), V, N, n, int(bool(cfg)), float(guidance_scale),
                                       _p(u_sample.contiguous()), _p(u_conf.contiguous()), _p(cur_ids), int(mask_id),
                                       int(id_offset), int(mask_len_sched), float(temperature), _p(sampled), _p(sel), _p(next_cur),
                                       _p(next_ids), _p(masking), _stream()), "ug_maskgit_step")
    return (sampled, next_cur, next_ids, masking.bool()) if want_masking else (sampled, next_cur, next_ids)


def maskgit_train_mask(tokens, scores, num_masked, mask_id, ignore_id=-100):
    _need_cuda(tokens, scores, num_masked)
    B, n = tokens.shape
    tokens = tokens.to(torch.int64).contiguous()
    ids, labels = torch.empty_like(tokens), torch.empty_like(tokens)
    _l.check(_l.load().ug_maskgit_train_mask(_p(tokens), _p(scores.float().contiguous()), _p(num_masked.float().contiguous()), B, n,
                                             int(mask_id), int(ignore_id), _p(ids), _p(labels), _stream()), "ug_maskgit_train_mask")
    return ids, labels


def ar_sample_(acc, bsz, V, guidance_scale, temperature, greedy, uniforms, pos_dev, pos0, nsteps, embed_master, id_offset, tok,
               out_tokens, x):
    _l.check(_l.load().ug_ar_sample(_p(acc), acc.stride(0), bsz, V, float(guidance_scale), float(temperature), int(bool(greedy)),
                                    _p(uniforms), _p(pos_dev), int(pos0), int(nsteps), _p(embed_master), embed_master.stride(0),
                                    embed_master.shape[1], int(id_offset), _p(tok), _p(out_tokens), _p(x), _stream()),
             "ug_ar_sample")


def ar_sample_filtered_(acc, bsz, V, guidance_scale, temperature, greedy, uniforms, pos_dev, pos0, nsteps, embed_master, id_offset, tok,
                        out_tokens, x, top_k=0, top_p=1.0, min_p=0.0, stats=None):
    _l.check(_l.load().ug_ar_sample_filtered(_p(acc), acc.stride(0), bsz, V, float(guidance_scale), float(temperature), int(bool(greedy)),
                                             _p(uniforms), _p(pos_dev), int(pos0), int(nsteps), _p(embed_master),
                                             embed_master.stride(0), embed_master.shape[1], int(id_offset), _p(tok), _p(out_tokens),
                                             _p(x), int(top_k), float(top_p), float(min_p), _p(stats), _stream()),
             "ug_ar_sample_filtered")


TEXT_MAX_ROWS, TEXT_MAX_STOP = 32, 8
TEXT_STATE_INTS = 4 + TEXT_MAX_ROWS


def text_state(rows, device):
    return text_state_reset_(torch.empty(TEXT_STATE_INTS, dtype=torch.int32, device=device), rows)


def text_state_reset_(state, rows):
    state.zero_()
    state[1:2].fill_(int(rows))
    return state


def text_sample_workspace(rows, device):
    n = _l.load().ug_text_sample_workspace_ints(int(rows))
    if n <= 0:
        _l.check(n, "ug_text_sample_workspace_ints")
    return torch.zeros(n, dtype=torch.int32, device=device)


def _text_out(stop_ids, pad_id, embed_master):
    return (_p(stop_ids), 0 if stop_ids is None else stop_ids.numel(), -1 if pad_id is None else int(pad_id), _p(embed_master),
            embed_master.stride(0), embed_master.shape[0], embed_master.shape[1])


def text_pick_(logits, V, state, nsteps, embed_master, tok, out_tokens, x, clear=False, stop_ids=None, pad_id=None, lengths=None):
    _need_cuda(logits, state, embed_master, tok, out_tokens, x)
    _l.check(_l.load().ug_text_pick(_p(logits), logits.stride(0), logits.shape[0], int(V), int(bool(clear)), *_text_out(stop_ids, pad_id, embed_master),
                                    _p(state), int(nsteps), _p(tok), _p(out_tokens), _p(lengths), _p(x), _stream()), "ug_text_pick")


def text_sample_(logits, V, state, nsteps, embed_master, tok, out_tokens, x, uniforms, workspace, temperature=1.0, top_k=0, top_p=1.0,
                 clear=False, stop_ids=None, pad_id=None, lengths=None, stats=None):
    _need_cuda(logits, state, embed_master, tok, out_tokens, x, uniforms, workspace)
    _l.check(_l.load().ug_text_sample(_p(logits), logits.stride(0), logits.shape[0], int(V), int(bool(clear)), float(temperature), int(top_k),
                                      float(top_p), _p(uniforms), _p(workspace), _p(stats), *_text_out(stop_ids, pad_id, embed_master),
                                      _p(state), int(nsteps), _p(tok), _p(out_tokens), _p(lengths), _p(x), _stream()), "ug_text_sample")


def text_seen(rows, V, device):
    return torch.zeros((int(rows), (int(V) + 31) // 32), dtype=torch.int32, device=device)


def text_seen_mark_(seen, ids, V, valid=None):
    ids = ids.long()
    if ids.stride(1) != 1:
        ids = ids.contiguous()
    if valid is not None:
        valid = valid.to(torch.uint8).contiguous()
        if tuple(valid.shape) != tuple(ids.shape):
            raise _l.UniGenHipError(f"text_seen_mark_: valid {tuple(valid.shape)} against ids {tuple(ids.shape)}")
    _need_cuda(seen, ids)
    if seen.shape[0] != ids.shape[0] or seen.stride(1) != 1:
        raise _l.UniGenHipError(f"text_seen_mark_: seen {tuple(seen.shape)} against ids {tuple(ids.shape)}")
    _l.check(_l.load().ug_text_seen_mark(_p(seen), seen.stride(0), _p(ids), ids.stride(0), ids.shape[0], ids.shape[1], _p(valid), int(V),
                                         _stream()), "ug_text_seen_mark")
    return seen


def text_penalize_(logits, V, penalty, seen, tok=None):
    _need_cuda(logits, seen)
    if seen.shape[0] != logits.shape[0] or seen.stride(1) != 1 or logits.stride(1) != 1:
        raise _l.UniGenHipError(f"text_penalize_: seen {tuple(seen.shape)} against logits {tuple(logits.shape)}")
    _l.check(_l.load().ug_text_penalize(_p(logits), logits.stride(0), logits.shape[0], int(V), float(penalty), _p(seen), seen.stride(0),
                                        _p(tok), _stream()), "ug_text_penalize")


def ce_fwd(logits, V, labels, ignore_index=-100, want_logp=False):
    R, ld = logits.shape[0], logits.stride(0)
    dev = logits.device
    lse = torch.empty((R,), dtype=torch.float32, device=dev)
    loss_row = torch.empty((R,), dtype=torch.float32, device=dev)
    logp = torch.empty((R,), dtype=torch.float32, device=dev) if want_logp else None
    lc = torch.empty((2,), dtype=torch.float32, device=dev)
    _l.check(_l.load().ug_ce_fwd(_p(logits), ld, R, V, _p(labels), ignore_index, _p(lse), _p(loss_row), _p(logp),
                                 _p(lc), _stream()), "ug_ce_fwd")
    return lc, lse, loss_row, logp


def ce_bwd_(logits, V, labels, lse, lc, gscale=None, ignore_index=-100, row_scale=None):
    R, ld = logits.shape[0], logits.stride(0)
    _l.check(_l.load().ug_ce_bwd(_p(logits), ld, R, V, _p(labels), ignore_index, _p(lse), _p(lc), _p(gscale),
                                 _p(row_scale), _stream()), "ug_ce_bwd")
    return logits


BF16_MIRRORS = []


def register_bf16_mirror(owner):
    import weakref
    BF16_MIRRORS.append(weakref.ref(owner))


def find_bf16_mirror(ptr, numel):
    for ref in list(BF16_MIRRORS):
        o = ref()
        if o is None:
            BF16_MIRRORS.remove(ref)
            continue
        base = o.master.data_ptr()
        if base <= ptr and ptr + 4 * numel <= base + 4 * o.master.numel():
            return o, o.bf16.data_ptr() + (ptr - base) // 2
    return None, 0


def adamw_flat_(p, g, m, v, p_bf16, lr, beta1, beta2, eps, wd, step, grad_scale=1.0, max_blocks=0):
    _l.check(_l.load().ug_adamw_flat(_p(p), _p(g), _p(m), _p(v), _p(p_bf16), p.numel(), lr, beta1, beta2, eps, wd,
                                     step, grad_scale, max_blocks, _stream()), "ug_adamw_flat")


def pack_conv_weight(w):
    cout, cin, kh, kw = w.shape
    cout_pad = round_up(cout, 128) if cout > 32 else 32
    wp = torch.zeros((kh * kw, cin, cout_pad), dtype=torch.float32, device=w.device)
    wp[:, :, :cout] = w.detach().float().permute(2, 3, 1, 0).reshape(kh * kw, cin, cout)
    return wp.contiguous(), cout_pad


def conv_split_eligible(cin, cout, cout_pad):
    return cin % 32 == 0 and cout % 4 == 0 and cout_pad % 128 == 0 and cout >= 64


def split_conv_weight(wp):
    taps, cin, cout_pad = wp.shape
    ws = torch.empty(2 * taps * round_up(cin, 32) * cout_pad + 8, dtype=torch.float16, device=wp.device)
    _l.check(_l.load().ug_conv_split_weights(_p(wp), _p(ws), taps, cin, cout_pad, _stream()), "ug_conv_split_weights")
    return ws


_AMAX_CONST = {}


def amax_const(value, device):
    key = (float(value), str(device))
    if key not in _AMAX_CONST:
        _AMAX_CONST[key] = torch.full((1,), float(value), dtype=torch.float32, device=device)
    return _AMAX_CONST[key]


def amax(x2d):
    _need_cuda(x2d)
    if x2d.dim() == 2 and x2d.stride(1) == 1:
        rows, cols, ld = x2d.shape[0], x2d.shape[1], x2d.stride(0)
    else:
        x2d = x2d.contiguous()
        rows, cols, ld = 1, x2d.numel(), x2d.numel()
    if torch.cuda.is_current_stream_capturing():
        out = torch.empty(1, dtype=torch.float32, device=x2d.device)
        _l.check(_l.load().ug_amax_f32(_p(x2d), rows, cols, ld, _p(out), _stream()), "ug_amax_f32")
        return out
    out = _amax_slot(x2d.device)
    _l.check(_l.load().ug_amax_f32_into_zeroed(_p(x2d), rows, cols, ld, _p(out), _stream()), "ug_amax_f32")
    return out


_AMAX_POOL = {}


def _amax_slot(device):
    key = (str(device), torch.cuda.current_stream(device).cuda_stream)
    pool = _AMAX_POOL.get(key)
    if pool is None or pool[1] >= pool[0].numel():
        pool = [torch.zeros(1024, dtype=torch.float32, device=device), 0]
        _AMAX_POOL[key] = pool
    i = pool[1]
    pool[1] = i + 1
    return pool[0][i:i + 1]


def conv2d_nhwc(x, wp, cout_pad, bias, cout, ksize, *, stride=1, pad=None, residual=None, upsample=False,
                asym_pad=False, w_split=None, x_amax=None, out_stats=None, out_groups=32):
    B, H, W, Cin = x.shape
    He, We = (2 * H, 2 * W) if upsample else (H, W)
    if asym_pad:
        pt = pl = 0
        Ho, Wo = (He + 1 - ksize) // stride + 1, (We + 1 - ksize) // stride + 1
    else:
        pt = pl = (ksize // 2) if pad is None else pad
        Ho, Wo = (He + 2 * pt - ksize) // stride + 1, (We + 2 * pl - ksize) // stride + 1
    y = torch.empty((B, Ho, Wo, cout), dtype=torch.float32, device=x.device)
    if w_split is not None:
        if x_amax is None:
            x_amax = amax(x.view(-1, Cin))
        if out_stats is not None and (out_stats.dtype != torch.float64 or out_stats.numel() != B * out_groups * 2 + 1):
            raise _l.UniGenHipError("conv2d_nhwc: out_stats must be a zeroed fp64 buffer of B * groups * 2 + 1 elements (gn_stats_slots)")
        _l.check(_l.load().ug_conv2d_split(_p(x), _p(x_amax), _p(w_split), _p(bias), _p(residual), _p(y), B, H, W, Cin, cout,
                                           cout_pad, ksize, stride, pt, pl, Ho, Wo, int(upsample), _p(out_stats),
                                           int(out_groups) if out_stats is not None else 0, _stream()), "ug_conv2d_split")
        return y
    if out_stats is not None:
        raise _l.UniGenHipError("conv2d_nhwc: out_stats needs the split path (w_split)")
    _l.check(_l.load().ug_conv2d_f32(_p(x), _p(wp), _p(bias), _p(residual), _p(y), B, H, W, Cin, cout, cout_pad, ksize,
                                     stride, pt, pl, Ho, Wo, int(upsample), _stream()), "ug_conv2d_f32")
    return y


def gemm_f32(a, b, *, b_is_nk, M, N, K, batch=1, lda=None, ldb=None, stride_a=0, stride_b=0, alpha=1.0, out=None,
             ldc=None, stride_c=None):
    if out is None:
        out = torch.empty((batch, M, N), dtype=torch.float32, device=a.device)
    ldc = N if ldc is None else ldc
    stride_c = M * N if stride_c is None else stride_c
    _l.check(_l.load().ug_gemm_f32(_p(a), lda, stride_a, _p(b), ldb, stride_b, int(b_is_nk), _p(out), ldc, stride_c, M, N,
                                   K, batch, alpha, _stream()), "ug_gemm_f32")
    return out


def gemm_f32_nested(a, b, out, *, b_is_nk, M, N, K, batch_in, batch_out, lda, ldb, ldc, sa, sb, sc, alpha=1.0):
    _l.check(_l.load().ug_gemm_f32_nested(_p(a), lda, sa[0], sa[1], _p(b), ldb, sb[0], sb[1], int(b_is_nk), _p(out), ldc,
                                          sc[0], sc[1], M, N, K, batch_in, batch_out, alpha, _stream()), "ug_gemm_f32_nested")
    return out


def groupnorm_swish(x, gamma, beta, *, groups=32, eps=1e-6, swish=True):
    B, H, W, C = x.shape
    y = torch.empty_like(x)
    ws = torch.empty((B, groups, 2), dtype=torch.float64, device=x.device)
    _l.check(_l.load().ug_groupnorm_swish(_p(x), _p(gamma), _p(beta), _p(y), _p(ws), B, H * W, C, groups, eps,
                                          int(swish), _stream()), "ug_groupnorm_swish")
    return y


def groupnorm_stats(x, *, groups=32, eps=1e-6):
    B, H, W, C = x.shape
    ws = torch.empty((B, groups, 2), dtype=torch.float64, device=x.device)
    mr = torch.empty((B, groups, 2), dtype=torch.float32, device=x.device)
    _l.check(_l.load().ug_groupnorm_stats(_p(x), _p(ws), _p(mr), B, H * W, C, groups, eps, _stream()),
             "ug_groupnorm_stats")
    return mr


def gn_out_bound(gamma_absmax, beta_absmax, group_elems):
    b = float(gamma_absmax) * math.sqrt(max(float(group_elems) - 1.0, 1.0)) + float(beta_absmax)
    return 2.0 ** math.ceil(math.log2(max(b, 1e-30)))


def gn_stats_slots(n, B, device, groups=32):
    per = B * groups * 2 + 1
    pool = torch.zeros(n * per, dtype=torch.float64, device=device)
    return [pool[i * per:(i + 1) * per] for i in range(n)]


def stats_amax(stats):
    return stats[-1:].view(torch.float32)[:1]


def groupnorm_finalize(stats, B, HW, C, *, groups=32, eps=1e-6):
    if stats.numel() != B * groups * 2 + 1:
        raise _l.UniGenHipError("groupnorm_finalize: stats buffer does not match B x groups")
    mr = torch.empty((B, groups, 2), dtype=torch.float32, device=stats.device)
    _l.check(_l.load().ug_groupnorm_finalize(_p(stats), _p(mr), B, HW, C, groups, eps, _stream()), "ug_groupnorm_finalize")
    return mr


def conv3x3_nhwc(x, w_split, cout_pad, bias, cout, *, residual=None, gn=None, x_amax=None, gn_bound=None, out_stats=None,
                 out_groups=32):
    B, H, W, Cin = x.shape
    y = torch.empty((B, H, W, cout), dtype=torch.float32, device=x.device)
    mr, ga, be, groups, swish = gn if gn is not None else (None, None, None, 0, 0)
    if x_amax is None:
        if gn is not None and gn_bound is None:
            raise _l.UniGenHipError("conv3x3_nhwc: GroupNorm on the load path needs gn_bound (ops.gn_out_bound of the layer's gamma / beta)")
        x_amax = amax_const(gn_bound, x.device) if gn is not None else amax(x.view(-1, Cin))
    if out_stats is not None and (out_stats.dtype != torch.float64 or out_stats.numel() != B * out_groups * 2 + 1):
        raise _l.UniGenHipError("conv3x3_nhwc: out_stats must be a zeroed fp64 buffer of B * groups * 2 + 1 elements (gn_stats_slots)")
    _l.check(_l.load().ug_conv3x3_split(_p(x), _p(x_amax), _p(w_split), _p(bias), _p(residual), _p(y), B, H, W, Cin, cout,
                                        cout_pad, _p(mr), _p(ga), _p(be), groups, int(swish), _p(out_stats),
                                        int(out_groups) if out_stats is not None else 0, _stream()), "ug_conv3x3_split")
    return y


def softmax_rows_(x2d, scale, cols=None):
    cols = x2d.shape[1] if cols is None else cols
    _l.check(_l.load().ug_softmax_rows_f32(_p(x2d), x2d.shape[0], cols, x2d.stride(0), scale, _stream()),
             "ug_softmax_rows_f32")
    return x2d


def linear_f32(x, W, bias=None, residual=None, act=0, out=None, M=None):
    M = x.shape[0] if M is None else M
    N, K = W.shape
    if out is None:
        out = torch.empty((M, N), dtype=torch.float32, device=x.device)
    _l.check(_l.load().ug_linear_f32(_p(x), x.stride(0), _p(W), W.stride(0), _p(bias), _p(residual),
                                     residual.stride(0) if residual is not None else 0, _p(out), out.stride(0), M, N, K, act,
                                     _stream()), "ug_linear_f32")
    return out


def split_linear_weight(W):
    N, K = W.shape
    n_pad = round_up(N, 128)
    wp = torch.zeros((1, K, n_pad), dtype=torch.float32, device=W.device)
    wp[0, :, :N] = W.detach().float().t()
    return split_conv_weight(wp), n_pad


def linear_split(x, w_split, n_pad, N, bias=None, residual=None, act=0, out=None, M=None, x_amax=None):
    M = x.shape[0] if M is None else M
    K = x.shape[1]
    if out is None:
        out = torch.empty((M, N), dtype=torch.float32, device=x.device)
    if x_amax is None:
        x_amax = amax(x[:M])
    _l.check(_l.load().ug_linear_split(_p(x), x.stride(0), _p(x_amax), _p(w_split), _p(bias), _p(residual),
                                       residual.stride(0) if residual is not None else 0, _p(out), out.stride(0), M, N, K,
                                       n_pad, act, _stream()), "ug_linear_split")
    return out


def siglip_attn(qkv, out, B, T, H, hd, scale, qkv_amax=None):
    _need_cuda(qkv, out)
    if qkv_amax is None:
        qkv_amax = amax(qkv[:B * T])
    _l.check(_l.load().ug_siglip_attn_f32(_p(qkv), qkv.stride(0), _p(qkv_amax), _p(out), out.stride(0), B, T, H, hd, float(scale),
                                          _stream()), "ug_siglip_attn_f32")
    return out


def layernorm_f32(x2d, gamma, beta, eps):
    y = torch.empty_like(x2d)
    _l.check(_l.load().ug_layernorm_f32(_p(x2d), _p(gamma), _p(beta), _p(y), x2d.shape[0], x2d.shape[1], eps, _stream()),
             "ug_layernorm_f32")
    return y


def layernorm_bwd_f32(dy, x, gamma, eps, dgamma, dbeta, dres_in=None):
    dx = torch.empty_like(x)
    _l.check(_l.load().ug_layernorm_bwd_f32(_p(dy), _p(x), _p(gamma), _p(dres_in), _p(dx), _p(dgamma), _p(dbeta), x.shape[0], x.shape[1],
                                            eps, _stream()), "ug_layernorm_bwd_f32")
    return dx


def gelu_tanh_f32(pre, dy=None):
    out = torch.empty_like(pre)
    _l.check(_l.load().ug_gelu_tanh_f32(_p(pre), _p(dy), _p(out), pre.numel(), _stream()), "ug_gelu_tanh_f32")
    return out


def softmax_bwd_rows_(P2d, dP2d, scale, cols):
    _l.check(_l.load().ug_softmax_bwd_rows_f32(_p(P2d), _p(dP2d), P2d.shape[0], cols, P2d.stride(0), scale, _stream()),
             "ug_softmax_bwd_rows_f32")
    return dP2d


def colsum_f32_(x2d, out):
    _l.check(_l.load().ug_colsum_f32(_p(x2d), x2d.stride(0), _p(out), x2d.shape[0], x2d.shape[1], _stream()), "ug_colsum_f32")
    return out


def transpose_f32(x, rows=None, cols=None, *, batch=1, ld_in=None, stride_in=0, pad_to=4, out=None):
    rows = x.shape[-2] if rows is None else rows
    cols = x.shape[-1] if cols is None else cols
    ld_in = x.stride(-2) if ld_in is None else ld_in
    ld_out = round_up(rows, pad_to)
    if out is None:
        out = torch.empty((batch, cols, ld_out), dtype=torch.float32, device=x.device)
    _l.check(_l.load().ug_transpose_f32(_p(x), ld_in, stride_in, _p(out), ld_out, cols * ld_out, rows, cols, batch, _stream()),
             "ug_transpose_f32")
    return out


def nchw_to_nhwc(x, c_pad):
    B, C, H, W = x.shape
    out = torch.empty((B, H, W, c_pad), dtype=torch.float32, device=x.device)
    _l.check(_l.load().ug_nchw_to_nhwc(_p(x), _p(out), B, C, H * W, c_pad, _stream()), "ug_nchw_to_nhwc")
    return out


def nhwc_to_nchw(x, C):
    B, H, W, Cp = x.shape
    out = torch.empty((B, C, H, W), dtype=torch.float32, device=x.device)
    _l.check(_l.load().ug_nhwc_to_nchw(_p(x), _p(out), B, C, H * W, Cp, _stream()), "ug_nhwc_to_nchw")
    return out


def lfq_pack(z2d, nbits):
    n = z2d.shape[0]
    idx = torch.empty((n,), dtype=torch.int64, device=z2d.device)
    _l.check(_l.load().ug_lfq_pack(_p(z2d), z2d.stride(0), _p(idx), n, nbits, _stream()), "ug_lfq_pack")
    return idx


def lfq_unpack(idx, nbits, err_flag=None):
    n = idx.numel()
    z = torch.empty((n, nbits), dtype=torch.float32, device=idx.device)
    _l.check(_l.load().ug_lfq_unpack(_p(idx), _p(z), n, nbits, _p(err_flag), _stream()), "ug_lfq_unpack")
    return z


def probe_layouts(device):
    out = torch.zeros((512,), dtype=torch.float32, device=device)
    _l.check(_l.load().ug_probe_layouts(_p(out), 512, _stream()), "ug_probe_layouts")
    return out


def gelu(x, dy=None):
    out = torch.empty_like(x)
    _l.check(_l.load().ug_gelu(_p(x), _p(dy), _p(out), x.numel(), _stream()), "ug_gelu")
    return out
```

Measured before the change: 132.8.

## Use scalar base plus 32-bit lane offsets for GEMM tile DMA addressing

Replaces per-lane 64-bit source pointers in the GEMM stagers with a wave-uniform 64-bit base in scalar registers plus 32-bit per-lane offsets, advancing the base once per k-step. The default path is chosen when offsets fit in 32 bits, and a wide fallback handles the rest. The k-loop is also unrolled by four with compile-time ring-buffer slots, so LDS stage addresses become constants. This is meant to cut VGPR pressure and per-issue address arithmetic, at the cost of more template instantiations and a new runtime addressing-mode switch.

After: 133.7, median of 6. No clear change (+0.7%).

```diff
diff --git a/include/unigen_hip.h b/include/unigen_hip.h
--- a/include/unigen_hip.h
+++ b/include/unigen_hip.h
@@ -33,6 +33,7 @@
 int ug_gemm_bf16_swiglu_bwd(const ug_handle* h, const void* dy, int64_t ld_dy, const void* w_down, int64_t ldw, const void* gu,
                             int64_t ld_gu, void* dgu, int64_t ld_dgu, int64_t M, int64_t I, int64_t K, hipStream_t stream);
 int ug_gemm_set_fused_tile_height(int rows);
+int ug_gemm_set_addressing(int mode);
 int ug_gemm_bf16_qkv_rope(const ug_handle* h, const void* x, int64_t ldx, const void* w, int64_t ldw, const void* bias, void* qkv,
                           int64_t ldq, int64_t M, int64_t N, int64_t K, const float* cos_tab, const float* sin_tab, int64_t L,
                           int64_t rope_cols, int head_dim, hipStream_t stream);
diff --git a/ml-unigen_amd/csrc/gemm_bf16.hip b/ml-unigen_amd/csrc/gemm_bf16.hip
--- a/ml-unigen_amd/csrc/gemm_bf16.hip
+++ b/ml-unigen_amd/csrc/gemm_bf16.hip
@@ -469,13 +469,43 @@
 
 __device__ __forceinline__ int swz_rowk32(int row, int chunk) { return chunk ^ ((0 - (row >> 2)) & 3); }
 
-template <bool KMAJOR>
+constexpr int SH_ROWK = 2, SH_KROW = 5;
+template <bool WIDE, int SH>
+__device__ __forceinline__ uint32_t lane_off(uint32_t row, uint32_t chunk, uint64_t ld2) {
+  return WIDE ? (row << SH | chunk) : (uint32_t)((uint64_t)row * ld2 + chunk * 16);
+}
+__device__ __forceinline__ uint64_t uniform64(uint64_t v) {
+  const uint32_t lo = __builtin_amdgcn_readfirstlane((uint32_t)v), hi = __builtin_amdgcn_readfirstlane((uint32_t)(v >> 32));
+  return ((uint64_t)hi << 32) | lo;
+}
+template <bool WIDE, int SH>
+__device__ __forceinline__ void dma_tile16(uint64_t base, uint32_t off, uint64_t ld2, uint32_t lds_addr) {
+  static_assert(CPOL_STAGER == 0 && CPOL_P10A == 0, "dma16 issues the default cache policy");
+  if constexpr (WIDE) dma16(reinterpret_cast<const void*>(base + (uint64_t)(off >> SH) * ld2 + (off & ((1u << SH) - 1)) * 16), lds_addr);
+  else dma16(base, off, lds_addr);
+}
+
+template <bool KMAJOR, bool WIDE>
 struct Stager32 {
-  const bf16_t* src[2];
-  int64_t step[2];
-  int kofs[2];
-  __device__ __forceinline__ void init(const bf16_t* X, int64_t ld, int row0, int rows_total, int wave, int lane, int split_rows = 0) {
-    const bf16_t* zero = reinterpret_cast<const bf16_t*>(g_zero_page);
+  uint64_t base;
+  uint64_t adv;
+  uint64_t ld2;
+  uint32_t off[2];
+  static constexpr int SH = KMAJOR ? SH_KROW : SH_ROWK;
+  static __device__ __forceinline__ int kofs(int i, int wave, int lane) {
+    const int inst = i * 8 + wave;
+    if constexpr (!KMAJOR) return swz_rowk32(inst * 16 + (lane >> 2), lane & 3) * 8;
+    else return inst * 2 + (lane >> 5);
+  }
+  __device__ __forceinline__ void init(const bf16_t* X, int64_t ld, int row0, int rows_total, int kt0, int wave, int lane, int split_rows = 0) {
+    ld2 = uniform64((uint64_t)ld * 2);
+    if constexpr (!KMAJOR) {
+      adv = PBK * 2;
+      base = uniform64(reinterpret_cast<uint64_t>(X) + ((uint64_t)row0 * (uint64_t)ld + (uint64_t)kt0 * PBK) * 2);
+    } else {
+      adv = uniform64((uint64_t)ld * (PBK * 2));
+      base = uniform64(reinterpret_cast<uint64_t>(X) + ((uint64_t)kt0 * PBK * (uint64_t)ld + (uint64_t)row0) * 2);
+    }
 #pragma unroll
     for (int i = 0; i < 2; ++i) {
       const int inst = i * 8 + wave;
@@ -484,34 +514,30 @@
         const int chunk = swz_rowk32(row, lane & 3);
         const int grow = (split_rows > 0 && row >= 128) ? split_rows + row0 + row - 128 : row0 + row;
         const int r = min(grow, rows_total - 1);
-        src[i] = X + (int64_t)r * ld + chunk * 8;
-        step[i] = PBK;
-        kofs[i] = chunk * 8;
+        off[i] = lane_off<WIDE, SH>(r - row0, chunk, ld2);
       } else {
         const int k = inst * 2 + (lane >> 5);
         const int chunk = swz_krow(k, lane & 31);
-        const int col = row0 + chunk * 8;
-        const bool ok = (col + 8 <= ld);
-        src[i] = ok ? X + (int64_t)k * ld + col : zero;
-        step[i] = ok ? (int64_t)PBK * ld : 0;
-        kofs[i] = k;
+        const bool ok = (row0 + chunk * 8 + 8 <= ld);
+        off[i] = lane_off<WIDE, SH>(k, ok ? chunk : 0, ld2);
       }
     }
   }
   template <bool CHECK>
-  __device__ __forceinline__ void issue(int kt, int K, char* lds_tile, int wave) const {
-    const bf16_t* zero = reinterpret_cast<const bf16_t*>(g_zero_page);
+  __device__ __forceinline__ void issue(int kt, int K, uint32_t lds_tile, int wave, int lane) {
 #pragma unroll
     for (int i = 0; i < 2; ++i) {
-      const bf16_t* s = src[i] + kt * step[i];
+      const uint32_t dst = lds_tile + (i * 8 + wave) * 1024;
       if constexpr (CHECK) {
-        const bool past = kt * PBK + kofs[i] >= (KMAJOR ? K : ((K + 7) & ~7));
-        s = reinterpret_cast<const bf16_t*>(past ? reinterpret_cast<uintptr_t>(zero) : reinterpret_cast<uintptr_t>(s));
-      }
-      char* dst = lds_tile + (i * 8 + wave) * 1024;
-      static_assert(CPOL_STAGER == 0, "dma16 issues the default cache policy");
-      dma16(s, __builtin_amdgcn_readfirstlane(lds_addr_of(dst)));
-    }
+        const bool past = kt * PBK + kofs(i, wave, lane) >= (KMAJOR ? K : ((K + 7) & ~7));
+        const uint64_t lo = WIDE ? (uint64_t)(off[i] >> SH) * ld2 + (off[i] & ((1u << SH) - 1)) * 16 : (uint64_t)off[i];
+        const uint64_t s = past ? reinterpret_cast<uint64_t>(g_zero_page) : base + lo;
+        dma16(reinterpret_cast<const void*>(s), dst);
+      } else {
+        dma_tile16<WIDE, SH>(base, off[i], ld2, dst);
+      }
+    }
+    base += adv;
   }
 };
 
@@ -541,7 +567,14 @@
     acc[i][j] = __builtin_amdgcn_mfma_f32_16x16x32_bf16(fb[j], fa[i], acc[i][j], 0, 0, 0);                                  \
     __builtin_amdgcn_sched_barrier(0); }
 
-template <int EPI, bool AK, bool BKM, bool ONEBAR>
+template <int S> using SlotC = std::integral_constant<int, S>;
+using SlotDyn = std::integral_constant<int, -1>;
+template <int S>
+__device__ __forceinline__ int ring_slot(std::integral_constant<int, S>, int t) { return S >= 0 ? (S & (P_NST - 1)) : (t & (P_NST - 1)); }
+template <int S, int D>
+using slot_plus = std::integral_constant<int, S >= 0 ? ((S + D) & (P_NST - 1)) : -1>;
+
+template <int EPI, bool AK, bool BKM, bool ONEBAR, bool WIDE>
 __device__ __forceinline__ void p8_body(const GemmArgs& p, const int bid, char* lds) {
   const int tid = threadIdx.x, lane = tid & 63;
   const int wave = __builtin_amdgcn_readfirstlane(tid >> 6);
@@ -559,46 +592,50 @@
   const int tn = (pid % per_group) / gsz;
   const int m0 = tm * PBM, n0 = tn * PBN;
 
-  Stager32<AK> sa; Stager32<BKM> sb;
-  sa.init(p.A, p.lda, m0, p.M, wave, lane);
-  sb.init(p.B, p.ldb, n0, p.N, wave, lane);
-
-  f32x4_t acc[8][4];
-#pragma unroll
-  for (int i = 0; i < 8; ++i)
-#pragma unroll
-    for (int j = 0; j < 4; ++j) acc[i][j] = f32x4_t{0.f, 0.f, 0.f, 0.f};
-
   const int nk_all = (p.K + PBK - 1) / PBK;
   const int per_split = tail ? (nk_all + p.tail_split - 1) / p.tail_split : nk_all;
   const int kt0 = tail ? (tail_j % p.tail_split) * per_split : 0;
   const int nk = min(nk_all, kt0 + per_split) - kt0;
   if (nk <= 0) return;
+
+  Stager32<AK, WIDE> sa; Stager32<BKM, WIDE> sb;
+  sa.init(p.A, p.lda, m0, p.M, kt0, wave, lane);
+  sb.init(p.B, p.ldb, n0, p.N, kt0, wave, lane);
+
+  f32x4_t acc[8][4];
+#pragma unroll
+  for (int i = 0; i < 8; ++i)
+#pragma unroll
+    for (int j = 0; j < 4; ++j) acc[i][j] = f32x4_t{0.f, 0.f, 0.f, 0.f};
+
   const bool ragged = (p.K % PBK) != 0;
-  auto stage_in = [&](int lt) {
+  const uint32_t lds0 = lds_addr_of(lds);
+  auto stage_in = [&](int lt, auto slot) {
     const int kt = kt0 + lt;
-    char* st = lds + (lt & (P_NST - 1)) * P_STAGE;
-    if (ragged && kt + 1 == nk_all) { sa.template issue<true>(kt, p.K, st, wave); sb.template issue<true>(kt, p.K, st + P_TILE, wave); }
-    else { sa.template issue<false>(kt, p.K, st, wave); sb.template issue<false>(kt, p.K, st + P_TILE, wave); }
+    const uint32_t st = lds0 + ring_slot(slot, lt) * P_STAGE;
+    if (ragged && kt + 1 == nk_all) { sa.template issue<true>(kt, p.K, st, wave, lane); sb.template issue<true>(kt, p.K, st + P_TILE, wave, lane); }
+    else { sa.template issue<false>(kt, p.K, st, wave, lane); sb.template issue<false>(kt, p.K, st + P_TILE, wave, lane); }
   };
-  auto stage_whole = [&](int lt) {
-    char* st = lds + (lt & (P_NST - 1)) * P_STAGE;
-    sa.template issue<false>(kt0 + lt, p.K, st, wave);
-    sb.template issue<false>(kt0 + lt, p.K, st + P_TILE, wave);
+  auto stage_whole = [&](int lt, auto slot) {
+    const uint32_t st = lds0 + ring_slot(slot, lt) * P_STAGE;
+    sa.template issue<false>(kt0 + lt, p.K, st, wave, lane);
+    sb.template issue<false>(kt0 + lt, p.K, st + P_TILE, wave, lane);
   };
   const int nk_steady = max(nk - 4, 0);
   bf16x8_t fa[8], fb[4];
-  auto read_frags = [&](int t) {
-    const char* tA = lds + (t & (P_NST - 1)) * P_STAGE;
+  auto read_frags = [&](int t, auto slot) {
+    const char* tA = lds + ring_slot(slot, t) * P_STAGE;
     const char* tB = tA + P_TILE;
-#pragma unroll
-    for (int i = 0; i < 8; ++i) fa[i] = load_frag32<AK>(tA, grp * 128 + i * 16, lane);
-#pragma unroll
-    for (int j = 0; j < 4; ++j) fb[j] = load_frag32<BKM>(tB, wn * 64 + j * 16, lane);
+    const int ln = (!WIDE && decltype(slot)::value < 0) ? (int)__builtin_amdgcn_mbcnt_hi(~0u, __builtin_amdgcn_mbcnt_lo(~0u, 0u)) : lane;
+#pragma unroll
+    for (int i = 0; i < 8; ++i) fa[i] = load_frag32<AK>(tA, grp * 128 + i * 16, ln);
+#pragma unroll
+    for (int j = 0; j < 4; ++j) fb[j] = load_frag32<BKM>(tB, wn * 64 + j * 16, ln);
   };
-  auto request = [&](int t, auto steady) {
-    if constexpr (decltype(steady)::value) stage_whole(t + 3);
-    else if (t + 3 < nk) stage_in(t + 3);
+  auto request = [&](int t, auto slot, auto steady) {
+    constexpr int S = decltype(slot)::value;
+    if constexpr (decltype(steady)::value) stage_whole(t + 3, slot_plus<S, 3>{});
+    else if (t + 3 < nk) stage_in(t + 3, slot_plus<S, 3>{});
   };
   auto landed = [&](int t, auto steady) {
     if constexpr (decltype(steady)::value) asm volatile("s_waitcnt vmcnt(8)" ::: "memory");
@@ -615,61 +652,67 @@
   };
   const std::true_type STEADY{};
   const std::false_type CHECKED{};
-  stage_in(0);
-  if (nk > 1) stage_in(1);
-  if (nk > 2) stage_in(2);
+  const SlotDyn DYN{};
+  auto k_loop = [&](auto first, auto&& body) {
+    constexpr int FIRST = decltype(first)::value;
+    int t = FIRST;
+    if constexpr (!WIDE) {
+      for (; t + 4 <= nk_steady; t += 4) {
+        body(t, SlotC<FIRST>{}, STEADY);
+        body(t + 1, SlotC<FIRST + 1>{}, STEADY);
+        body(t + 2, SlotC<FIRST + 2>{}, STEADY);
+        body(t + 3, SlotC<FIRST + 3>{}, STEADY);
+      }
+    }
+    for (; t < nk_steady; ++t) body(t, DYN, STEADY);
+    for (; t < nk; ++t) body(t, DYN, CHECKED);
+  };
+  stage_in(0, SlotC<0>{});
+  if (nk > 1) stage_in(1, SlotC<1>{});
+  if (nk > 2) stage_in(2, SlotC<2>{});
   if (nk > 2) asm volatile("s_waitcnt vmcnt(8)" ::: "memory");
   else if (nk > 1) asm volatile("s_waitcnt vmcnt(4)" ::: "memory");
   else asm volatile("s_waitcnt vmcnt(0)" ::: "memory");
   if constexpr (ONEBAR) {
     if (grp == 0) {
-      auto interval = [&](int t, auto steady) {
+      k_loop(SlotC<0>{}, [&](int t, auto slot, auto steady) {
         P_BARRIER();
-        read_frags(t);
-        request(t, steady);
+        read_frags(t, slot);
+        request(t, slot, steady);
         asm volatile("s_waitcnt lgkmcnt(0)" ::: "memory");
         mfmas(1);
         landed(t, steady);
-      };
-      int t = 0;
-      for (; t < nk_steady; ++t) interval(t, STEADY);
-      for (; t < nk; ++t) interval(t, CHECKED);
+      });
       P_BARRIER();
     } else {
       P_BARRIER();
-      read_frags(0);
-      request(0, CHECKED);
+      read_frags(0, SlotC<0>{});
+      request(0, SlotC<0>{}, CHECKED);
       landed(0, CHECKED);
       asm volatile("s_waitcnt lgkmcnt(0)" ::: "memory");
-      auto interval = [&](int t, auto steady) {
+      k_loop(SlotC<1>{}, [&](int t, auto slot, auto steady) {
         P_BARRIER();
         mfmas(2);
-        read_frags(t);
-        request(t, steady);
+        read_frags(t, slot);
+        request(t, slot, steady);
         asm volatile("s_waitcnt lgkmcnt(0)" ::: "memory");
         landed(t, steady);
-      };
-      int t = 1;
-      for (; t < nk_steady; ++t) interval(t, STEADY);
-      for (; t < nk; ++t) interval(t, CHECKED);
+      });
       P_BARRIER();
       mfmas(2);
     }
   } else {
     P_BARRIER();
     if (grp == 1) P_BARRIER();
-    auto iteration = [&](int t, auto steady) {
-      read_frags(t);
-      request(t, steady);
+    k_loop(SlotC<0>{}, [&](int t, auto slot, auto steady) {
+      read_frags(t, slot);
+      request(t, slot, steady);
       landed(t, steady);
       asm volatile("s_waitcnt lgkmcnt(0)" ::: "memory");
       P_BARRIER();
       mfmas(1);
       P_BARRIER();
-    };
-    int t = 0;
-    for (; t < nk_steady; ++t) iteration(t, STEADY);
-    for (; t < nk; ++t) iteration(t, CHECKED);
+    });
     if (grp == 0) P_BARRIER();
   }
 
@@ -704,10 +747,10 @@
   store_tile<EPI>(p, reinterpret_cast<f32x4_t (&)[4][4]>(acc[4]), m0 + grp * 128 + 64, n0 + wn * 64, lane, false);
 }
 
-template <int EPI, bool AK, bool BKM, bool ONEBAR = false>
+template <int EPI, bool AK, bool BKM, bool ONEBAR, bool WIDE>
 __global__ __launch_bounds__(512, 2) void gemm_kernel_p8(GemmArgs p) {
   __shared__ __attribute__((aligned(16))) char lds[P_NST * P_STAGE];
-  p8_body<EPI, AK, BKM, ONEBAR>(p, (int)blockIdx.x, lds);
+  p8_body<EPI, AK, BKM, ONEBAR, WIDE>(p, (int)blockIdx.x, lds);
 }
 
 constexpr int GROUP_MAX = 8;
@@ -718,6 +761,7 @@
 };
 struct GroupArgs { GroupProblem pr[GROUP_MAX]; int n; };
 
+template <bool WIDE>
 __global__ __launch_bounds__(512, 2) void gemm_kernel_p8_wgrad_group(GroupArgs g) {
   __shared__ __attribute__((aligned(16))) char lds[P_NST * P_STAGE];
   const int b = (int)blockIdx.x;
@@ -732,7 +776,7 @@
   p.M = pr.M; p.N = pr.N; p.K = pr.K; p.lda = pr.lda; p.ldb = pr.ldb; p.ldc = pr.ldc; p.ldr = 0; p.beta = pr.beta;
   p.tiles_m = pr.tiles_m; p.tiles_n = pr.tiles_n; p.full_tiles = pr.tiles_m * pr.tiles_n; p.tail_split = 1;
   p.tail_ws = nullptr; p.tail_private = 1; p.one_barrier = 1; p.wide_epilogue = 1; p.swiglu_I = 0; p.act = nullptr; p.ld_act = 0;
-  p8_body<EPI_F32, true, true, true>(p, local, lds);
+  p8_body<EPI_F32, true, true, true, WIDE>(p, local, lds);
 }
 
 constexpr int P10_GROUP_M = 4;
@@ -740,7 +784,7 @@
 constexpr int Q_TILE_A = QBM * PBK * 2;
 constexpr int Q_STAGE = Q_TILE_A + P_TILE;
 
-template <int EPI, bool BKM, int F0, int F1>
+template <int EPI, bool BKM, int F0, int F1, bool WIDE>
 __global__ __launch_bounds__(512, 2) void gemm_kernel_p10(GemmArgs p) {
   constexpr int BMV = 16 * (F0 + F1), NINST = BMV / 16, LO = NINST / 8, REM = NINST % 8;
   constexpr int TILE_A = BMV * PBK * 2, STAGE = TILE_A + P_TILE;
@@ -758,17 +802,19 @@
   const int tn = (pid % per_group) / gsz;
   const int m0 = tm * BMV, n0 = tn * PBN;
 
-  const bf16_t* asrc[3];
+  uint64_t abase = uniform64(reinterpret_cast<uint64_t>(p.A) + (uint64_t)m0 * (uint64_t)p.lda * 2);
+  const uint64_t ald2 = uniform64((uint64_t)p.lda * 2);
+  uint32_t aoff[3];
 #pragma unroll
   for (int i = 0; i < 3; ++i) {
     const int inst = min(i * 8 + wave, NINST - 1);
     const int row = inst * 16 + (lane >> 2);
     const int r = min(m0 + row, p.M - 1);
-    asrc[i] = p.A + (int64_t)r * p.lda + swz_rowk32(row, lane & 3) * 8;
-  }
-  Stager32<BKM> sb;
-  if constexpr (EPI == EPI_SWIGLU) sb.init(p.B, p.ldb, tn * 128, p.N, wave, lane, p.swiglu_I);
-  else sb.init(p.B, p.ldb, n0, p.N, wave, lane);
+    aoff[i] = lane_off<WIDE, SH_ROWK>(r - m0, swz_rowk32(row, lane & 3), ald2);
+  }
+  Stager32<BKM, WIDE> sb;
+  if constexpr (EPI == EPI_SWIGLU) sb.init(p.B, p.ldb, tn * 128, p.N, 0, wave, lane, p.swiglu_I);
+  else sb.init(p.B, p.ldb, n0, p.N, 0, wave, lane);
 
   f32x4_t acc[F0][4];
 #pragma unroll
@@ -776,32 +822,34 @@
 #pragma unroll
     for (int j = 0; j < 4; ++j) acc[i][j] = f32x4_t{0.f, 0.f, 0.f, 0.f};
   const int nk = p.K / PBK;
+  const uint32_t lds0 = lds_addr_of(lds);
 
   auto run = [&](auto group0, auto na_tag) {
     constexpr bool G0 = decltype(group0)::value;
     constexpr int NA = decltype(na_tag)::value;
     constexpr int FG = G0 ? F0 : F1;
     constexpr int PER = NA + 2;
-    auto stage_in = [&](int lt) {
-      char* st = lds + (lt & (P_NST - 1)) * STAGE;
-#pragma unroll
-      for (int i = 0; i < NA; ++i)
-        dma16(asrc[i] + (int64_t)lt * PBK, __builtin_amdgcn_readfirstlane(lds_addr_of(st + (i * 8 + wave) * 1024)));
-      sb.template issue<false>(lt, p.K, st + TILE_A, wave);
+    auto stage_in = [&](int lt, auto slot) {
+      const uint32_t st = lds0 + ring_slot(slot, lt) * STAGE;
+#pragma unroll
+      for (int i = 0; i < NA; ++i) dma_tile16<WIDE, SH_ROWK>(abase, aoff[i], ald2, st + (i * 8 + wave) * 1024);
+      abase += PBK * 2;
+      sb.template issue<false>(lt, p.K, st + TILE_A, wave, lane);
     };
     auto landed = [&](int in_flight) {
       if (in_flight >= 2) asm volatile("s_waitcnt vmcnt(%0)" ::"n"(2 * PER) : "memory");
       else if (in_flight == 1) asm volatile("s_waitcnt vmcnt(%0)" ::"n"(PER) : "memory");
       else asm volatile("s_waitcnt vmcnt(0)" ::: "memory");
     };
-    stage_in(0);
-    if (nk > 1) stage_in(1);
-    if (nk > 2) stage_in(2);
+    stage_in(0, SlotC<0>{});
+    if (nk > 1) stage_in(1, SlotC<1>{});
+    if (nk > 2) stage_in(2, SlotC<2>{});
     landed(min(nk, 3) - 1);
     P_BARRIER();
     if (!G0) P_BARRIER();
-    auto iteration = [&](int t, auto steady) {
-      const char* tA = lds + (t & (P_NST - 1)) * STAGE;
+    auto iteration = [&](int t, auto slot, auto steady) {
+      constexpr int S = decltype(slot)::value;
+      const char* tA = lds + ring_slot(slot, t) * STAGE;
       const char* tB = tA + TILE_A;
       bf16x8_t fa[FG], fb[4];
 #pragma unroll
@@ -811,10 +859,10 @@
         fb[j] = load_frag32<BKM>(tB, EPI == EPI_ROPE ? (wn >> 1) * 128 + (wn & 1) * 32 + (j & 1) * 16 + (j >> 1) * 64
                                      : EPI == EPI_SWIGLU ? (j >> 1) * 128 + wn * 32 + (j & 1) * 16 : wn * 64 + j * 16, lane);
       if constexpr (decltype(steady)::value) {
-        stage_in(t + 3);
+        stage_in(t + 3, slot_plus<S, 3>{});
         landed(2);
       } else {
-        if (t + 3 < nk) stage_in(t + 3);
+        if (t + 3 < nk) stage_in(t + 3, slot_plus<S, 3>{});
         landed(min(nk - 1, t + 3) - (t + 1));
       }
       asm volatile("s_waitcnt lgkmcnt(0)" ::: "memory");
@@ -825,8 +873,16 @@
       P_BARRIER();
     };
     int t = 0;
-    for (; t + 4 < nk; ++t) iteration(t, std::true_type{});
-    for (; t < nk; ++t) iteration(t, std::false_type{});
+    if constexpr (!WIDE) {
+      for (; t + 8 <= nk; t += 4) {
+        iteration(t, SlotC<0>{}, std::true_type{});
+        iteration(t + 1, SlotC<1>{}, std::true_type{});
+        iteration(t + 2, SlotC<2>{}, std::true_type{});
+        iteration(t + 3, SlotC<3>{}, std::true_type{});
+      }
+    }
+    for (; t + 4 < nk; ++t) iteration(t, SlotDyn{}, std::true_type{});
+    for (; t < nk; ++t) iteration(t, SlotDyn{}, std::false_type{});
     if (G0) P_BARRIER();
     if constexpr (EPI == EPI_SWIGLU_BWD)
       store_tile_swiglu_bwd<FG>(p, reinterpret_cast<f32x4_t (&)[FG][4]>(acc[0]), lds + wave * EP_STRIP, m0 + (G0 ? 0 : 16 * F0), n0 + wn * 64, lane);
@@ -893,8 +949,31 @@
 
 constexpr int WS_PRIVATE_SLOTS = UG_HANDLE_WS_SLOTS;
 
+std::atomic<int> g_addressing{1};
+bool offsets_fit32(bool kmajor, int64_t ld, int64_t row_span) {
+  const int64_t max_off = kmajor ? (int64_t)(PBK - 1) * ld * 2 + PBN * 2 : (row_span - 1) * ld * 2 + PBK * 2;
+  return max_off < (int64_t)0xffffffffLL;
+}
+bool wide_addressing(bool fit) { return g_addressing.load() == 2 || !fit; }
+#define UG_LAUNCH_P10(wide, grid, block, st, a, ...)                                                        \
+  do {                                                                                                      \
+    if (wide) hipLaunchKernelGGL((gemm_kernel_p10<__VA_ARGS__, true>), grid, block, 0, st, a);              \
+    else hipLaunchKernelGGL((gemm_kernel_p10<__VA_ARGS__, false>), grid, block, 0, st, a);                  \
+  } while (0)
+template <int EPI, bool AK, bool BKM>
+void launch_p8(const GemmArgs& a, dim3 grid, bool wide, hipStream_t st) {
+  if (a.one_barrier) {
+    if (wide) hipLaunchKernelGGL((gemm_kernel_p8<EPI, AK, BKM, true, true>), grid, dim3(512), 0, st, a);
+    else hipLaunchKernelGGL((gemm_kernel_p8<EPI, AK, BKM, true, false>), grid, dim3(512), 0, st, a);
+  } else {
+    if (wide) hipLaunchKernelGGL((gemm_kernel_p8<EPI, AK, BKM, false, true>), grid, dim3(512), 0, st, a);
+    else hipLaunchKernelGGL((gemm_kernel_p8<EPI, AK, BKM, false, false>), grid, dim3(512), 0, st, a);
+  }
+}
+
 template <int EPI, bool AK, bool BKM>
 int launch(GemmArgs a, const ug_handle* h, int policy, hipStream_t st) {
+  const bool wide8 = wide_addressing(offsets_fit32(AK, a.lda, PBM) && offsets_fit32(BKM, a.ldb, PBN));
   float* const ws = (h && h->tail_ws) ? h->tail_ws : nullptr;
   const int g_tile_policy = policy;
   const int tiles = a.tiles_m * a.tiles_n;
@@ -940,20 +1019,21 @@
     if (hb != 0) {
       a.tiles_m = (a.M + hb - 1) / hb; a.tiles_n = a.N / PBN;
       const dim3 grid(a.tiles_m * a.tiles_n), block(512);
+      const bool wide = wide_addressing(offsets_fit32(false, a.lda, hb) && offsets_fit32(BKM, a.ldb, PBN));
       switch (hb) {
-        case 320: hipLaunchKernelGGL((gemm_kernel_p10<EPI, BKM, 10, 10>), grid, block, 0, st, a); break;
-        case 304: hipLaunchKernelGGL((gemm_kernel_p10<EPI, BKM, 10, 9>), grid, block, 0, st, a); break;
-        case 288: hipLaunchKernelGGL((gemm_kernel_p10<EPI, BKM, 9, 9>), grid, block, 0, st, a); break;
-        case 272: hipLaunchKernelGGL((gemm_kernel_p10<EPI, BKM, 9, 8>), grid, block, 0, st, a); break;
-        case 256: hipLaunchKernelGGL((gemm_kernel_p10<EPI, BKM, 8, 8>), grid, block, 0, st, a); break;
-        case 240: hipLaunchKernelGGL((gemm_kernel_p10<EPI, BKM, 8, 7>), grid, block, 0, st, a); break;
-        case 224: hipLaunchKernelGGL((gemm_kernel_p10<EPI, BKM, 7, 7>), grid, block, 0, st, a); break;
-        case 208: hipLaunchKernelGGL((gemm_kernel_p10<EPI, BKM, 7, 6>), grid, block, 0, st, a); break;
-        case 192: hipLaunchKernelGGL((gemm_kernel_p10<EPI, BKM, 6, 6>), grid, block, 0, st, a); break;
-        case 176: hipLaunchKernelGGL((gemm_kernel_p10<EPI, BKM, 6, 5>), grid, block, 0, st, a); break;
-        case 160: hipLaunchKernelGGL((gemm_kernel_p10<EPI, BKM, 5, 5>), grid, block, 0, st, a); break;
-        case 144: hipLaunchKernelGGL((gemm_kernel_p10<EPI, BKM, 5, 4>), grid, block, 0, st, a); break;
-        default: hipLaunchKernelGGL((gemm_kernel_p10<EPI, BKM, 4, 4>), grid, block, 0, st, a); break;
+        case 320: UG_LAUNCH_P10(wide, grid, block, st, a, EPI, BKM, 10, 10); break;
+        case 304: UG_LAUNCH_P10(wide, grid, block, st, a, EPI, BKM, 10, 9); break;
+        case 288: UG_LAUNCH_P10(wide, grid, block, st, a, EPI, BKM, 9, 9); break;
+        case 272: UG_LAUNCH_P10(wide, grid, block, st, a, EPI, BKM, 9, 8); break;
+        case 256: UG_LAUNCH_P10(wide, grid, block, st, a, EPI, BKM, 8, 8); break;
+        case 240: UG_LAUNCH_P10(wide, grid, block, st, a, EPI, BKM, 8, 7); break;
+        case 224: UG_LAUNCH_P10(wide, grid, block, st, a, EPI, BKM, 7, 7); break;
+        case 208: UG_LAUNCH_P10(wide, grid, block, st, a, EPI, BKM, 7, 6); break;
+        case 192: UG_LAUNCH_P10(wide, grid, block, st, a, EPI, BKM, 6, 6); break;
+        case 176: UG_LAUNCH_P10(wide, grid, block, st, a, EPI, BKM, 6, 5); break;
+        case 160: UG_LAUNCH_P10(wide, grid, block, st, a, EPI, BKM, 5, 5); break;
+        case 144: UG_LAUNCH_P10(wide, grid, block, st, a, EPI, BKM, 5, 4); break;
+        default: UG_LAUNCH_P10(wide, grid, block, st, a, EPI, BKM, 4, 4); break;
       }
       UG_CHECK_LAUNCH("ug_gemm_bf16(p10)");
       return UG_OK;
@@ -984,8 +1064,7 @@
       a.tiles_m = (a.M + PBM - 1) / PBM; a.tiles_n = (a.N + PBN - 1) / PBN;
       a.full_tiles = 0; a.tail_split = sp; a.tail_private = 1;
       a.tail_ws = ws;
-      if (a.one_barrier) hipLaunchKernelGGL((gemm_kernel_p8<EPI, AK, BKM, true>), dim3(tiles_p8 * sp), dim3(512), 0, st, a);
-      else hipLaunchKernelGGL((gemm_kernel_p8<EPI, AK, BKM>), dim3(tiles_p8 * sp), dim3(512), 0, st, a);
+      launch_p8<EPI, AK, BKM>(a, dim3(tiles_p8 * sp), wide8, st);
       UG_CHECK_LAUNCH("ug_gemm_bf16(p8 k-sliced)");
       hipLaunchKernelGGL((tail_finish_kernel<EPI>), dim3(tiles_p8 * 16), dim3(256), 0, st, a, tiles_p8);
       UG_CHECK_LAUNCH("ug_gemm_bf16(partial sum)");
@@ -997,8 +1076,7 @@
     a.full_tiles = tiles_p8 - tail_r; a.tail_split = tail_s;
     a.tail_private = 1;
     a.tail_ws = ws;
-    if (a.one_barrier) hipLaunchKernelGGL((gemm_kernel_p8<EPI, AK, BKM, true>), dim3(a.full_tiles + tail_r * tail_s), dim3(512), 0, st, a);
-    else hipLaunchKernelGGL((gemm_kernel_p8<EPI, AK, BKM>), dim3(a.full_tiles + tail_r * tail_s), dim3(512), 0, st, a);
+    launch_p8<EPI, AK, BKM>(a, dim3(a.full_tiles + tail_r * tail_s), wide8, st);
     UG_CHECK_LAUNCH("ug_gemm_bf16(p8)");
     if (tail_s > 1) {
       hipLaunchKernelGGL((tail_finish_kernel<EPI>), dim3(tail_r * 16), dim3(256), 0, st, a, tail_r);
@@ -1085,11 +1163,20 @@
     start += (pr.tiles_m * pr.tiles_n + 7) & ~7;
   }
   for (int i = n; i < GROUP_MAX; ++i) { g.pr[i] = g.pr[0]; g.pr[i].start = 1 << 30; }
-  hipLaunchKernelGGL(gemm_kernel_p8_wgrad_group, dim3(start), dim3(512), 0, stream, g);
+  bool fit = true;
+  for (int i = 0; i < n; ++i) fit = fit && offsets_fit32(true, g.pr[i].lda, PBM) && offsets_fit32(true, g.pr[i].ldb, PBN);
+  if (wide_addressing(fit)) hipLaunchKernelGGL(gemm_kernel_p8_wgrad_group<true>, dim3(start), dim3(512), 0, stream, g);
+  else hipLaunchKernelGGL(gemm_kernel_p8_wgrad_group<false>, dim3(start), dim3(512), 0, stream, g);
   UG_CHECK_LAUNCH("ug_gemm_bf16_wgrad_group");
   return UG_OK;
 }
 
+
+extern "C" int ug_gemm_set_addressing(int mode) {
+  UG_REQUIRE(mode == 1 || mode == 2, "ug_gemm_set_addressing: 1 (scalar tile base + 32-bit lane offsets where they fit) or 2 (per-lane 64-bit addresses) (%d)", mode);
+  g_addressing.store(mode);
+  return UG_OK;
+}
 
 static std::atomic<int> g_fused_height{0};
 extern "C" int ug_gemm_set_fused_tile_height(int rows) {
@@ -1143,15 +1230,16 @@
   if (int rc = pick_fused_height(heights, M, 2 * I / PBN, "ug_gemm_bf16_swiglu", &hb)) return rc;
   a.tiles_m = (int)((M + hb - 1) / hb); a.tiles_n = (int)(2 * I / PBN);
   const dim3 grid(a.tiles_m * a.tiles_n), block(512);
+  const bool wide = wide_addressing(offsets_fit32(false, ldx, hb) && offsets_fit32(false, ldw, I + 128));
   switch (hb) {
-    case 320: hipLaunchKernelGGL((gemm_kernel_p10<EPI_SWIGLU, false, 10, 10>), grid, block, 0, stream, a); break;
-    case 288: hipLaunchKernelGGL((gemm_kernel_p10<EPI_SWIGLU, false, 9, 9>), grid, block, 0, stream, a); break;
-    case 256: hipLaunchKernelGGL((gemm_kernel_p10<EPI_SWIGLU, false, 8, 8>), grid, block, 0, stream, a); break;
-    case 224: hipLaunchKernelGGL((gemm_kernel_p10<EPI_SWIGLU, false, 7, 7>), grid, block, 0, stream, a); break;
-    case 208: hipLaunchKernelGGL((gemm_kernel_p10<EPI_SWIGLU, false, 7, 6>), grid, block, 0, stream, a); break;
-    case 192: hipLaunchKernelGGL((gemm_kernel_p10<EPI_SWIGLU, false, 6, 6>), grid, block, 0, stream, a); break;
-    case 160: hipLaunchKernelGGL((gemm_kernel_p10<EPI_SWIGLU, false, 5, 5>), grid, block, 0, stream, a); break;
-    default: hipLaunchKernelGGL((gemm_kernel_p10<EPI_SWIGLU, false, 4, 4>), grid, block, 0, stream, a); break;
+    case 320: UG_LAUNCH_P10(wide, grid, block, stream, a, EPI_SWIGLU, false, 10, 10); break;
+    case 288: UG_LAUNCH_P10(wide, grid, block, stream, a, EPI_SWIGLU, false, 9, 9); break;
+    case 256: UG_LAUNCH_P10(wide, grid, block, stream, a, EPI_SWIGLU, false, 8, 8); break;
+    case 224: UG_LAUNCH_P10(wide, grid, block, stream, a, EPI_SWIGLU, false, 7, 7); break;
+    case 208: UG_LAUNCH_P10(wide, grid, block, stream, a, EPI_SWIGLU, false, 7, 6); break;
+    case 192: UG_LAUNCH_P10(wide, grid, block, stream, a, EPI_SWIGLU, false, 6, 6); break;
+    case 160: UG_LAUNCH_P10(wide, grid, block, stream, a, EPI_SWIGLU, false, 5, 5); break;
+    default: UG_LAUNCH_P10(wide, grid, block, stream, a, EPI_SWIGLU, false, 4, 4); break;
   }
   UG_CHECK_LAUNCH("ug_gemm_bf16_swiglu(p10)");
   return UG_OK;
@@ -1187,15 +1275,16 @@
   if (int rc = pick_fused_height(heights, M, N / PBN, "ug_gemm_bf16_qkv_rope", &hb)) return rc;
   a.tiles_m = (int)((M + hb - 1) / hb); a.tiles_n = (int)(N / PBN);
   const dim3 grid(a.tiles_m * a.tiles_n), block(512);
+  const bool wide = wide_addressing(offsets_fit32(false, ldx, hb) && offsets_fit32(false, ldw, PBN));
   switch (hb) {
-    case 320: hipLaunchKernelGGL((gemm_kernel_p10<EPI_ROPE, false, 10, 10>), grid, block, 0, stream, a); break;
-    case 288: hipLaunchKernelGGL((gemm_kernel_p10<EPI_ROPE, false, 9, 9>), grid, block, 0, stream, a); break;
-    case 256: hipLaunchKernelGGL((gemm_kernel_p10<EPI_ROPE, false, 8, 8>), grid, block, 0, stream, a); break;
-    case 224: hipLaunchKernelGGL((gemm_kernel_p10<EPI_ROPE, false, 7, 7>), grid, block, 0, stream, a); break;
-    case 208: hipLaunchKernelGGL((gemm_kernel_p10<EPI_ROPE, false, 7, 6>), grid, block, 0, stream, a); break;
-    case 192: hipLaunchKernelGGL((gemm_kernel_p10<EPI_ROPE, false, 6, 6>), grid, block, 0, stream, a); break;
-    case 160: hipLaunchKernelGGL((gemm_kernel_p10<EPI_ROPE, false, 5, 5>), grid, block, 0, stream, a); break;
-    default: hipLaunchKernelGGL((gemm_kernel_p10<EPI_ROPE, false, 4, 4>), grid, block, 0, stream, a); break;
+    case 320: UG_LAUNCH_P10(wide, grid, block, stream, a, EPI_ROPE, false, 10, 10); break;
+    case 288: UG_LAUNCH_P10(wide, grid, block, stream, a, EPI_ROPE, false, 9, 9); break;
+    case 256: UG_LAUNCH_P10(wide, grid, block, stream, a, EPI_ROPE, false, 8, 8); break;
+    case 224: UG_LAUNCH_P10(wide, grid, block, stream, a, EPI_ROPE, false, 7, 7); break;
+    case 208: UG_LAUNCH_P10(wide, grid, block, stream, a, EPI_ROPE, false, 7, 6); break;
+    case 192: UG_LAUNCH_P10(wide, grid, block, stream, a, EPI_ROPE, false, 6, 6); break;
+    case 160: UG_LAUNCH_P10(wide, grid, block, stream, a, EPI_ROPE, false, 5, 5); break;
+    default: UG_LAUNCH_P10(wide, grid, block, stream, a, EPI_ROPE, false, 4, 4); break;
   }
   UG_CHECK_LAUNCH("ug_gemm_bf16_qkv_rope");
   return UG_OK;
@@ -1220,16 +1309,17 @@
   if (int rc = pick_fused_height(heights, M, I / PBN, "ug_gemm_bf16_swiglu_bwd", &hb)) return rc;
   a.tiles_m = (int)((M + hb - 1) / hb); a.tiles_n = (int)(I / PBN);
   const dim3 grid(a.tiles_m * a.tiles_n), block(512);
+  const bool wide = wide_addressing(offsets_fit32(false, ld_dy, hb) && offsets_fit32(true, ldw, PBN));
   switch (hb) {
-    case 320: hipLaunchKernelGGL((gemm_kernel_p10<EPI_SWIGLU_BWD, true, 10, 10>), grid, block, 0, stream, a); break;
-    case 288: hipLaunchKernelGGL((gemm_kernel_p10<EPI_SWIGLU_BWD, true, 9, 9>), grid, block, 0, stream, a); break;
-    case 272: hipLaunchKernelGGL((gemm_kernel_p10<EPI_SWIGLU_BWD, true, 9, 8>), grid, block, 0, stream, a); break;
-    case 256: hipLaunchKernelGGL((gemm_kernel_p10<EPI_SWIGLU_BWD, true, 8, 8>), grid, block, 0, stream, a); break;
-    case 224: hipLaunchKernelGGL((gemm_kernel_p10<EPI_SWIGLU_BWD, true, 7, 7>), grid, block, 0, stream, a); break;
-    case 208: hipLaunchKernelGGL((gemm_kernel_p10<EPI_SWIGLU_BWD, true, 7, 6>), grid, block, 0, stream, a); break;
-    case 192: hipLaunchKernelGGL((gemm_kernel_p10<EPI_SWIGLU_BWD, true, 6, 6>), grid, block, 0, stream, a); break;
-    case 160: hipLaunchKernelGGL((gemm_kernel_p10<EPI_SWIGLU_BWD, true, 5, 5>), grid, block, 0, stream, a); break;
-    default: hipLaunchKernelGGL((gemm_kernel_p10<EPI_SWIGLU_BWD, true, 4, 4>), grid, block, 0, stream, a); break;
+    case 320: UG_LAUNCH_P10(wide, grid, block, stream, a, EPI_SWIGLU_BWD, true, 10, 10); break;
+    case 288: UG_LAUNCH_P10(wide, grid, block, stream, a, EPI_SWIGLU_BWD, true, 9, 9); break;
+    case 272: UG_LAUNCH_P10(wide, grid, block, stream, a, EPI_SWIGLU_BWD, true, 9, 8); break;
+    case 256: UG_LAUNCH_P10(wide, grid, block, stream, a, EPI_SWIGLU_BWD, true, 8, 8); break;
+    case 224: UG_LAUNCH_P10(wide, grid, block, stream, a, EPI_SWIGLU_BWD, true, 7, 7); break;
+    case 208: UG_LAUNCH_P10(wide, grid, block, stream, a, EPI_SWIGLU_BWD, true, 7, 6); break;
+    case 192: UG_LAUNCH_P10(wide, grid, block, stream, a, EPI_SWIGLU_BWD, true, 6, 6); break;
+    case 160: UG_LAUNCH_P10(wide, grid, block, stream, a, EPI_SWIGLU_BWD, true, 5, 5); break;
+    default: UG_LAUNCH_P10(wide, grid, block, stream, a, EPI_SWIGLU_BWD, true, 4, 4); break;
   }
   UG_CHECK_LAUNCH("ug_gemm_bf16_swiglu_bwd");
   return UG_OK;
diff --git a/ml-unigen_amd/csrc/vmem_asm.h b/ml-unigen_amd/csrc/vmem_asm.h
--- a/ml-unigen_amd/csrc/vmem_asm.h
+++ b/ml-unigen_amd/csrc/vmem_asm.h
@@ -11,18 +11,21 @@
   }
 #undef UG_W
 }
+#pragma clang diagnostic push
+#pragma clang diagnostic ignored "-Winline-asm"
 __device__ __forceinline__ void dma16_nt(uint64_t base, uint32_t voff, uint32_t lds_addr) {
-  asm volatile("s_mov_b32 m0, %2\n\ts_nop 0\n\tglobal_load_lds_dwordx4 %0, %1 nt" ::"v"(voff), "s"(base), "s"(lds_addr) : "memory");
+  asm volatile("s_mov_b32 m0, %2\n\ts_nop 0\n\tglobal_load_lds_dwordx4 %0, %1 nt" ::"v"(voff), "s"(base), "s"(lds_addr) : "memory", "m0");
 }
 __device__ __forceinline__ void dma16(uint64_t base, uint32_t voff, uint32_t lds_addr) {
-  asm volatile("s_mov_b32 m0, %2\n\ts_nop 0\n\tglobal_load_lds_dwordx4 %0, %1" ::"v"(voff), "s"(base), "s"(lds_addr) : "memory");
+  asm volatile("s_mov_b32 m0, %2\n\ts_nop 0\n\tglobal_load_lds_dwordx4 %0, %1" ::"v"(voff), "s"(base), "s"(lds_addr) : "memory", "m0");
 }
 __device__ __forceinline__ void dma16_nt(const void* src, uint32_t lds_addr) {
-  asm volatile("s_mov_b32 m0, %1\n\ts_nop 0\n\tglobal_load_lds_dwordx4 %0, off nt" ::"v"(src), "s"(lds_addr) : "memory");
+  asm volatile("s_mov_b32 m0, %1\n\ts_nop 0\n\tglobal_load_lds_dwordx4 %0, off nt" ::"v"(src), "s"(lds_addr) : "memory", "m0");
 }
 __device__ __forceinline__ void dma16(const void* src, uint32_t lds_addr) {
-  asm volatile("s_mov_b32 m0, %1\n\ts_nop 0\n\tglobal_load_lds_dwordx4 %0, off" ::"v"(src), "s"(lds_addr) : "memory");
+  asm volatile("s_mov_b32 m0, %1\n\ts_nop 0\n\tglobal_load_lds_dwordx4 %0, off" ::"v"(src), "s"(lds_addr) : "memory", "m0");
 }
+#pragma clang diagnostic pop
 template <int OFF, typename T>
 __device__ __forceinline__ void ld16(T& v, uint64_t base, uint32_t voff) {
   asm volatile("global_load_dwordx4 %0, %1, %2 offset:%3" : "=&v"(v) : "v"(voff), "s"(base), "n"(OFF) : "memory");
diff --git a/ml-unigen_amd/unigen_hip/lib.py b/ml-unigen_amd/unigen_hip/lib.py
--- a/ml-unigen_amd/unigen_hip/lib.py
+++ b/ml-unigen_amd/unigen_hip/lib.py
@@ -44,6 +44,7 @@
     "ug_decode_gemv_resid_norm": [P, P, I64, P, P, P, I64, P, I64, P, I64, I64, I64, P, I64, P, I64, P, P],
     "ug_decode_gemv_swiglu": [P, I64, P, F32, I64, I64, P, I64, P, I64, I64, I64, P, I64, P, I64, P, P],
     "ug_gemm_set_fused_tile_height": [I32],
+    "ug_gemm_set_addressing": [I32],
     "ug_attn_decode_fused": [P, I64, P, F32, I64, P, P, P, P, P, P, P, P, I64, I64, I32, I32, I32, I64, I64, F32, P],
     "ug_decode_finish_resid_norm": [P, I64, P, P, P, I64, I64, F32, P, P, P],
     "ug_decode_sw_supported": [I64, I64, I64, I32],
diff --git a/ml-unigen_amd/unigen_hip/ops.py b/ml-unigen_amd/unigen_hip/ops.py
--- a/ml-unigen_amd/unigen_hip/ops.py
+++ b/ml-unigen_amd/unigen_hip/ops.py
@@ -157,6 +157,10 @@
     _l.check(_l.load().ug_gemm_set_fused_tile_height(int(rows)), "ug_gemm_set_fused_tile_height")
 
 
+def set_gemm_addressing(per_lane_64bit):
+    _l.check(_l.load().ug_gemm_set_addressing(2 if per_lane_64bit else 1), "ug_gemm_set_addressing")
+
+
 def gemm_nt(a, b, out=None, **kw):
     return gemm(a, b, out, **kw)
 
```
